# david-mathews-1994/deltarice

Measured on AMD Instinct MI355X. Metric: encode+decode GB/s (int16 in), higher is better.
Workload: dtype int16; 1 GPU; 1000000x7000 int16 Gaussian(sigma=10), m=8, 500 chunks of 2000x7000 per GPU, encode then decode, HBM resident; waveforms_per_gpu=1000000, wave_len=7000, rice_m=8, chunks_per_gpu=500, decode_impl=8

## Files before the change

deltarice_amd/_lib.py:

```python
from __future__ import annotations

import ctypes as C
import os

_HERE = os.path.dirname(os.path.abspath(__file__))
LIB_PATH = os.environ.get("DRX_LIB_PATH") or os.path.join(_HERE, "libdeltarice_hip.so")
PLUGIN_PATH = os.path.join(_HERE, "plugin", "libh5deltarice.so")

DRX_OK = 0
STATUS_NAMES = {0: "DRX_OK", 1: "DRX_ERR_ARG", 2: "DRX_ERR_DEVICE", 3: "DRX_ERR_CAPACITY",
                4: "DRX_ERR_CORRUPT", 5: "DRX_ERR_UNSUPPORTED", 6: "DRX_ERR_NOMEM"}
DRX_MAX_TAPS = 64

PATH_LANES_FUSED, PATH_LANES, PATH_BLOCKS, PATH_LONG, PATH_SIMPLE, PATH_IIR, PATH_IIR_FUSED = 1, 2, 4, 8, 16, 32, 64
PATH_SELECT = 128
PATH_GATHER = 256
PATH_STATS = 512
PATH_TRANSCODE = 1024
PATH_WINDOW = 2048
PATH_PULSES = 4096
PATH_WINDOWS = 8192
PATH_BINS = 16384
PATH_STACK = 32768
STACK_COUNT, STACK_SUM, STACK_SUMSQ = range(3)
STACK_COLS = 3
BIN_SUM, BIN_SUMSQ, BIN_MIN, BIN_MAX = range(4)
BIN_COLS = 4
STAT_MIN, STAT_ARGMIN, STAT_MAX, STAT_ARGMAX, STAT_SUM, STAT_SUMSQ, STAT_HEAD_SUM, STAT_HEAD_SUMSQ = range(8)
STAT_COLS = 8
PULSE_START, PULSE_WIDTH, PULSE_PEAK, PULSE_ARGPEAK, PULSE_SUM = range(5)
PULSE_COLS = 5
ENC_TWO_PASS, ENC_SEGMENTS, ENC_FUSED, ENC_PIECES, ENC_STREAM, ENC_STREAM_SEGS = 1, 2, 3, 4, 5, 6
DBG_BINS_LANES = 64
DBG_BINS_ALL_FALLBACK = 128
DBG_NO_LONG_PATHS = 256
DBG_LONG_NOT_BLOCKS = 512
DBG_TRANSCODE_LANES = 1024
DBG_NO_PARALLEL_WALKS = 2048
DBG_NO_PIECES = 4096
DBG_FORCE_SEGMENTS = 8192
DBG_TRANSCODE_ALL_FALLBACK = 16384
DBG_FORCE_PIECES = 32768
DBG_NO_WIDE_FUSED = 65536
DBG_RAGGED_ONE_LANES_LAUNCH = 131072
DBG_STREAM_THREE_WGS = 262144
DBG_FORCE_STREAM = 524288
DBG_REFILTER_SERIAL = 1048576
DBG_IIR_SEPARATE = 2097152
DBG_FORCE_STREAM_SEGS = 4194304
DBG_WALK_BY_SCAN = 8388608
DBG_WALK_BY_CHAINS = 16777216
DBG_GATHER_OTHER_COPY = 33554432
DBG_STATS_LANES = 67108864
DBG_STATS_ALL_FALLBACK = 134217728
DBG_PULSES_LANES = 268435456
DBG_PULSES_ALL_FALLBACK = 536870912
DBG_WINDOWS_LANES = 1073741824
DBG_WINDOWS_ALL_FALLBACK = 2147483648
STATS_FORM_LANES, STATS_FORM_BLOCKS, STATS_FORM_FALLBACK_ALL = 1, 2, 4
PULSES_FORM_LANES, PULSES_FORM_BLOCKS, PULSES_FORM_FALLBACK_ALL = 1, 2, 4
PULSES_STAGE_CAP = 8
WINDOWS_FORM_LANES, WINDOWS_FORM_BLOCKS, WINDOWS_FORM_FALLBACK_ALL = 1, 2, 4
BINS_FORM_LANES, BINS_FORM_BLOCKS, BINS_FORM_FALLBACK_ALL = 1, 2, 4
TRANSCODE_FORM_LANES, TRANSCODE_FORM_BLOCKS, TRANSCODE_FORM_FALLBACK_ALL = 1, 2, 4
TRANSCODE_FORM_REFILTER, TRANSCODE_FORM_REFILTER_SERIAL = 8, 16


class DrxOpts(C.Structure):
    _fields_ = [("rice_k", C.c_uint32), ("wave_len", C.c_int64), ("n_taps", C.c_uint32),
                ("taps", C.c_int32 * DRX_MAX_TAPS)]


class DeltaRiceError(RuntimeError):
    def __init__(self, status: int, msg: str = ""):
        self.status = status
        super().__init__(f"{STATUS_NAMES.get(status, status)}: {msg}")


_vp, _u64, _u32 = C.c_void_p, C.c_uint64, C.c_uint32
SIGNATURES = {
    "drx_version": (C.c_char_p, []),
    "drx_status_str": (C.c_char_p, [C.c_int]),
    "drx_device_count": (C.c_int, []),
    "drx_parse_cd_values": (C.c_int, [C.c_size_t, C.POINTER(C.c_uint), C.POINTER(DrxOpts)]),
    "drx_ctx_create": (C.c_int, [C.c_int, _vp, C.POINTER(_vp)]),
    "drx_ctx_destroy": (None, [_vp]),
    "drx_ctx_synchronize": (C.c_int, [_vp]),
    "drx_ctx_last_error": (C.c_char_p, [_vp]),
    "drx_ctx_stream": (_vp, [_vp]),
    "drx_ctx_device": (C.c_int, [_vp]),
    "drx_ctx_host_staging": (C.c_int, [_vp, C.c_size_t, C.POINTER(_vp)]),
    "drx_ctx_set_option": (C.c_int, [_vp, C.c_char_p, C.c_int64]),
    "drx_plan_create": (C.c_int, [_vp, _u64, C.POINTER(_u32), C.POINTER(_u32), _u32, C.POINTER(_vp)]),
    "drx_plan_create_uniform": (C.c_int, [_vp, _u64, _u32, _u32, _u32, C.POINTER(_vp)]),
    "drx_plan_set_filter": (C.c_int, [_vp, _u32, C.POINTER(C.c_int32)]),
    "drx_plan_destroy": (None, [_vp]),
    "drx_plan_n_chunks": (_u64, [_vp]),
    "drx_plan_total_samples": (_u64, [_vp]),
    "drx_plan_total_waves": (_u64, [_vp]),
    "drx_plan_max_encoded_words": (_u64, [_vp]),
    "drx_plan_wave_words": (_vp, [_vp]),
    "drx_plan_wave_word_off": (_vp, [_vp]),
    "drx_plan_last_decode_path": (C.c_uint32, [_vp]),
    "drx_plan_last_encode_path": (C.c_uint32, [_vp]),
    "drx_plan_last_stats_form": (C.c_uint32, [_vp]),
    "drx_plan_last_pulses_form": (C.c_uint32, [_vp]),
    "drx_plan_last_windows_form": (C.c_uint32, [_vp]),
    "drx_plan_last_windows_listed": (C.c_uint32, [_vp]),
    "drx_plan_last_bins_form": (C.c_uint32, [_vp]),
    "drx_plan_last_bins_listed": (C.c_uint32, [_vp]),
    "drx_plan_last_transcode_form": (C.c_uint32, [_vp]),
    "drx_plan_last_transcode_listed": (C.c_uint32, [_vp]),
    "drx_plan_last_pulses_listed": (C.c_uint32, [_vp]),
    "drx_plan_last_pulses_redone": (C.c_uint32, [_vp]),
    "drx_plan_read_wave_words": (C.c_int, [_vp, C.POINTER(_u32)]),
    "drx_encode": (C.c_int, [_vp, _vp, _vp, _u64, _vp]),
    "drx_decode": (C.c_int, [_vp, _vp, _u64, _vp, _vp]),
    "drx_decode_with_wave_words": (C.c_int, [_vp, _vp, _u64, _vp, _vp, _vp]),
    "drx_decode_select": (C.c_int, [_vp, _vp, _u64, _vp, C.POINTER(_u64), _u64, _vp, _u64]),
    "drx_decode_select_with_wave_words": (C.c_int, [_vp, _vp, _u64, _vp, _vp, C.POINTER(_u64), _u64, _vp, _u64]),
    "drx_gather_encoded": (C.c_int, [_vp, _vp, _u64, _vp, C.POINTER(_u64), _u64, _u64, _vp, _u64, _vp, _vp]),
    "drx_gather_encoded_with_wave_words": (C.c_int, [_vp, _vp, _u64, _vp, _vp, C.POINTER(_u64), _u64, _u64, _vp, _u64, _vp, _vp]),
    "drx_wave_stats": (C.c_int, [_vp, _vp, _u64, _vp, _u32, _vp]),
    "drx_wave_stats_with_wave_words": (C.c_int, [_vp, _vp, _u64, _vp, _vp, _u32, _vp]),
    "drx_wave_bins": (C.c_int, [_vp, _vp, _u64, _vp, _vp, _u64, C.c_int64, _u32, _u32, _vp, _u64]),
    "drx_wave_bins_with_wave_words": (C.c_int, [_vp, _vp, _u64, _vp, _vp, _vp, _u64, C.c_int64, _u32, _u32, _vp, _u64]),
    "drx_wave_stack": (C.c_int, [_vp, _vp, _u64, _vp, _vp, _u64, C.c_int64, _u32, _vp, _vp, _u64]),
    "drx_wave_stack_with_wave_words": (C.c_int, [_vp, _vp, _u64, _vp, _vp, _vp, _u64, C.c_int64, _u32, _vp, _vp, _u64]),
    "drx_decode_window": (C.c_int, [_vp, _vp, _u64, _vp, _vp, _u64, C.c_int64, _u32, C.c_int16, _vp, _u64]),
    "drx_decode_window_with_wave_words": (C.c_int, [_vp, _vp, _u64, _vp, _vp, _vp, _u64, C.c_int64, _u32, C.c_int16, _vp, _u64]),
    "drx_decode_windows": (C.c_int, [_vp, _vp, _u64, _vp, _vp, _u64, _u64, _vp, _u32, C.c_int64, _u32, C.c_int16, _vp, _u64, _u64]),
    "drx_decode_windows_with_wave_words": (C.c_int, [_vp, _vp, _u64, _vp, _vp, _vp, _u64, _u64, _vp, _u32, C.c_int64, _u32, C.c_int16, _vp, _u64,
                                                     _u64]),
    "drx_find_pulses": (C.c_int, [_vp, _vp, _u64, _vp, _vp, _u64, C.c_int64, C.c_int32, _u32, _u32, _vp, _vp]),
    "drx_find_pulses_with_wave_words": (C.c_int, [_vp, _vp, _u64, _vp, _vp, _vp, _u64, C.c_int64, C.c_int32, _u32, _u32, _vp, _vp]),
    "drx_transcode": (C.c_int, [_vp, _vp, _u64, _vp, _u32, _vp, _u64, _vp, _vp]),
    "drx_transcode_with_wave_words": (C.c_int, [_vp, _vp, _u64, _vp, _vp, _u32, _vp, _u64, _vp, _vp]),
    "drx_estimate_words_encoded": (C.c_int, [_vp, _vp, _u64, _vp, _vp, C.POINTER(_u64)]),
    "drx_transcode_filter": (C.c_int, [_vp, _vp, _u64, _vp, _u32, _u32, C.POINTER(C.c_int32), _vp, _u64, _vp, _vp]),
    "drx_transcode_filter_with_wave_words": (C.c_int, [_vp, _vp, _u64, _vp, _vp, _u32, _u32, C.POINTER(C.c_int32), _vp, _u64, _vp, _vp]),
    "drx_estimate_words_encoded_filter": (C.c_int, [_vp, _vp, _u64, _vp, _vp, _u32, C.POINTER(C.c_int32), C.POINTER(_u64)]),
    "drx_estimate_words": (C.c_int, [_vp, _vp, C.POINTER(_u64)]),
    "drx_plan_last_timings": (C.c_int, [_vp, C.POINTER(C.c_float)]),
    "drx_plan_finish": (C.c_int, [_vp, C.POINTER(_u64)]),
    "drx_filter_chunk_host": (C.c_int, [_vp, C.c_int, C.c_size_t, C.POINTER(C.c_uint), _vp, C.c_size_t,
                                        C.POINTER(_vp), C.POINTER(C.c_size_t)]),
}

_lib = None


def load() -> C.CDLL:
    global _lib
    if _lib is None:
        if not os.path.exists(LIB_PATH):
            raise ImportError(
                f"{LIB_PATH} is missing: build it with `make` (hipcc --offload-arch=gfx950). "
                "deltarice_amd has no CPU fallback.")
        lib = C.CDLL(LIB_PATH)
        for name, (res, args) in SIGNATURES.items():
            f = getattr(lib, name)
            f.restype = res
            f.argtypes = args
        _lib = lib
    return _lib
```

deltarice_amd/codec.py:

```python
from __future__ import annotations

import ctypes as C
import math
from dataclasses import dataclass
from typing import Optional, Sequence

import numpy as np
import torch

from . import _lib
from ._lib import DeltaRiceError, DrxOpts

H5FILTER = 32025


def _cd_values(opts: Sequence[int]):
    return (C.c_uint * max(len(opts), 1))(*[int(v) & 0xFFFFFFFF for v in opts])


def parse_opts(opts: Sequence[int] = ()) -> DrxOpts:
    lib = _lib.load()
    o = DrxOpts()
    st = lib.drx_parse_cd_values(len(opts), _cd_values(opts), C.byref(o))
    if st != _lib.DRX_OK:
# ... 605 lines not shown
        t = (1, -1) if taps is None else tuple(int(v) for v in taps)
        if not 1 <= len(t) <= _lib.DRX_MAX_TAPS:
            raise DeltaRiceError(1, f"taps: {len(t)} values (1 .. {_lib.DRX_MAX_TAPS})")
        if any(not -(1 << 31) <= v < 1 << 31 for v in t):
            raise DeltaRiceError(1, "taps: a value is not an int32")
        return (C.c_int32 * len(t))(*t), len(t), (None if t == (1, -1) else t)

    def estimate_words_refiltered(self, enc: EncodedBatch, taps: Optional[Sequence[int]],
                                  wave_words: Optional[torch.Tensor] = None) -> np.ndarray:
        self._open("estimate_words_refiltered")
        arr, n, _ = self._target_taps(taps)
        return self._estimate("drx_estimate_words_encoded_filter", enc, wave_words, n, arr)

    def refilter_async(self, words: torch.Tensor, chunk_word_off: torch.Tensor, taps: Optional[Sequence[int]], rice_m: int,
                       out_words: Optional[torch.Tensor] = None, in_words: Optional[int] = None,
                       wave_words: Optional[torch.Tensor] = None, out_chunk_word_off: Optional[torch.Tensor] = None,
                       out_wave_words: Optional[torch.Tensor] = None):
        self._open("refilter")
        k = parse_opts((int(rice_m),)).rice_k
        arr, n, _ = self._target_taps(taps)
        return self._batch_call("transcode_filter", words, chunk_word_off, wave_words, in_words, (k, n, arr), out_words,
                                out_chunk_word_off, self.n_chunks, out_wave_words, self.total_waves)

    def refilter(self, enc: EncodedBatch, taps: Optional[Sequence[int]], rice_m: Optional[int] = None,
                 wave_words: Optional[torch.Tensor] = None, out_words: Optional[torch.Tensor] = None) -> "Transcoded":
        self._open("refilter")
        _, _, carried = self._target_taps(taps)
        if rice_m is None:
            rice_m = 1 << int(np.argmin(self.estimate_words_refiltered(enc, taps, wave_words)))
        res, tab = self._sized(self.refilter_async, enc, (taps, rice_m), wave_words, out_words)
        return Transcoded(res, tab, int(rice_m), carried, self._chunk_samples.copy(), self._wave_lens.copy())

    def estimate_words(self, x: torch.Tensor) -> np.ndarray:
        self._dev_check(x, torch.int16, self.total_samples, "x")
        cur = torch.cuda.current_stream(self.ctx.device)
        self.ctx.stream.wait_stream(cur)
        out = (C.c_uint64 * 16)()
        self.ctx._check(self.ctx.lib.drx_estimate_words(self._h, x.data_ptr(), out))
        return np.array(list(out), dtype=np.uint64)

    def last_timings(self):
        ms = (C.c_float * 4)()
        self.ctx._check(self.ctx.lib.drx_plan_last_timings(self._h, ms))
        return tuple(float(v) for v in ms)

    def last_decode_path(self) -> int:
        return int(self.ctx.lib.drx_plan_last_decode_path(self._h))

    def last_stats_form(self) -> int:
        return int(self.ctx.lib.drx_plan_last_stats_form(self._h))

    def last_pulses_form(self) -> int:
        return int(self.ctx.lib.drx_plan_last_pulses_form(self._h))

    def last_windows_form(self) -> int:
        return int(self.ctx.lib.drx_plan_last_windows_form(self._h))

    def last_windows_listed(self) -> int:
        return int(self.ctx.lib.drx_plan_last_windows_listed(self._h))

    def last_bins_form(self) -> int:
        self._open("last_bins_form")
        return int(self.ctx.lib.drx_plan_last_bins_form(self._h))

    def last_bins_listed(self) -> int:
        self._open("last_bins_listed")
        return int(self.ctx.lib.drx_plan_last_bins_listed(self._h))

    def last_transcode_form(self) -> int:
        return int(self.ctx.lib.drx_plan_last_transcode_form(self._h))

    def last_transcode_listed(self) -> int:
        return int(self.ctx.lib.drx_plan_last_transcode_listed(self._h))

    def last_pulses_listed(self) -> int:
        return int(self.ctx.lib.drx_plan_last_pulses_listed(self._h))

    def last_pulses_redone(self) -> int:
        return int(self.ctx.lib.drx_plan_last_pulses_redone(self._h))

    def last_encode_path(self) -> int:
        return int(self.ctx.lib.drx_plan_last_encode_path(self._h))

    def wave_words(self) -> np.ndarray:
        buf = np.empty(self.total_waves, dtype=np.uint32)
        self.ctx._check(self.ctx.lib.drx_plan_read_wave_words(self._h, buf.ctypes.data_as(C.POINTER(C.c_uint32))))
        return buf
```

deltarice_amd/csrc/drx_api.h:

```cpp
#ifndef DRX_API_H
#define DRX_API_H
#include <hip/hip_runtime.h>

#include <cstring>
#include <mutex>
#include <string>
#include <vector>

#include "../../include/deltarice_hip.h"
#include "drx_internal.h"

struct Grown {
    void *ptr = nullptr;
    size_t cap = 0;
};

class Buffers {
    struct Buf { void *ptr; bool pinned; };
    std::vector<Buf> bufs_;
    static void free_buf(const Buf &b) {
        if (b.pinned) (void)hipHostFree(b.ptr);
        else (void)hipFree(b.ptr);
    }

// ... 21 lines not shown
    }
    template <typename T> hipError_t once(T **out, size_t bytes, bool pinned = false) {
        return *out ? hipSuccess : alloc(out, bytes, pinned);
    }

    enum Order { KeepOld, ReleaseFirst };
    static size_t size(size_t need, unsigned slack) { return slack ? need + need / slack + 4096 : need; }
    hipError_t reserve(Grown &b, size_t need, unsigned slack, bool pinned, Order order, hipStream_t wait) {
        if (b.cap >= need) return hipSuccess;
        void *fresh = nullptr;
        hipError_t e = order == KeepOld ? alloc(&fresh, size(need, slack), pinned) : hipSuccess;
        if (e == hipSuccess && b.ptr) e = hipStreamSynchronize(wait);
        if (e != hipSuccess) { release(fresh); return e; }
        release(b.ptr);
        b = Grown{};
        if (order == ReleaseFirst && (e = alloc(&fresh, size(need, slack), pinned)) != hipSuccess) return e;
        b = Grown{fresh, size(need, slack)};
        return hipSuccess;
    }
};

struct HostPlanKey {
    uint32_t samples = 0, wave_len = 0, k = 0, n_taps = 0;
    int32_t taps[DRX_MAX_TAPS] = {0};
    bool operator==(const HostPlanKey &o) const {
        return samples == o.samples && wave_len == o.wave_len && k == o.k && n_taps == o.n_taps && memcmp(taps, o.taps, sizeof taps) == 0;
    }
};

struct drx_ctx {
    int device = 0;
    hipStream_t stream = nullptr;
    bool own_stream = false;
    drx::SideStream side{nullptr, nullptr, nullptr};
    int decode_impl = 8;
    int encode_impl = 2;
    int bins_impl = 0;
    uint32_t stack_workgroups = 0;
    int profile = 0;
    uint32_t debug_flags = 0;
    std::string last_error;
    Buffers mem;
    struct HostPath {
        Grown d_raw, d_enc, h_pin;
        uint64_t *d_off = nullptr;
        drx_plan *plan = nullptr;
        HostPlanKey key;
    } host;
    Grown h_stage;
    std::mutex mu;
    std::mutex err_mu;
};

struct DeviceGuard {
    int prev = -1;
    hipError_t err;
    explicit DeviceGuard(int device) {
        if (hipGetDevice(&prev) != hipSuccess) prev = -1;
        err = (prev == device) ? hipSuccess : hipSetDevice(device);
        if (prev == device) prev = -1;
    }
    ~DeviceGuard() { if (prev >= 0) (void)hipSetDevice(prev); }
    DeviceGuard(const DeviceGuard &) = delete;
    DeviceGuard &operator=(const DeviceGuard &) = delete;
};
#define DRX_ON_DEVICE(ctx)                                                                         \
    DeviceGuard dev_guard_((ctx)->device);                                                         \
    if (dev_guard_.err != hipSuccess)                                                              \
        return drx::fail((ctx), DRX_ERR_DEVICE, "hipSetDevice(%d) failed: %s", (ctx)->device, hipGetErrorString(dev_guard_.err))

struct drx_plan {
    drx_ctx *ctx = nullptr;
    drx::Geom G{};
    Buffers mem;
    uint64_t max_words = 0;
    std::vector<drx::ChunkDesc> host_chunks;
    uint32_t *d_wave_words = nullptr;
    uint32_t *d_wave_rel = nullptr;
    uint64_t *d_wave_off = nullptr;
    uint64_t *d_chunk_words = nullptr;
    drx::DevStatus *d_status = nullptr;
    drx::DevStatus *h_status = nullptr;
    bool last_was_encode = false;
    struct Encoders {
        Grown scan;
        uint32_t *d_seg_bits = nullptr;
        uint64_t *d_seg_pos = nullptr;
        uint64_t *d_pc_scan = nullptr;
        uint64_t pc_wgs = 0;
        uint32_t last_path = 0;
        uint64_t words_per_wave = 0;
    } enc;
    struct Decoder {
        void *d_pw = nullptr;
        void *d_blk = nullptr;
        uint32_t last_path = 0;
    } dec;
    struct BlockForm {
        void *d = nullptr;
        uint32_t last_form = 0;
    };
    BlockForm stats;
    BlockForm windows;
    BlockForm bins;
    struct Pulses : BlockForm {
        Grown stage;
    } pulses;
    struct Transcode { void *d = nullptr; BlockForm blocks; } trc;
    void *stack_list = nullptr;
    struct Selection {
        Grown h, d;
        uint32_t *d_fail = nullptr;
        hipEvent_t copied = nullptr;
    } sel;
    struct Gather {
        Grown d;
        struct Key {
            bool valid = false;
            const uint32_t *d_in = nullptr, *d_sideband = nullptr;
            const uint64_t *d_off = nullptr;
            uint64_t in_words = 0, n_sel = 0, cw = 0;
        } last;
    } gat;
    struct Profiling {
        hipEvent_t ev[4] = {nullptr, nullptr, nullptr, nullptr};
        bool valid = false;
    } prof;
};

namespace drx {

drx_status fail(drx_ctx *ctx, drx_status st, const char *fmt, ...) __attribute__((format(printf, 3, 4)));

#define DRX_HIP(ctx, expr)                                                                           \
    do {                                                                                             \
        hipError_t e_ = (expr);                                                                      \
        if (e_ != hipSuccess)                                                                        \
            return drx::fail((ctx), DRX_ERR_DEVICE, "%s failed: %s", #expr, hipGetErrorString(e_)); \
    } while (0)

void plan_free(drx_plan *p);
hipError_t seg_scratch(drx_plan *p);

drx_status call_begin(drx_plan *p);
drx_status stream_call_begin(drx_plan *p, const uint32_t *d_in, uint64_t in_words, const uint64_t *d_chunk_word_off,
                             const uint32_t *d_sideband, bool tables_ready, StreamCall *c);
drx_status call_end(drx_plan *p, uint32_t path, bool encode = false);
drx_status stream_call_args(drx_plan *p, const char *who, bool have_pointers, const uint32_t *d_sideband, bool sideband);

drx_status decode_launch(drx_plan *p, const uint32_t *d_in, uint64_t in_words, const uint64_t *d_chunk_word_off, int16_t *d_out,
                         bool tables_ready, const uint32_t *d_sideband = nullptr);

}
#endif
```

deltarice_amd/csrc/drx_api_encode.hip:

```cpp
#include "drx_api.h"

using namespace drx;

static bool stream_encoder_suits(const drx_plan *p, int wide) {
    const Geom &G = p->G;
    if (wide != 0 || G.total_waves < kEsMinUnits) return false;
    const uint64_t L = G.uniform ? G.u_wave_len : G.max_wave_len64 / 64u;
    const uint64_t words = p->enc.words_per_wave ? p->enc.words_per_wave : (L * (2u * G.k + 7u)) / 64u;
    return words <= (uint64_t)kEsRingWords * 67u / 100u;
}

static uint32_t stream_segs_target(const drx_plan *p) {
    const Geom &G = p->G;
    const uint64_t L = G.u_wave_len;
    if (L < kEsSegsFromLen) return 0u;
    const uint64_t bps16 = p->enc.words_per_wave ? (p->enc.words_per_wave * 512u) / L : 16u * G.k + 56u;
    uint64_t t = ((uint64_t)kEsRingWords * 32u * 57u / 100u) * 16u / (bps16 ? bps16 : 1u);
    t = t > kEsSegMaxLen ? kEsSegMaxLen : (t < kEsSegMinLen ? kEsSegMinLen : t);
    const EsSegShape sh = es_seg_shape((uint32_t)L, (uint32_t)t);
    if (G.total_waves * sh.nseg < kEsMinUnits) return 0u;
    return (uint32_t)t;
}

struct EncodeRoute { uint32_t enc, seg_target; int wide; };

static EncodeRoute route_encode(const drx_plan *p, int impl, uint32_t dbg) {
    const Geom &G = p->G;
    const int wide = (dbg & DRX_DBG_NO_WIDE_FUSED) ? 0 : fused_wide(G);
    const bool fast = G.n_taps == 0 || G.enc_fast, single = impl >= 1;
    const bool segs_in = impl == 2 && stream_segs_admits(G), pieces_in = single && pieces_admits(G);
    const bool long_in = single && long_batch_admits(G), stream_in = impl == 2 && fast && G.total_waves < 0xffff0000ull;
    const bool fused_in = single && fast && G.total_waves <= kMaxWavefrontWaves;
    if ((dbg & DRX_DBG_FORCE_STREAM_SEGS) && segs_in) return {DRX_ENC_STREAM_SEGS, kEsSegMinLen, wide};
    if ((dbg & DRX_DBG_FORCE_SEGMENTS) && long_in) return {DRX_ENC_SEGMENTS, 0, wide};
    if ((dbg & DRX_DBG_FORCE_PIECES) && pieces_in) return {DRX_ENC_PIECES, 0, wide};
    if ((dbg & DRX_DBG_FORCE_STREAM) && stream_in) return {DRX_ENC_STREAM, 0, wide};
    if (segs_in && !(dbg & (DRX_DBG_NO_PIECES | DRX_DBG_NO_LONG_PATHS)))
        if (const uint32_t t = stream_segs_target(p)) return {DRX_ENC_STREAM_SEGS, t, wide};
    if (pieces_in && !(dbg & DRX_DBG_NO_PIECES) && pieces_batch(G, wide)) return {DRX_ENC_PIECES, 0, wide};
    if (long_in && !(dbg & DRX_DBG_NO_LONG_PATHS) && long_batch(G)) return {DRX_ENC_SEGMENTS, 0, wide};
    if (stream_in && stream_encoder_suits(p, wide)) return {DRX_ENC_STREAM, 0, wide};
    return {fused_in ? DRX_ENC_FUSED : DRX_ENC_TWO_PASS, 0, wide};
}

static drx_status route_scratch(drx_plan *p, const EncodeRoute &R) {
    drx_ctx *ctx = p->ctx;
    if (R.enc == DRX_ENC_STREAM_SEGS)
        DRX_HIP(ctx, p->mem.reserve(p->enc.scan, segs_scan_words(p->G, R.seg_target) * sizeof(uint64_t), 4, false, Buffers::KeepOld, ctx->stream));
    if (R.enc == DRX_ENC_SEGMENTS) DRX_HIP(ctx, seg_scratch(p));
    return DRX_OK;
}

extern "C" {

drx_status drx_encode(drx_plan *p, const int16_t *d_in, uint32_t *d_out, uint64_t out_cap_words,
                      uint64_t *d_chunk_word_off) {
    if (!p || !d_in || !d_out || !d_chunk_word_off) return DRX_ERR_ARG;
    drx_ctx *ctx = p->ctx;
    DRX_ON_DEVICE(ctx);
    if (const drx_status st = call_begin(p)) return st;
    if (const uint64_t w = *(volatile uint64_t *)p->G.host_words) p->enc.words_per_wave = p->G.total_waves ? w / p->G.total_waves : 0;
    const EncodeRoute R = route_encode(p, ctx->encode_impl, ctx->debug_flags);
    if (const drx_status st = route_scratch(p, R)) return st;
    const EncodeCall c{&p->G, d_in, EncOut{d_out, out_cap_words, d_chunk_word_off, p->d_wave_words}, p->d_status,
                       ctx->profile ? p->prof.ev : nullptr, ctx->stream};
    const drx_plan::Encoders &E = p->enc;
    uint64_t *d_scan = (uint64_t *)E.scan.ptr;
    switch (R.enc) {
    case DRX_ENC_STREAM_SEGS: DRX_HIP(ctx, launch_encode_stream_segs(c, R.seg_target, d_scan)); break;
    case DRX_ENC_PIECES: DRX_HIP(ctx, launch_encode_pieces(c, p->G.total_samples, E.d_pc_scan, E.pc_wgs)); break;
    case DRX_ENC_SEGMENTS: DRX_HIP(ctx, launch_encode_long(c, p->d_wave_rel, p->d_chunk_words, E.d_seg_bits, E.d_seg_pos)); break;
    case DRX_ENC_STREAM: DRX_HIP(ctx, launch_encode_stream(c, d_scan)); break;
    case DRX_ENC_FUSED: DRX_HIP(ctx, launch_encode_fused(c, R.wide, d_scan)); break;
    default: DRX_HIP(ctx, launch_encode(c, p->d_wave_rel, p->d_chunk_words));
    }
    return call_end(p, R.enc,  true);
}

drx_status drx_estimate_words(drx_plan *p, const int16_t *d_in, uint64_t words_out[16]) {
    if (!p || !d_in || !words_out) return DRX_ERR_ARG;
    drx_ctx *ctx = p->ctx;
    DRX_ON_DEVICE(ctx);
    DRX_HIP(ctx, hipStreamSynchronize(ctx->stream));
    DRX_HIP(ctx, launch_estimate_words(p->G, d_in, (unsigned long long *)p->enc.scan.ptr, ctx->stream));
    DRX_HIP(ctx, hipMemcpyAsync(words_out, p->enc.scan.ptr, 16 * sizeof(uint64_t), hipMemcpyDeviceToHost, ctx->stream));
    DRX_HIP(ctx, hipStreamSynchronize(ctx->stream));
    return DRX_OK;
}

}
```

deltarice_amd/csrc/drx_api_plan.hip:

```cpp
#include <cstdarg>
#include <cstdio>
#include <cstdlib>
#include <new>

#include "drx_api.h"

using namespace drx;

drx_status drx::fail(drx_ctx *ctx, drx_status st, const char *fmt, ...) {
    char buf[512];
    va_list ap;
    va_start(ap, fmt);
    vsnprintf(buf, sizeof buf, fmt, ap);
    va_end(ap);
    if (ctx) {
        std::lock_guard<std::mutex> lock(ctx->err_mu);
        ctx->last_error = buf;
    }
    return st;
}

drx_status drx::call_begin(drx_plan *p) {
    drx_ctx *ctx = p->ctx;
    p->gat.last.valid = false;
    DRX_HIP(ctx, hipMemsetAsync(p->d_status, 0, sizeof(DevStatus), ctx->stream));
    p->G.dbg = ctx->debug_flags;
    return DRX_OK;
}
drx_status drx::stream_call_begin(drx_plan *p, const uint32_t *d_in, uint64_t in_words, const uint64_t *d_chunk_word_off,
                                  const uint32_t *d_sideband, bool tables_ready, StreamCall *c) {
    drx_ctx *ctx = p->ctx;
    if (const drx_status st = call_begin(p)) return st;
    *c = StreamCall{&p->G, d_in, in_words, d_chunk_word_off, p->d_wave_off, p->d_wave_words, tables_ready || d_sideband, p->dec.d_pw,
                    p->d_status, ctx->profile ? p->prof.ev : nullptr, ctx->stream};
    if (d_sideband)
        DRX_HIP(ctx, launch_sideband_tables(*c, d_sideband));
    return DRX_OK;
}
drx_status drx::call_end(drx_plan *p, uint32_t path, bool encode) {
    (encode ? p->enc.last_path : p->dec.last_path) = path;
    p->prof.valid = p->ctx->profile != 0;
    p->last_was_encode = encode;
    return DRX_OK;
}
drx_status drx::stream_call_args(drx_plan *p, const char *who, bool have_pointers, const uint32_t *d_sideband, bool sideband) {
    if (!have_pointers || (sideband && !d_sideband)) return fail(p->ctx, DRX_ERR_ARG, "%s: null pointer", who);
    if (sideband && d_sideband == p->d_wave_words) return fail(p->ctx, DRX_ERR_ARG, "the side-band table must not be the plan's own (copy it first)");
    return DRX_OK;
}

template <typename T> static hipError_t upload(drx_plan *p, const T *host, size_t n, const T **view) {
    if (!n) return hipSuccess;
    T *d = const_cast<T *>(*view);
    const hipError_t e = p->mem.once(&d, n * sizeof(T));
    if (e != hipSuccess) return e;
    *view = d;
    return hipMemcpy(d, host, n * sizeof(T), hipMemcpyHostToDevice);
}
template <typename T> static hipError_t upload(drx_plan *p, const std::vector<T> &tab, const T **view) {
    return upload(p, tab.data(), tab.size(), view);
}

void drx::plan_free(drx_plan *p) {
    if (!p) return;
    DeviceGuard guard(p->ctx->device);
    for (hipEvent_t e : p->prof.ev) if (e) (void)hipEventDestroy(e);
    if (p->sel.copied) (void)hipEventDestroy(p->sel.copied);
    delete p;
}

hipError_t drx::seg_scratch(drx_plan *p) {
    drx_plan::Encoders &E = p->enc;
    if (E.d_seg_bits) return hipSuccess;
    const uint64_t units = long_batch_units(p->G);
    hipError_t e = p->mem.once(&E.d_seg_bits, units * sizeof(uint32_t));
    if (e == hipSuccess && (e = p->mem.once(&E.d_seg_pos, units * sizeof(uint64_t))) != hipSuccess) {
        p->mem.release(E.d_seg_bits);
        E.d_seg_bits = nullptr;
    }
    return e;
}

static drx_status plan_alloc(drx_plan *p) {
    drx_ctx *ctx = p->ctx;
    Geom &G = p->G;
    const uint64_t W = G.total_waves ? G.total_waves : 1;
    DRX_HIP(ctx, p->mem.alloc(&p->d_wave_words, W * sizeof(uint32_t)));
    DRX_HIP(ctx, p->mem.alloc(&p->d_wave_rel, W * sizeof(uint32_t)));
    DRX_HIP(ctx, p->mem.alloc(&p->d_wave_off, W * sizeof(uint64_t)));
    DRX_HIP(ctx, p->mem.alloc(&p->d_chunk_words, (G.n_chunks + 1) * sizeof(uint64_t)));
    uint64_t words = 2 * W + 192;
    if (stream_segs_admits(G) && G.u_wave_len >= kEsSegsFromLen) words = std::max(words, segs_scan_words(G, kEsSegMinLen));
    DRX_HIP(ctx, p->mem.reserve(p->enc.scan, words * sizeof(uint64_t), 0, false, Buffers::KeepOld, ctx->stream));
    DRX_HIP(ctx, p->mem.alloc(&p->d_status, sizeof(DevStatus)));
    DRX_HIP(ctx, hipMemset(p->d_status, 0, sizeof(DevStatus)));
    DRX_HIP(ctx, p->mem.alloc(&p->h_status, sizeof(DevStatus), true));
    memset(p->h_status, 0, sizeof(DevStatus));
    DRX_HIP(ctx, p->mem.alloc(&G.host_words, sizeof(uint64_t), true));
    *G.host_words = 0;
    for (hipEvent_t &e : p->prof.ev) DRX_HIP(ctx, hipEventCreate(&e));
    return DRX_OK;
}

static drx_status plan_ragged(drx_plan *p, const std::vector<ChunkDesc> &desc) {
    Geom &G = p->G;
    const ChunkDesc *d = desc.data();
    const std::vector<uint32_t> walk_lists = walk_plan_ragged(G, d);
    const std::vector<uint2> order = decode_plan_ragged(G, d);
    const std::vector<uint64_t> unit_base = segments_plan_ragged(G, d);
    const std::vector<uint32_t> wg_base = pieces_plan_ragged(G, d);
    p->enc.pc_wgs = wg_base.empty() ? 0 : wg_base.back();
    const std::vector<uint32_t> blk_list = blocks_plan_ragged(G, d);
    std::vector<uint64_t> tile_base;
    if (!blk_list.empty()) {
        tile_base.resize(G.n_chunks + 1);
        G.iir_n_tiles = iir_tiles(G, d, tile_base.data());
    }
    hipError_t e = upload(p, desc, &G.chunks);
    if (e == hipSuccess) e = upload(p, walk_lists, &G.walk_short);
    if (e == hipSuccess) e = upload(p, order, &G.rag_order);
    if (e == hipSuccess) e = upload(p, unit_base, &G.seg_unit_base);
    if (e == hipSuccess) e = upload(p, wg_base, &G.pc_wg_base);
    if (e == hipSuccess) e = upload(p, blk_list, &G.rag_blk_list);
    if (e == hipSuccess) e = upload(p, tile_base, &G.iir_chunk_tile_base);
    if (e != hipSuccess) return fail(p->ctx, DRX_ERR_DEVICE, "chunk table upload failed: %s", hipGetErrorString(e));
    G.walk_long = G.walk_short + G.n_short;
    return DRX_OK;
}

static drx_status plan_alloc_scratch(drx_plan *p) {
    drx_ctx *ctx = p->ctx;
    Geom &G = p->G;
    if (long_batch(G)) DRX_HIP(ctx, seg_scratch(p));
    if (const uint64_t nb = walk_scratch_bytes(G)) DRX_HIP(ctx, p->mem.alloc(&p->dec.d_pw, nb));
    if (const uint64_t nb = blocks_scratch_bytes(G)) {
        DRX_HIP(ctx, p->mem.alloc(&p->dec.d_blk, nb));
        if (G.uniform) G.iir_n_tiles = iir_tiles(G, nullptr, nullptr);
        DRX_HIP(ctx, p->mem.alloc(&G.iir_state, (G.iir_n_tiles + 1) * sizeof(uint64_t)));
    }
    if (G.uniform && pieces_admits(G)) p->enc.pc_wgs = pieces_workgroups(G);
    if (p->enc.pc_wgs) DRX_HIP(ctx, p->mem.alloc(&p->enc.d_pc_scan, pieces_scan_words(G, p->enc.pc_wgs) * sizeof(uint64_t)));
    return DRX_OK;
}

static drx_status chunk_desc(drx_ctx *ctx, uint64_t c, uint32_t N, uint32_t wave_len, ChunkDesc *out) {
    if (N == 0 || N > 0x7fffffffu) return fail(ctx, DRX_ERR_ARG, "chunk %llu: bad sample count %u", (unsigned long long)c, N);
    const uint32_t L = wave_len ? wave_len : N;
    if (L > 0x7fffffffu) return fail(ctx, DRX_ERR_ARG, "chunk %llu: bad waveform length", (unsigned long long)c);
    *out = ChunkDesc{0, 0, N, L, (uint32_t)(((uint64_t)N + L - 1) / L), 0};
    return DRX_OK;
}

static drx_status plan_create(drx_ctx *ctx, uint64_t n_chunks, const uint32_t *chunk_samples, const uint32_t *chunk_wave_len,
                              bool per_chunk, uint32_t rice_k, drx_plan **out) {
    if (!ctx || !out || !n_chunks || !chunk_samples || !chunk_wave_len) return DRX_ERR_ARG;
    *out = nullptr;
    if (rice_k > 15) return fail(ctx, DRX_ERR_ARG, "rice_k %u out of range 0..15", rice_k);
    if (n_chunks > 0xffffffffull) return fail(ctx, DRX_ERR_ARG, "too many chunks");
    ChunkDesc first;
    if (const drx_status st = chunk_desc(ctx, 0, chunk_samples[0], chunk_wave_len[0], &first)) return st;
    std::vector<ChunkDesc> desc;
    bool uniform = true;
    if (per_chunk) {
        desc.resize(n_chunks);
        uint64_t soff = 0, wbase = 0;
        for (uint64_t c = 0; c < n_chunks; ++c) {
            if (const drx_status st = chunk_desc(ctx, c, chunk_samples[c], chunk_wave_len[c], &desc[c])) return st;
            desc[c].sample_off = soff;
            desc[c].wave_base = wbase;
            uniform = uniform && desc[c].n_samples == first.n_samples && desc[c].wave_len == first.wave_len;
            soff += desc[c].n_samples;
            wbase += desc[c].n_waves;
        }
        if (uniform) desc.clear();
    }
    DRX_ON_DEVICE(ctx);
    drx_plan *p = new (std::nothrow) drx_plan;
    if (!p) return DRX_ERR_NOMEM;
// ... 154 lines not shown
    if (!strcmp(key, "debug_flags")) {
        c->debug_flags = (uint32_t)value;
        return DRX_OK;
    }
    if (!strcmp(key, "profile")) {
        c->profile = value != 0;
        return DRX_OK;
    }
    return DRX_ERR_ARG;
}

drx_status drx_plan_create(drx_ctx *ctx, uint64_t n_chunks, const uint32_t *chunk_samples,
                           const uint32_t *chunk_wave_len, uint32_t rice_k, drx_plan **out) {
    return plan_create(ctx, n_chunks, chunk_samples, chunk_wave_len, true, rice_k, out);
}

drx_status drx_plan_create_uniform(drx_ctx *ctx, uint64_t n_chunks, uint32_t chunk_samples,
                                   uint32_t wave_len, uint32_t rice_k, drx_plan **out) {
    return plan_create(ctx, n_chunks, &chunk_samples, &wave_len, false, rice_k, out);
}

drx_status drx_plan_set_filter(drx_plan *p, uint32_t n_taps, const int32_t *taps) {
    if (!p || !taps || n_taps == 0 || n_taps > DRX_MAX_TAPS) return DRX_ERR_ARG;
    drx_ctx *ctx = p->ctx;
    if (taps[0] == 0) return fail(ctx, DRX_ERR_ARG, "taps[0] must not be 0 (the inverse filter divides by it)");
    DRX_ON_DEVICE(ctx);
    DRX_HIP(ctx, hipStreamSynchronize(ctx->stream));
    Geom &G = p->G;
    p->enc.words_per_wave = 0;
    p->gat.last.valid = false;
    *G.host_words = 0;
    G.fast_taps = 0;
    G.enc_fast = 0;
    const bool delta = n_taps == 2 && taps[0] == 1 && taps[1] == -1;
    if (!delta && n_taps <= 4) {
        G.enc_fast = 1;
        for (uint32_t j = 0; j < 4; ++j) G.enc_t[j] = (j < n_taps) ? (uint32_t)taps[j] & 0xffffu : 0u;
    }
    if (!delta && n_taps <= 4 && (taps[0] == 1 || taps[0] == -1)) {
        G.fast_taps = 1;
        G.fast_t0neg = taps[0] == -1;
        for (uint32_t j = 1; j < 4; ++j) G.fast_nt[j - 1] = (j < n_taps) ? 0u - (uint32_t)taps[j] : 0u;
    }
    if (G.fast_taps && G.iir_state) {
        const uint32_t words = kIirTabWords + blocks_iir_tab_words();
        std::vector<uint32_t> tab(words);
        iir_tables(G.fast_nt, G.fast_t0neg, tab.data());
        blocks_iir_tables(G.fast_nt, G.fast_t0neg, tab.data() + kIirTabWords);
        DRX_HIP(ctx, upload(p, tab, &G.iir_tab));
        G.blk_iir_tab = G.iir_tab + kIirTabWords;
    } else {
        p->mem.release(G.iir_tab);
        G.iir_tab = G.blk_iir_tab = nullptr;
    }
    if (delta) {
        p->mem.release(G.taps);
        G.n_taps = 0;
        G.taps = nullptr;
        return DRX_OK;
    }
    int32_t t[DRX_MAX_TAPS] = {0};
    memcpy(t, taps, n_taps * sizeof(int32_t));
    DRX_HIP(ctx, upload(p, t, DRX_MAX_TAPS, &G.taps));
    G.n_taps = n_taps;
    return DRX_OK;
}

void drx_plan_destroy(drx_plan *p) { plan_free(p); }
uint64_t drx_plan_n_chunks(const drx_plan *p) { return p ? p->G.n_chunks : 0; }
uint64_t drx_plan_total_samples(const drx_plan *p) { return p ? p->G.total_samples : 0; }
uint64_t drx_plan_total_waves(const drx_plan *p) { return p ? p->G.total_waves : 0; }
uint64_t drx_plan_max_encoded_words(const drx_plan *p) { return p ? p->max_words : 0; }
const uint32_t *drx_plan_wave_words(const drx_plan *p) { return p ? p->d_wave_words : nullptr; }
const uint64_t *drx_plan_wave_word_off(const drx_plan *p) { return p ? p->d_wave_off : nullptr; }
uint32_t drx_plan_last_decode_path(const drx_plan *p) { return p ? p->dec.last_path : 0u; }
uint32_t drx_plan_last_encode_path(const drx_plan *p) { return p ? p->enc.last_path : 0u; }
uint32_t drx_plan_last_stats_form(const drx_plan *p) { return p ? p->stats.last_form : 0u; }
uint32_t drx_plan_last_pulses_form(const drx_plan *p) { return p ? p->pulses.last_form : 0u; }
uint32_t drx_plan_last_windows_form(const drx_plan *p) { return p ? p->windows.last_form : 0u; }
uint32_t drx_plan_last_transcode_form(const drx_plan *p) { return p ? p->trc.blocks.last_form : 0u; }
uint32_t drx_plan_last_transcode_listed(const drx_plan *p) { return (p && p->h_status && p->dec.last_path == DRX_PATH_TRANSCODE) ? p->h_status->listed : 0u; }
uint32_t drx_plan_last_pulses_redone(const drx_plan *p) { return (p && p->h_status && p->dec.last_path == DRX_PATH_PULSES) ? p->h_status->redone : 0u; }
uint32_t drx_plan_last_pulses_listed(const drx_plan *p) { return (p && p->h_status && p->dec.last_path == DRX_PATH_PULSES) ? p->h_status->listed : 0u; }
uint32_t drx_plan_last_bins_form(const drx_plan *p) { return p ? p->bins.last_form : 0u; }
uint32_t drx_plan_last_bins_listed(const drx_plan *p) { return (p && p->h_status && p->dec.last_path == DRX_PATH_BINS) ? p->h_status->listed : 0u; }
uint32_t drx_plan_last_windows_listed(const drx_plan *p) { return (p && p->h_status && p->dec.last_path == DRX_PATH_WINDOWS) ? p->h_status->listed : 0u; }

drx_status drx_plan_read_wave_words(drx_plan *p, uint32_t *host_out) {
    if (!p || !host_out) return DRX_ERR_ARG;
    drx_ctx *ctx = p->ctx;
    DRX_ON_DEVICE(ctx);
    DRX_HIP(ctx, hipMemcpyAsync(host_out, p->d_wave_words, p->G.total_waves * sizeof(uint32_t),
                                hipMemcpyDeviceToHost, ctx->stream));
    DRX_HIP(ctx, hipStreamSynchronize(ctx->stream));
    return DRX_OK;
}

drx_status drx_plan_last_timings(drx_plan *p, float ms[4]) {
    if (!p || !ms) return DRX_ERR_ARG;
    drx_ctx *ctx = p->ctx;
    if (!p->prof.valid) return fail(ctx, DRX_ERR_ARG, "set the context option \"profile\" before the call to be timed");
    DRX_ON_DEVICE(ctx);
    hipEvent_t *ev = p->prof.ev;
    DRX_HIP(ctx, hipEventSynchronize(ev[3]));
    for (int i = 0; i < 3; ++i) DRX_HIP(ctx, hipEventElapsedTime(&ms[i], ev[i], ev[i + 1]));
    DRX_HIP(ctx, hipEventElapsedTime(&ms[3], ev[0], ev[3]));
    return DRX_OK;
}

drx_status drx_plan_finish(drx_plan *p, uint64_t *total_words) {
    if (!p) return DRX_ERR_ARG;
    drx_ctx *ctx = p->ctx;
    DRX_ON_DEVICE(ctx);
    DRX_HIP(ctx, hipMemcpyAsync(p->h_status, p->d_status, sizeof(DevStatus), hipMemcpyDeviceToHost, ctx->stream));
    DRX_HIP(ctx, hipStreamSynchronize(ctx->stream));
    if (total_words) *total_words = p->h_status->total_words;
    if (p->last_was_encode && !p->h_status->err && p->G.total_waves) p->enc.words_per_wave = p->h_status->total_words / p->G.total_waves;
    if (p->h_status->err & kErrInternal) return fail(ctx, DRX_ERR_DEVICE, "encoder look-back timed out (internal error)");
    if (p->h_status->err & kErrCorrupt) return fail(ctx, DRX_ERR_CORRUPT, "encoded input failed header-chain validation");
    if (p->h_status->err & kErrCapacity)
        return fail(ctx, DRX_ERR_CAPACITY, "encoded batch needs %llu words", (unsigned long long)p->h_status->total_words);
    return DRX_OK;
}

}
```

deltarice_amd/csrc/drx_api_select.hip:

```cpp
#include <algorithm>
#include <new>

#include "drx_api.h"
#include "drx_sel_survey.h"

using namespace drx;

template <typename F>
static int plan_survey(drx_plan *p, const char *who, const uint64_t *wave_idx, uint64_t n_sel, bool sideband,
                       std::vector<uint32_t> &lists, uint32_t n_class[3], uint64_t *at, F &&per_entry) {
    const Geom &G = p->G;
    const SelGeom S{G.uniform != 0, G.n_chunks, G.total_waves, G.u_n_samples, G.u_wave_len, G.u_n_waves};
    const int r = sel_survey(S, p->host_chunks.data(), wave_idx, n_sel, sideband, select_walk_class, lists, n_class, at, per_entry);
    if (r == kSelBadIndex)
        (void)fail(p->ctx, DRX_ERR_ARG, "%s: entry %llu is waveform %llu of %llu", who, (unsigned long long)*at,
                   (unsigned long long)wave_idx[*at], (unsigned long long)G.total_waves);
    return r;
}

static drx_status sel_scratch(drx_plan *p, size_t bytes) {
    drx_ctx *ctx = p->ctx;
    drx_plan::Selection &S = p->sel;
    if (!S.copied) DRX_HIP(ctx, hipEventCreateWithFlags(&S.copied, hipEventDisableTiming));
    DRX_HIP(ctx, p->mem.once(&S.d_fail, p->G.n_chunks * sizeof(uint32_t)));
    DRX_HIP(ctx, p->mem.reserve(S.h, bytes, 4, true, Buffers::KeepOld, ctx->stream));
    const hipError_t e = p->mem.reserve(S.d, bytes, 4, false, Buffers::KeepOld, ctx->stream);
    if (e != hipSuccess) return fail(ctx, DRX_ERR_NOMEM, "selection scratch of %zu bytes: %s", Buffers::size(bytes, 4), hipGetErrorString(e));
    return DRX_OK;
}

static drx_status gather_scratch(drx_plan *p, size_t bytes) {
    const hipError_t e = p->mem.reserve(p->gat.d, bytes, 4, false, Buffers::KeepOld, p->ctx->stream);
    if (e != hipSuccess) return fail(p->ctx, DRX_ERR_NOMEM, "gather scratch of %zu bytes: %s", Buffers::size(bytes, 4), hipGetErrorString(e));
    return DRX_OK;
}

struct SelStaged {
    const uint64_t *d_sel;
    const uint32_t *d_chunk_n, *d_lists;
};
static SelStaged sel_staged(const drx_plan *p, uint64_t n_sel, uint64_t n_out) {
    const uint32_t *d_chunk_n = (const uint32_t *)((const char *)p->sel.d.ptr + n_sel * sizeof(uint64_t));
    return SelStaged{(const uint64_t *)p->sel.d.ptr, d_chunk_n, d_chunk_n + n_out};
}
static drx_status sel_stage(drx_plan *p, const uint64_t *wave_idx, uint64_t n_sel, const std::vector<uint32_t> &chunk_n,
                            const std::vector<uint32_t> &lists, size_t gather_bytes) {
    drx_ctx *ctx = p->ctx;
    const size_t sel_bytes = n_sel * sizeof(uint64_t), cn_bytes = chunk_n.size() * sizeof(uint32_t), ls_bytes = lists.size() * sizeof(uint32_t);
    if (const drx_status st = sel_scratch(p, sel_bytes + cn_bytes + ls_bytes)) return st;
    if (gather_bytes)
        if (const drx_status st = gather_scratch(p, gather_bytes)) return st;
    char *h_sel = (char *)p->sel.h.ptr;
    DRX_HIP(ctx, hipEventSynchronize(p->sel.copied));
    memcpy(h_sel, wave_idx, sel_bytes);
    if (cn_bytes) memcpy(h_sel + sel_bytes, chunk_n.data(), cn_bytes);
    memcpy(h_sel + sel_bytes + cn_bytes, lists.data(), ls_bytes);
    DRX_HIP(ctx, hipMemcpyAsync(p->sel.d.ptr, h_sel, sel_bytes + cn_bytes + ls_bytes, hipMemcpyHostToDevice, ctx->stream));
    DRX_HIP(ctx, hipEventRecord(p->sel.copied, ctx->stream));
    return DRX_OK;
}
static drx_status sel_walk(drx_plan *p, const StreamCall &c, const uint32_t *d_sideband, const uint32_t *d_lists, size_t n_lists,
                           const uint32_t n_class[3]) {
    drx_ctx *ctx = p->ctx;
    mark(c.ev, 0, c.s);
    if (d_sideband)
        DRX_HIP(ctx, launch_sideband_tables(c, d_sideband, d_lists, (uint32_t)n_lists));
    else
        DRX_HIP(ctx, launch_select_walk(c, d_lists, n_class[0], n_class[1], n_class[2], p->sel.d_fail));
    mark(c.ev, 1, c.s);
    return DRX_OK;
}

template <typename F> static drx_status list_call(drx_plan *p, const char *who, uint64_t n_sel, F &&f) {
    try {
        return f();
    } catch (const std::bad_alloc &) { return fail(p->ctx, DRX_ERR_NOMEM, "%s: host memory for a list of %llu entries", who, (unsigned long long)n_sel); }
}

static drx_status decode_select(drx_plan *p, const uint32_t *d_in, uint64_t in_words, const uint64_t *d_chunk_word_off,
                                const uint32_t *d_sideband, bool sideband, const uint64_t *wave_idx, uint64_t n_sel,
                                int16_t *d_out, uint64_t stride) {
    if (!p) return DRX_ERR_ARG;
    drx_ctx *ctx = p->ctx;
    if (n_sel == 0) return DRX_OK;
    if (!d_in || !d_chunk_word_off || !wave_idx || !d_out || (sideband && !d_sideband)) return fail(ctx, DRX_ERR_ARG, "decode_select: null pointer");
    if (sideband && d_sideband == p->d_wave_words) return fail(ctx, DRX_ERR_ARG, "the side-band table must not be the plan's own (copy it first)");
    if (n_sel >= (1ull << 32)) return fail(ctx, DRX_ERR_ARG, "decode_select: %llu entries (at most 2^32 - 1)", (unsigned long long)n_sel);
    uint32_t longest = 0;
    uint32_t n_class[3];
    uint64_t at;
    std::vector<uint32_t> lists;
    if (plan_survey(p, "decode_select", wave_idx, n_sel, sideband, lists, n_class, &at, [&](uint64_t, uint64_t, uint32_t len) {
            longest = std::max(longest, len);
            return 0;
        }))
        return DRX_ERR_ARG;
    p->gat.last.valid = false;
    if (stride < longest) return fail(ctx, DRX_ERR_ARG, "decode_select: row stride %llu below the longest selected waveform (%u)", (unsigned long long)stride, longest);
    DRX_ON_DEVICE(ctx);
    if (const drx_status st = sel_stage(p, wave_idx, n_sel, {}, lists, 0)) return st;
    const SelStaged S = sel_staged(p, n_sel, 0);
    StreamCall c;
    if (const drx_status st = stream_call_begin(p, d_in, in_words, d_chunk_word_off, nullptr, false, &c)) return st;
    if (const drx_status st = sel_walk(p, c, sideband ? d_sideband : nullptr, S.d_lists, lists.size(), n_class)) return st;
    DRX_HIP(ctx, launch_decode_select(c, S.d_sel, n_sel, d_out, stride));
    mark(c.ev, 2, c.s);
    mark(c.ev, 3, c.s);
    return call_end(p, DRX_PATH_SELECT);
}

constexpr uint64_t kGatherWavesFromWords = 192;

static drx_status gather_encoded(drx_plan *p, const uint32_t *d_in, uint64_t in_words, const uint64_t *d_chunk_word_off,
                                 const uint32_t *d_sideband, bool sideband, const uint64_t *wave_idx, uint64_t n_sel,
                                 uint64_t cw, uint32_t *d_out, uint64_t out_cap, uint64_t *d_out_off, uint32_t *d_out_wave_words) {
    if (!p) return DRX_ERR_ARG;
    drx_ctx *ctx = p->ctx;
    if (cw == 0) return fail(ctx, DRX_ERR_ARG, "gather_encoded: out_chunk_waves is 0");
    if (n_sel == 0) return DRX_OK;
    if (!d_in || !d_chunk_word_off || !wave_idx || !d_out_off || (sideband && !d_sideband)) return fail(ctx, DRX_ERR_ARG, "gather_encoded: null pointer");
    if (!d_out && out_cap) return fail(ctx, DRX_ERR_ARG, "gather_encoded: no output buffer but a capacity of %llu words", (unsigned long long)out_cap);
    if (sideband && (d_sideband == p->d_wave_words || d_out_wave_words == d_sideband))
        return fail(ctx, DRX_ERR_ARG, "the side-band table must be neither the plan's own nor the output's (copy it first)");
    if (n_sel >= (1ull << 32)) return fail(ctx, DRX_ERR_ARG, "gather_encoded: %llu entries (at most 2^32 - 1)", (unsigned long long)n_sel);
    const Geom &G = p->G;
    const uint64_t n_out = (n_sel + cw - 1) / cw;
    const EncOut out{d_out, out_cap, d_out_off, d_out_wave_words};
    const uint64_t mean_words = in_words / G.total_waves;
    const bool tiles = (mean_words < kGatherWavesFromWords) != ((ctx->debug_flags & DRX_DBG_GATHER_OTHER_COPY) != 0);
    const drx_plan::Gather::Key K = p->gat.last;
    p->gat.last.valid = false;
    if (K.valid && d_out && K.d_in == d_in && K.in_words == in_words && K.d_off == d_chunk_word_off && K.d_sideband == (sideband ? d_sideband : nullptr) &&
        K.n_sel == n_sel && K.cw == cw && memcmp(p->sel.h.ptr, wave_idx, n_sel * sizeof(uint64_t)) == 0) {
        DRX_ON_DEVICE(ctx);
        StreamCall c;
        if (const drx_status st = stream_call_begin(p, d_in, in_words, d_chunk_word_off, nullptr, true, &c)) return st;
        const SelStaged S = sel_staged(p, n_sel, n_out);
        mark(c.ev, 0, c.s);
        mark(c.ev, 1, c.s);
        DRX_HIP(ctx, launch_gather(c, S.d_sel, n_sel, cw, S.d_chunk_n, out, gather_scratch_view(p->gat.d.ptr, n_sel), tiles, mean_words,  true));
        mark(c.ev, 3, c.s);
        return call_end(p, DRX_PATH_GATHER);
    }
    std::vector<uint32_t> chunk_n(n_out);
    GatherChunks rule{cw, chunk_n.data()};
    uint32_t n_class[3], refused_len = 0;
    uint64_t at;
    std::vector<uint32_t> lists;
    const int refused = plan_survey(p, "gather_encoded", wave_idx, n_sel, sideband, lists, n_class, &at, [&](uint64_t i, uint64_t, uint32_t len) {
        refused_len = len;
        return (int)rule.add(i, len);
// ... 62 lines not shown
```

deltarice_amd/csrc/drx_api_stream.hip:

```cpp
#include "drx_api.h"

using namespace drx;

drx_status drx::decode_launch(drx_plan *p, const uint32_t *d_in, uint64_t in_words, const uint64_t *d_chunk_word_off, int16_t *d_out,
                              bool tables_ready, const uint32_t *d_sideband) {
    if (!p || !d_in || !d_chunk_word_off || !d_out) return DRX_ERR_ARG;
    drx_ctx *ctx = p->ctx;
    DRX_ON_DEVICE(ctx);
    StreamCall c;
    if (const drx_status st = stream_call_begin(p, d_in, in_words, d_chunk_word_off, d_sideband, tables_ready, &c)) return st;
    DRX_HIP(ctx, launch_decode(c, d_out, (uint64_t *)p->enc.scan.ptr, ctx->decode_impl, p->dec.d_blk, ctx->side.s ? &ctx->side : nullptr,
                               &p->dec.last_path));
    return call_end(p, p->dec.last_path);
}

static hipError_t form_scratch(drx_plan *p, const BlkFormRule &r, drx_plan::BlockForm &f, uint64_t (*bytes)(const Geom &)) {
    return blocks_form_batch(p->G, p->dec.d_blk, r) ? p->mem.once(&f.d, bytes(p->G)) : hipSuccess;
}

static drx_status wave_stats(drx_plan *p, const uint32_t *d_in, uint64_t in_words, const uint64_t *d_chunk_word_off,
                             const uint32_t *d_sideband, bool sideband, uint32_t head_len, int64_t *d_out) {
    if (!p) return DRX_ERR_ARG;
    drx_ctx *ctx = p->ctx;
    if (const drx_status st = stream_call_args(p, "wave_stats", d_in && d_chunk_word_off && d_out, d_sideband, sideband)) return st;
    DRX_ON_DEVICE(ctx);
    StreamCall c;
    if (const drx_status st = stream_call_begin(p, d_in, in_words, d_chunk_word_off, d_sideband, false, &c)) return st;
    DRX_HIP(ctx, form_scratch(p, kStatsForm, p->stats, stats_blocks_scratch_bytes));
    DRX_HIP(ctx, launch_wave_stats(c, p->dec.d_blk, p->stats.d, head_len, d_out, &p->stats.last_form));
    return call_end(p, DRX_PATH_STATS);
}

static drx_status wave_bins(drx_plan *p, const uint32_t *d_in, uint64_t in_words, const uint64_t *d_chunk_word_off,
                            const uint32_t *d_sideband, bool sideband, const int64_t *d_start, uint64_t start_stride, int64_t offset,
                            uint32_t bin, uint32_t n_bins, int64_t *d_out, uint64_t out_wave_stride) {
    if (!p) return DRX_ERR_ARG;
    drx_ctx *ctx = p->ctx;
    if (const drx_status st = stream_call_args(p, "wave_bins", d_in && d_chunk_word_off && d_out, d_sideband, sideband)) return st;
    if (bin == 0) return fail(ctx, DRX_ERR_ARG, "wave_bins: bin 0");
    if (d_start && start_stride == 0) return fail(ctx, DRX_ERR_ARG, "wave_bins: start_stride 0");
    if (out_wave_stride < (uint64_t)n_bins * DRX_BIN_COLS)
        return fail(ctx, DRX_ERR_ARG, "wave_bins: waveforms %llu int64 apart do not hold %u rows", (unsigned long long)out_wave_stride, n_bins);
    if (n_bins == 0) return DRX_OK;
    DRX_ON_DEVICE(ctx);
    StreamCall c;
    if (const drx_status st = stream_call_begin(p, d_in, in_words, d_chunk_word_off, d_sideband, false, &c)) return st;
    if (ctx->bins_impl == 1) DRX_HIP(ctx, form_scratch(p, kBinsForm, p->bins, bins_blocks_scratch_bytes));
    DRX_HIP(ctx, launch_wave_bins(c, p->dec.d_blk, p->bins.d, ctx->bins_impl, d_start, start_stride, offset, bin, n_bins, d_out, out_wave_stride,
                                  &p->bins.last_form));
    return call_end(p, DRX_PATH_BINS);
}

static drx_status decode_window(drx_plan *p, const uint32_t *d_in, uint64_t in_words, const uint64_t *d_chunk_word_off,
                                const uint32_t *d_sideband, bool sideband, const int64_t *d_start, uint64_t start_stride,
                                int64_t offset, uint32_t width, int16_t pad, int16_t *d_out, uint64_t out_stride) {
    if (!p) return DRX_ERR_ARG;
    drx_ctx *ctx = p->ctx;
    if (const drx_status st = stream_call_args(p, "decode_window", d_in && d_chunk_word_off && d_out, d_sideband, sideband)) return st;
    if (out_stride < width)
        return fail(ctx, DRX_ERR_ARG, "decode_window: rows %llu samples apart do not hold %u", (unsigned long long)out_stride, width);
    if (d_start && start_stride == 0) return fail(ctx, DRX_ERR_ARG, "decode_window: start_stride 0");
    if (width == 0) return DRX_OK;
    DRX_ON_DEVICE(ctx);
    StreamCall c;
    if (const drx_status st = stream_call_begin(p, d_in, in_words, d_chunk_word_off, d_sideband, false, &c)) return st;
    DRX_HIP(ctx, launch_decode_window(c, d_start, start_stride, offset, width, pad, d_out, out_stride));
    return call_end(p, DRX_PATH_WINDOW);
}

static drx_status wave_stack(drx_plan *p, const uint32_t *d_in, uint64_t in_words, const uint64_t *d_chunk_word_off,
                             const uint32_t *d_sideband, bool sideband, const int64_t *d_start, uint64_t start_stride, int64_t offset,
                             uint32_t width, const uint8_t *d_select, int64_t *d_out, uint64_t out_stride) {
    if (!p) return DRX_ERR_ARG;
    drx_ctx *ctx = p->ctx;
    if (const drx_status st = stream_call_args(p, "wave_stack", d_in && d_chunk_word_off && d_out, d_sideband, sideband)) return st;
    if (d_start && start_stride == 0) return fail(ctx, DRX_ERR_ARG, "wave_stack: start_stride 0");
    if (out_stride < (uint64_t)DRX_STACK_COLS)
        return fail(ctx, DRX_ERR_ARG, "wave_stack: rows %llu int64 apart do not hold %d", (unsigned long long)out_stride, DRX_STACK_COLS);
    if (width == 0) return DRX_OK;
    DRX_ON_DEVICE(ctx);
    StreamCall c;
    if (const drx_status st = stream_call_begin(p, d_in, in_words, d_chunk_word_off, d_sideband, false, &c)) return st;
    if (d_select) DRX_HIP(ctx, p->mem.once(&p->stack_list, stack_list_bytes(p->G)));
    DRX_HIP(ctx, launch_wave_stack(c, p->stack_list, ctx->stack_workgroups, d_start, start_stride, offset, width, d_select, d_out, out_stride));
    return call_end(p, DRX_PATH_STACK);
}

static drx_status decode_windows(drx_plan *p, const uint32_t *d_in, uint64_t in_words, const uint64_t *d_chunk_word_off,
                                 const uint32_t *d_sideband, bool sideband, const int64_t *d_start, uint64_t start_wave_stride,
                                 uint64_t start_win_stride, const uint32_t *d_count, uint32_t n_win, int64_t offset, uint32_t width,
                                 int16_t pad, int16_t *d_out, uint64_t out_wave_stride, uint64_t out_win_stride) {
    if (!p) return DRX_ERR_ARG;
    drx_ctx *ctx = p->ctx;
    if (const drx_status st = stream_call_args(p, "decode_windows", d_in && d_chunk_word_off && d_start && d_out, d_sideband, sideband)) return st;
    if (start_wave_stride == 0 || start_win_stride == 0) return fail(ctx, DRX_ERR_ARG, "decode_windows: a start stride of 0");
// ... 262 lines not shown
```

deltarice_amd/csrc/drx_decode_kernels.hip:

```cpp
#include <hip/hip_runtime.h>
#include <stdint.h>

#include <algorithm>
#include <type_traits>

#include "drx_internal.h"
#include "drx_device.h"
#include "drx_lane_stream.h"
#include "drx_walk.h"

namespace drx {

__global__ __launch_bounds__(64) void k_decode_simple(Geom G, const uint32_t *__restrict__ in,
                                                      const uint64_t *__restrict__ wave_off,
                                                      const uint32_t *__restrict__ wave_words, DevStatus *st,
                                                      int16_t *__restrict__ out, const uint32_t *__restrict__ only) {
    const uint64_t g = (uint64_t)blockIdx.x * 64u + threadIdx.x;
    if (g >= G.total_waves) return;
    if (only && !only[g]) return;
    const WaveRef r = locate(G, g);
    const uint32_t *s = in + wave_off[g] + 1;
    const uint32_t n = wave_words[g];
    int16_t *y = out + r.sample_off;
    int16_t hist[64];
// ... 547 lines not shown
            const int st = i * SPI + lane / PPS, p = lane % PPS;
            const uint4 v = orow16(st, p);
            store16(outg + wo_off[i] + t0, v);
        }
        wave_sync();
    }
    commit_if_fits();
    pneed = false;
    wave_sync();
    for (; t0 < steps; t0 += T) edge_round(t0);
    if (active && len && (((0u - Q_end) - 32u * s0 + 31u) >> 5) != n) atomicOr(&st->err, kErrCorrupt);
}

std::vector<uint2> decode_plan_ragged(Geom &G, const ChunkDesc *d) {
    const uint64_t n = G.n_chunks;
    uint32_t max_groups = 0, max_len = 0;
    for (uint64_t c = 0; c < n; ++c) {
        max_groups = std::max(max_groups, (d[c].n_waves + 63u) / 64u);
        max_len = std::max(max_len, d[c].wave_len);
    }
    G.max_groups = max_groups;
    G.max_wave_len64 = 64ull * max_len;
    std::vector<uint32_t> by_len(n);
    for (uint64_t c = 0; c < n; ++c) by_len[c] = (uint32_t)c;
    std::stable_sort(by_len.begin(), by_len.end(), [&](uint32_t a, uint32_t b) { return d[a].wave_len > d[b].wave_len; });
    std::vector<uint2> order;
    uint64_t n_long_groups = 0;
    for (uint32_t c : by_len)
        for (uint32_t j = 0; j < (d[c].n_waves + 63u) / 64u; ++j) {
            order.push_back(make_uint2(c, j));
            if (d[c].wave_len > kWalkShortLen) ++n_long_groups;
        }
    if (order.size() <= 0x7fffffffull) {
        G.rag_groups = (uint32_t)order.size();
        G.rag_groups_long = (uint32_t)n_long_groups;
    } else {
        order.clear();
    }
    return order;
}

enum class Dec { Simple, Blocks, Long, LanesFused, Lanes, LanesSplit };
enum class Walk { None, InLaunch, Parallel, Serial };
struct DecodeRoute {
    Dec dec;
    Walk walk;
    WalkRoute par;
    bool gen;
};

static DecodeRoute route_decode(const Geom &G, int impl, bool tables_ready, bool have_pw, bool have_blk, bool have_side) {
    DecodeRoute R{};
    R.gen = G.n_taps != 0;
    R.par = route_walk(G, tables_ready, have_pw);
    const bool simple = impl == 0 || (R.gen && !G.fast_taps);
    const bool want_fused = !tables_ready && impl == 8;
    const bool blocks = !simple && !(G.dbg & (DRX_DBG_NO_LONG_PATHS | DRX_DBG_LONG_NOT_BLOCKS)) && have_blk && blocks_batch(G) && (!R.gen || (G.iir_tab && G.iir_state));
    const bool longp = !simple && !blocks && !R.gen && !(G.dbg & DRX_DBG_NO_LONG_PATHS) && G.uniform && long_waveform_batch(G.total_waves, G.u_wave_len);
    const bool sparse = !G.uniform && (uint64_t)G.n_chunks * G.max_groups > 8ull * ((G.total_waves + 63u) / 64u) + 4096ull;
    R.dec = simple ? Dec::Simple : (blocks ? Dec::Blocks : (longp ? Dec::Long : Dec::Lanes));
    const bool parallel = R.par.chunk_wide || R.par.blocks;
    if (R.dec == Dec::Lanes && want_fused && !sparse && !parallel) R.dec = Dec::LanesFused;
    R.walk = tables_ready ? Walk::None : (R.dec == Dec::LanesFused ? Walk::InLaunch : (parallel ? Walk::Parallel : Walk::Serial));
    if (R.dec == Dec::Lanes && R.par.chunk_wide && R.par.blocks && have_side && G.rag_order && G.rag_groups_long &&
        G.rag_groups_long < G.rag_groups && !(G.dbg & DRX_DBG_RAGGED_ONE_LANES_LAUNCH)) R.dec = Dec::LanesSplit;
    return R;
}

hipError_t launch_decode(const StreamCall &c, int16_t *d_out, uint64_t *d_granules, int impl, void *d_blk, const SideStream *side,
                         uint32_t *path_out) {
    const Geom &G = *c.G;
    const hipStream_t s = c.s;
    uint32_t path_dummy = 0;
    uint32_t &path = path_out ? *path_out : path_dummy;
    path = 0;
    if (G.total_waves == 0) return hipSuccess;
    mark(c.ev, 0, s);
    const DecodeRoute R = route_decode(G, impl, c.tables_ready, c.d_pw != nullptr, d_blk != nullptr, side && side->s);
    const bool gen = R.gen;
    const unsigned nb_plain = blocks_for(G.total_waves, 64);

    auto launch_lanes = [&](const StreamCall &v, unsigned nb) {
        path |= DRX_PATH_LANES;
        if (gen)
            k_decode_lanes<false, true><<<nb, 64, 0, v.s>>>(*v.G, v.d_in, v.in_words, v.d_chunk_word_off, v.d_wave_off, v.d_wave_words, nullptr, nullptr, v.d_status, d_out);
        else
            k_decode_lanes<false><<<nb, 64, 0, v.s>>>(*v.G, v.d_in, v.in_words, v.d_chunk_word_off, v.d_wave_off, v.d_wave_words, nullptr, nullptr, v.d_status, d_out);
    };

    if (R.walk == Walk::InLaunch) {
        hipError_t e = hipMemsetAsync(d_granules, 0, (G.total_waves + 2) * sizeof(uint64_t), s);
        if (e != hipSuccess) return e;
    } else if (R.walk == Walk::Parallel) {
        const bool split = R.dec == Dec::LanesSplit;
        hipError_t e = walk_scratch_reset(G, c.d_pw, s);
        if (e != hipSuccess) return e;
        const bool forked = R.par.chunk_wide && R.par.blocks && side && side->s;
        hipStream_t spw = forked ? side->s : s;
        if (forked) {
            if ((e = hipEventRecord(side->fork, s)) != hipSuccess) return e;
            if ((e = hipStreamWaitEvent(side->s, side->fork, 0)) != hipSuccess) return e;
        }
        if (R.par.chunk_wide) launch_walk_chunk_wide(c.on(spw), R.par.by_chains);
        if (split) {
            Geom Gl = G;
            Gl.rag_groups = G.rag_groups_long;
            launch_lanes(c.view(Gl).on(spw), Gl.rag_groups);
        }
        if (forked && (e = hipEventRecord(side->join, side->s)) != hipSuccess) {
            (void)hipStreamSynchronize(side->s);
            return e;
        }
        if (R.par.blocks) launch_walk_blocks(c);
        if (split) {
            mark(c.ev, 1, s);
            Geom Gs = G;
            Gs.rag_order = G.rag_order + G.rag_groups_long;
            Gs.rag_groups = G.rag_groups - G.rag_groups_long;
            launch_lanes(c.view(Gs), Gs.rag_groups);
        }
        if (forked && (e = hipStreamWaitEvent(s, side->join, 0)) != hipSuccess) {
            (void)hipStreamSynchronize(side->s);
            return e;
        }
    } else if (R.walk == Walk::Serial) {
        launch_walk_serial(c);
    }
    if (R.dec != Dec::LanesSplit) mark(c.ev, 1, s);

    switch (R.dec) {
    case Dec::LanesFused: {
        uint32_t *ticket = reinterpret_cast<uint32_t *>(d_granules + G.total_waves);
        unsigned n_walk, groups;
        unsigned nb;
        if (G.uniform) {
            n_walk = (G.u_wave_len <= kWalkShortLen) ? (unsigned)G.n_chunks : blocks_for(G.n_chunks, kWalkChains);
            groups = (G.u_n_waves + 63u) / 64u;
            const uint32_t full = G.u_n_waves >> 6, rem = G.u_n_waves & 63u;
            nb = n_walk + (unsigned)(G.n_chunks * full) + (rem ? (unsigned)((G.n_chunks + 64u / rem - 1u) / (64u / rem)) : 0u);
        } else {
            n_walk = G.n_short + blocks_for(G.n_long, kWalkChains);
            groups = G.max_groups;
            nb = n_walk + (unsigned)(G.n_chunks * groups);
        }
        path |= DRX_PATH_LANES_FUSED;
        if (gen)
            k_decode_lanes<true, true><<<nb, 64, 0, s>>>(G, c.d_in, c.in_words, c.d_chunk_word_off, c.d_wave_off, c.d_wave_words, d_granules, ticket, c.d_status, d_out);
        else
            k_decode_lanes<true><<<nb, 64, 0, s>>>(G, c.d_in, c.in_words, c.d_chunk_word_off, c.d_wave_off, c.d_wave_words, d_granules, ticket, c.d_status, d_out);
        break;
    }
    case Dec::Blocks: {
        const uint32_t *fail = nullptr, *suspect = nullptr;
        bool fused = false;
        hipError_t e = launch_decode_blocks(c, d_blk, d_out, &fail, &suspect, gen, &fused);
        if (e != hipSuccess) return e;
        path |= DRX_PATH_BLOCKS | (gen ? (fused ? DRX_PATH_IIR_FUSED : DRX_PATH_IIR) : 0u);
        k_decode_long<<<(unsigned)G.total_waves, kLongThreads, 0, s>>>(G, c.d_in, c.d_wave_off, c.d_wave_words, c.d_status, d_out, fail, suspect, gen ? 1u : 0u);
        if (gen) {
            if (!fused && (e = launch_iir(G, G.iir_chunk_tile_base, G.iir_n_tiles, G.iir_tab, G.iir_state, fail, c.d_status, d_out, s)) != hipSuccess) return e;
            k_decode_simple<<<nb_plain, 64, 0, s>>>(G, c.d_in, c.d_wave_off, c.d_wave_words, c.d_status, d_out, fail);
        }
        break;
    }
    case Dec::Long:
        path |= DRX_PATH_LONG;
        k_decode_long<<<(unsigned)G.total_waves, kLongThreads, 0, s>>>(G, c.d_in, c.d_wave_off, c.d_wave_words, c.d_status, d_out, nullptr, nullptr, 0u);
        break;
    case Dec::Lanes:
        launch_lanes(c, (!G.uniform && G.rag_order) ? G.rag_groups : nb_plain);
        break;
    case Dec::LanesSplit:
        break;
    case Dec::Simple:
        path |= DRX_PATH_SIMPLE;
        k_decode_simple<<<nb_plain, 64, 0, s>>>(G, c.d_in, c.d_wave_off, c.d_wave_words, c.d_status, d_out, nullptr);
        break;
    }
    mark(c.ev, 2, s);
    mark(c.ev, 3, s);
    return hipGetLastError();
}

}
```

deltarice_amd/csrc/drx_encode_kernels.hip:

```cpp
#include <hip/hip_runtime.h>
#include <stdint.h>

#include <algorithm>
#include <type_traits>

#include "drx_internal.h"
#include "drx_device.h"
#include "drx_encode.h"
#include "drx_lookback.h"

namespace drx {

constexpr int kStageWords = 416;

__device__ __forceinline__ int load8(const int16_t *__restrict__ x, uint32_t len, uint32_t t0, int lane,
                                     bool vec_ok, int32_t v[8]) {
    const uint32_t i0 = t0 + 8u * (uint32_t)lane;
    const int nv = (i0 >= len) ? 0 : (int)((len - i0) < 8u ? (len - i0) : 8u);
    if (vec_ok && nv == 8) {
        const uint4 q = *reinterpret_cast<const uint4 *>(x + i0);
        v[0] = (int16_t)(q.x & 0xffffu); v[1] = (int16_t)(q.x >> 16);
        v[2] = (int16_t)(q.y & 0xffffu); v[3] = (int16_t)(q.y >> 16);
        v[4] = (int16_t)(q.z & 0xffffu); v[5] = (int16_t)(q.z >> 16);
        v[6] = (int16_t)(q.w & 0xffffu); v[7] = (int16_t)(q.w >> 16);
// ... 476 lines not shown
                                                  const uint64_t *__restrict__ chunk_word_off, uint32_t *__restrict__ out,
                                                  uint64_t out_cap, uint32_t upw) {
    __shared__ __attribute__((aligned(16))) uint32_t stage_all[4][4 + kStageWords + 12];
    const int lane = lane_id();
    const int wv = wave_id();
    uint32_t *row = stage_all[wv];
    uint32_t *stage = row + 4;
    const uint64_t u0 = ((uint64_t)blockIdx.x * 4u + (uint32_t)wv) * upw;
    for (uint32_t rep = 0; rep < upw; ++rep) {
        const uint64_t u = u0 + rep;
        if (u >= n_units) return;
        const SegRef q = locate_seg_uniform(G, u, segs_per_wave);
        if (q.count == 0) continue;
        for (int i = lane; i < 4 + (int)kStageWords + 12; i += 64) row[i] = 0;
        const uint64_t pos = chunk_word_off[q.r.chunk] + wave_rel[q.g];
        const uint32_t n = wave_words[q.g];
        if (pos + 1u + n > out_cap) continue;
        if (q.s == 0 && lane == 0) {
            out[pos] = n;
            if (q.r.idx == 0) out[pos - 1] = q.r.n_samples;
        }
        const uint64_t B = seg_pos[u];
        uint32_t *__restrict__ outp = out + pos + 1 + (B >> 5);
        const uint32_t stage_bits = lds_addr(stage) * 8u;
        uint32_t P = (uint32_t)(B & 31u);
        uint32_t wdone = 0;
        bool shared_first = (B & 31u) != 0;
        wave_sync();
        for_segment_tiles(in + q.r.sample_off, q, G.k, lane,
                          [&](const PackedCodes &c, uint32_t lane_bits, uint32_t incl, uint32_t tile_bits, bool full) {
            if (full && !__any(lane_bits > 128u)) {
                uint32_t cw[4];
                concat_codes(c, cw);
                place_words(cw, stage_bits + P + incl);
            } else {
                emit_tile<false>(c, stage_bits + P + incl - lane_bits);
            }
            P += tile_bits;
            wave_sync();
            const uint32_t nfull = P >> 5;
            for (uint32_t i = lane; i < nfull; i += 64) {
                const uint32_t v = stage[i];
                stage[i] = 0;
                if (i == 0 && shared_first) atomicOr(outp + wdone, v); else outp[wdone + i] = v;
            }
            wave_sync();
            if (nfull) {
                if (lane == 0) { const uint32_t cwd = stage[nfull]; stage[nfull] = 0; stage[0] = cwd; }
                shared_first = false;
                wdone += nfull;
                P &= 31u;
            }
            wave_sync();
        });
        if (P && lane == 0) {
            if (q.last && !shared_first) outp[wdone] = stage[0]; else atomicOr(outp + wdone, stage[0]);
        }

        wave_sync();
    }
}

constexpr uint64_t kWaveSliceBlocks = 1u << 22;
template <class F> static void for_wave_slices(uint64_t total_waves, F go) {
    const uint64_t blocks = (total_waves + 3u) / 4u;
    for (uint64_t b0 = 0; b0 < blocks; b0 += kWaveSliceBlocks) go(4u * b0, (unsigned)std::min(kWaveSliceBlocks, blocks - b0));
}

hipError_t launch_estimate_words(const Geom &G, const int16_t *d_in, unsigned long long *d_words16, hipStream_t s) {
    hipError_t e = hipMemsetAsync(d_words16, 0, 16 * sizeof(unsigned long long), s);
    if (e != hipSuccess || G.total_waves == 0) return e;
    const uint32_t per = (uint32_t)((G.total_waves + (1u << 18) - 1u) >> 18);
    k_estimate_words<<<blocks_for(G.total_waves, 4u * per), 256, 0, s>>>(G, per, d_in, d_words16);
    return hipGetLastError();
}

hipError_t launch_encode_fused(const EncodeCall &c, int wide, uint64_t *d_scan) {
    const Geom &G = *c.G;
    const hipStream_t s = c.s;
    if (G.total_waves == 0) return hipSuccess;
    mark(c.ev, 0, s);
    hipError_t e = hipMemsetAsync(d_scan, 0, (G.total_waves + 2) * sizeof(uint64_t), s);
    if (e != hipSuccess) return e;
    mark(c.ev, 1, s);
    mark(c.ev, 2, s);
    uint32_t *ticket = reinterpret_cast<uint32_t *>(d_scan + G.total_waves);
    auto go = [&](auto gen_tag, auto wv_tag, auto cap_tag) {
        constexpr bool GEN = decltype(gen_tag)::value;
        constexpr int WV = decltype(wv_tag)::value;
        constexpr uint32_t CAPW = decltype(cap_tag)::value;
        k_encode_fused<GEN, WV, CAPW><<<blocks_for(G.total_waves, WV), 64 * WV, 0, s>>>(G, c.d_in, c.out.d_out, c.out.out_cap, c.out.d_chunk_word_off,
                                                                                      c.out.d_wave_words, d_scan, ticket, c.d_status);
    };
    using std::integral_constant;
    const std::true_type T;
    const std::false_type F;
    auto pick = [&](auto wv_tag, auto cap_tag) { if (G.n_taps) go(T, wv_tag, cap_tag); else go(F, wv_tag, cap_tag); };
    switch (wide) {
        case 1: pick(integral_constant<int, 8>{}, integral_constant<uint32_t, kEncWide1Words>{}); break;
        case 2: pick(integral_constant<int, 4>{}, integral_constant<uint32_t, kEncWide2Words>{}); break;
        case 3: pick(integral_constant<int, 4>{}, integral_constant<uint32_t, kEncWide3Words>{}); break;
        default: pick(integral_constant<int, kEncWaves>{}, integral_constant<uint32_t, kEncCapWords>{}); break;
    }
    mark(c.ev, 3, s);
    return hipGetLastError();
}

hipError_t launch_chunk_offsets(const Geom &G, const uint32_t *d_wave_words, uint32_t *d_wave_rel, uint64_t *d_chunk_words,
                                uint64_t *d_chunk_word_off, uint64_t out_cap, DevStatus *d_status, hipStream_t s) {
    k_chunk_scan<<<(unsigned)G.n_chunks, 256, 0, s>>>(G, d_wave_words, d_wave_rel, d_chunk_words);
    k_chunk_offsets<<<1, 1024, 0, s>>>(G.n_chunks, d_chunk_words, d_chunk_word_off, out_cap, d_status, nullptr);
    return hipGetLastError();
}

hipError_t launch_encode(const EncodeCall &c, uint32_t *d_wave_rel, uint64_t *d_chunk_words) {
    const Geom &G = *c.G;
    const EncOut &o = c.out;
    const hipStream_t s = c.s;
    if (G.total_waves == 0) return hipSuccess;
    mark(c.ev, 0, s);
    for_wave_slices(G.total_waves, [&](uint64_t g0, unsigned nb) { k_encode_sizes<<<nb, 256, 0, s>>>(G, g0, c.d_in, o.d_wave_words); });
    mark(c.ev, 1, s);
    k_chunk_scan<<<(unsigned)G.n_chunks, 256, 0, s>>>(G, o.d_wave_words, d_wave_rel, d_chunk_words);
    k_chunk_offsets<<<1, 1024, 0, s>>>(G.n_chunks, d_chunk_words, o.d_chunk_word_off, o.out_cap, c.d_status, G.host_words);
    mark(c.ev, 2, s);
    for_wave_slices(G.total_waves, [&](uint64_t g0, unsigned nb) {
        k_encode_pack<<<nb, 256, 0, s>>>(G, g0, c.d_in, o.d_wave_words, d_wave_rel, o.d_chunk_word_off, o.d_out, o.out_cap);
    });
    mark(c.ev, 3, s);
    return hipGetLastError();
}

bool long_batch_admits(const Geom &G) {
    return !G.n_taps && (G.uniform || G.seg_unit_base != nullptr) && G.total_waves <= kMaxWavefrontWaves && long_batch_units(G) <= kMaxWavefrontWaves;
}
constexpr uint32_t kSegShortLen = 3072, kSegLongLen = 10240;
static bool seg_len_suits(uint32_t wave_len) { return wave_len <= kSegShortLen || wave_len >= kSegLongLen; }
bool long_batch(const Geom &G) {
    return long_batch_admits(G) && (!G.uniform || long_waveform_batch(G.total_waves, G.u_wave_len) || seg_len_suits(G.u_wave_len));
}
static uint32_t segments_of(uint32_t wave_len) { return (wave_len + kSegSamples - 1u) / kSegSamples; }
uint64_t long_batch_units(const Geom &G) { return G.uniform ? G.total_waves * segments_of(G.u_wave_len) : G.seg_units; }

std::vector<uint64_t> segments_plan_ragged(Geom &G, const ChunkDesc *d) {
    bool seg = false;
    std::vector<uint64_t> unit_base(G.n_chunks + 1, 0);
    for (uint64_t c = 0; c < G.n_chunks; ++c) {
        seg = seg || seg_len_suits(d[c].wave_len);
        unit_base[c + 1] = unit_base[c] + (uint64_t)d[c].n_waves * segments_of(d[c].wave_len);
    }
    if (!seg) return {};
    G.seg_units = unit_base[G.n_chunks];
    return unit_base;
}

hipError_t launch_encode_long(const EncodeCall &c, uint32_t *d_wave_rel, uint64_t *d_chunk_words, uint32_t *d_seg_bits,
                              uint64_t *d_seg_pos) {
    const Geom &G = *c.G;
    const EncOut &o = c.out;
    const hipStream_t s = c.s;
    if (G.total_waves == 0) return hipSuccess;
    const uint32_t S = G.uniform ? segments_of(G.u_wave_len) : 0u;
    const uint64_t units = long_batch_units(G);
    mark(c.ev, 0, s);
    const uint32_t upw = (G.uniform && S == 1u && G.u_wave_len <= 1024u) ? 8u : 1u;
    k_seg_sizes<<<blocks_for(units, 4 * upw), 256, 0, s>>>(G, c.d_in, S, units, upw, d_seg_bits);
// ... 14 lines not shown
```

deltarice_amd/csrc/drx_encode_stream.hip:

```cpp
#include <hip/hip_runtime.h>
#include <stdint.h>

#include <type_traits>

#include "drx_internal.h"
#include "drx_device.h"
#include "drx_encode.h"

namespace drx {

constexpr int kEsWaves = 4;
constexpr uint32_t kEsFront = kBufFront;
constexpr uint32_t kEsBack = 12;
constexpr uint64_t kEsFlag = 1ull << 63;
constexpr uint32_t kEsCtrlWords = 32;
constexpr uint32_t kEsRing = kEsRingWords;
constexpr int kEsPollSleep = 4;

__device__ __forceinline__ uint64_t es_load(const uint64_t *p) {
    return __hip_atomic_load(p, __ATOMIC_RELAXED, __HIP_MEMORY_SCOPE_AGENT);
}
__device__ __forceinline__ void es_store(uint64_t *p, uint64_t v) {
    __hip_atomic_store(p, v, __ATOMIC_RELAXED, __HIP_MEMORY_SCOPE_AGENT);
}

constexpr uint32_t kScPer = 8;

__device__ __forceinline__ void es_scanner(uint64_t total, const uint64_t *__restrict__ size, uint64_t *__restrict__ place,
                                           DevStatus *st) {
    const int lane = lane_id();
    if (threadIdx.x >= 64) return;
    __builtin_amdgcn_s_setprio(3);
    uint64_t pos = 0, base = 0;
    uint32_t idle = 0;
    auto sample = [&](uint64_t (&v)[kScPer], uint64_t at) {
#pragma unroll
        for (int j = 0; j < (int)kScPer; ++j) {
            const uint64_t e = at + 64u * j + (uint32_t)lane;
            v[j] = e < total ? es_load(size + e) : kEsFlag;
        }
    };
    while (pos < total) {
        uint64_t v[kScPer];
        const uint64_t bs = pos;
        sample(v, pos);
        uint64_t run = 0;
        bool open = true, big = false;
#pragma unroll
        for (int j = 0; j < (int)kScPer; ++j) {
            const uint64_t e = bs + 64u * j + (uint32_t)lane;
            const uint64_t m = __ballot(e < pos || (v[j] >> 63) != 0);
            const uint32_t l = (m == ~0ull) ? 64u : (uint32_t)__builtin_ctzll(~m);
            run += open ? l : 0u;
            open = open && l == 64u;
            big = big || __any((v[j] & ~kEsFlag) >= (1ull << 24));
        }
        uint64_t end = bs + run;
        end = end < total ? end : total;
        if (end <= pos) {
            if (++idle > (1u << 22)) {
                if (lane == 0) atomicOr(&st->err, kErrInternal);
                return;
            }
            __builtin_amdgcn_s_sleep(1);
            continue;
        }
        idle = 0;
        uint64_t running = 0;
#pragma unroll
        for (int j = 0; j < (int)kScPer; ++j) {
            if (bs + 64u * j < end) {
                const uint64_t e = bs + 64u * j + (uint32_t)lane;
                const bool in = e >= pos && e < end;
                const uint64_t val = in ? (v[j] & ~kEsFlag) : 0ull;
                uint64_t inc;
                if (!big) {
                    inc = wave_incl_scan_dpp((uint32_t)val);
                } else {
                    inc = val;
#pragma unroll
                    for (int d = 1; d < 64; d <<= 1) {
                        const uint64_t t = __shfl_up(inc, d);
                        if (lane >= d) inc += t;
                    }
                }
                if (in) es_store(place + e, kEsFlag | (base + running + inc - val));
                running += big ? __shfl(inc, 63) : (uint64_t)(uint32_t)__builtin_amdgcn_readlane((int)(uint32_t)inc, 63);
            }
        }
        base += running;
        pos = end;
    }
}

template <int WV>
struct EsShared {
    uint32_t role, arrive, ticket[4];
    uint64_t mine[2][WV];
    uint32_t place_t[2];
};

template <int WV>
__device__ __forceinline__ uint32_t es_rendezvous(EsShared<WV> &shm, uint32_t cyc, int lane, int wv, uint32_t *__restrict__ ctrl,
                                                  uint64_t *__restrict__ size, uint32_t Tprev, uint64_t &off) {
    typedef uint32_t __attribute__((address_space(3))) lds_u32;
    uint32_t arr = 0;
    if (lane == 0) arr = __hip_atomic_fetch_add((lds_u32 *)&shm.arrive, 1u, __ATOMIC_RELAXED, __HIP_MEMORY_SCOPE_WORKGROUP);
    arr = (uint32_t)__builtin_amdgcn_readfirstlane((int)arr);
    if (arr == (uint32_t)WV * cyc) {
        if (lane == 0) shm.ticket[cyc & 3u] = atomicAdd(ctrl + 32, 1u);
    }
    __syncthreads();
    const uint32_t T = rfl(shm.ticket[cyc & 3u]);
    if (cyc) {
        uint64_t sum = 0, before = 0;
#pragma unroll
        for (int i = 0; i < WV; ++i) {
            const uint64_t m = rfl64(shm.mine[(cyc - 1u) & 1u][i]);
            sum += m;
            before += i < wv ? m : 0ull;
        }
        off = before;
        if (wv == 0 && lane == 0) es_store(size + Tprev, kEsFlag | sum);
    }
    return T;
}

template <uint32_t RING>
__device__ __forceinline__ uint32_t es_gap(bool pend, uint32_t startA, uint32_t start, uint32_t behind) {
    if (!pend) return RING - 8u;
    const uint32_t d = startA >= start ? startA - start : startA + RING - start;
    return d > behind ? d - behind : 0u;
}

template <typename InLds, typename Wait, typename Copy>
__device__ __forceinline__ bool es_release(bool must, uint64_t P, InLds &&place_in_lds, Wait &&wait_place, Copy &&copy_out) {
    decltype(wait_place()) pl;
    const bool seen = place_in_lds(pl);
    if (!(seen || must)) return false;
    if (!seen) __builtin_amdgcn_s_setprio(0);
    else if (P < (uint64_t)(4u * kTile * 7u)) __builtin_amdgcn_s_setprio(2);
    else __builtin_amdgcn_s_setprio(1);
    copy_out(seen ? pl : wait_place());
    return true;
}

template <uint32_t RING, typename Put>
__device__ __forceinline__ void ring_put_with(const TileCodes &t, uint32_t *row, uint32_t s0, int lane, Put &&put) {
    constexpr uint32_t kRingBits = RING * 32u;
    uint32_t *ring = row + kEsFront;
    const uint32_t ring_bits0 = lds_addr(ring) * 8u;
    put([&](uint32_t bit) -> uint32_t {
        const uint32_t b = s0 + bit;
        return ring_bits0 + (b >= kRingBits ? b - kRingBits : b);
    });
    if (s0 < kRingBits && s0 + t.tile_bits >= kRingBits) {
        wave_sync();
        if (lane < (int)kEsFront) {
            const uint32_t v = row[lane];
            if (v) { ring[RING - kEsFront + lane] |= v; row[lane] = 0; }
        } else if (lane < (int)(kEsFront + kEsBack)) {
            const uint32_t i = (uint32_t)lane - kEsFront, v = ring[RING + i];
            if (v) { ring[i] |= v; ring[RING + i] = 0; }
        }
        wave_sync();
    }
}
template <bool FULLT, uint32_t RING>
__device__ __forceinline__ void ring_put(const TileCodes &t, uint32_t *row, uint32_t s0, int lane) {
    ring_put_with<RING>(t, row, s0, lane, [&](auto &&at) { put_tile<FULLT>(t, at); });
}

static unsigned es_grid(const Geom &G, uint64_t tickets) {
    const unsigned full = 256u * (16u / kEsWaves);
    return (G.dbg & DRX_DBG_STREAM_THREE_WGS) ? 3u : (unsigned)(tickets + 1 < full ? tickets + 1 : full);
}

template <bool GEN, int WV, uint32_t RING>
__global__ __launch_bounds__(64 * WV, 4) void k_encode_stream(Geom G, const int16_t *__restrict__ in, uint32_t *__restrict__ out,
                                                              uint64_t out_cap, uint64_t *__restrict__ chunk_word_off,
                                                              uint32_t *__restrict__ wave_words, uint64_t *__restrict__ size,
                                                              uint64_t *__restrict__ place, uint32_t *__restrict__ ctrl,
                                                              DevStatus *st) {
    __shared__ __attribute__((aligned(16))) uint32_t ring_all[WV][kEsFront + RING + kEsBack];
    __shared__ EsShared<WV> shm;
    __shared__ uint64_t s_place_v[2];
    typedef uint32_t __attribute__((address_space(3))) lds_u32;
    typedef uint64_t __attribute__((address_space(3))) lds_u64;
    static_assert((kEsFront + RING + kEsBack) % 4 == 0 && RING % 4 == 0, "16-byte LDS accesses");
    constexpr uint32_t kRowWords = kEsFront + RING + kEsBack;
    const int lane = lane_id(), wv = wave_id();
    uint32_t *row = ring_all[wv];
    uint32_t *ring = row + kEsFront;

    if (threadIdx.x == 0) {
        shm.role = atomicAdd(ctrl, 1u);
        shm.arrive = 0;
        shm.place_t[0] = shm.place_t[1] = 0;
    }
    zero_row(row, kRowWords, lane);
    __syncthreads();
    const uint64_t n_tickets = (G.total_waves + WV - 1) / WV;
    if (rfl(shm.role) == 0) {
        es_scanner(n_tickets, size, place, st);
        return;
    }

    const uint32_t k = G.k;
    const u16x2 tp[4] = {splat(GEN ? G.enc_t[0] : 1u), splat(GEN ? G.enc_t[1] : 0xffffu), splat(GEN ? G.enc_t[2] : 0u),
                         splat(GEN ? G.enc_t[3] : 0u)};

    bool pend = false, fitsA = true;
    uint64_t gA = 0, offA = 0;
    uint32_t TA = 0, startA = 0, nA = 0;
    WaveRef rA = {};

    auto place_header = [&](const WaveRef &r, uint64_t g, uint32_t n, uint64_t ex, uint64_t &pos) -> bool {
        const uint64_t mine = 1ull + n + (r.idx == 0 ? 1ull : 0ull);
        pos = ex + (r.idx == 0 ? 1ull : 0ull);
        if (lane == 0) {
            if (r.idx == 0) chunk_word_off[r.chunk] = ex;
            if (g + 1 == G.total_waves) {
                chunk_word_off[G.n_chunks] = ex + mine;
                st->total_words = ex + mine;
                if (G.host_words) *G.host_words = ex + mine;
                if (ex + mine > out_cap) atomicOr(&st->err, kErrCapacity);
            }
        }
        const bool room = pos + 1u + n <= out_cap;
        if (room && lane == 0) {
            out[pos] = n;
            if (r.idx == 0) out[pos - 1] = r.n_samples;
        }
        return room;
    };
    auto copy_out = [&](uint64_t ex) {
        uint64_t pos;
        const bool room = place_header(rA, gA, nA, ex + offA, pos);
        uint32_t *__restrict__ outp = out + pos + 1;
        typedef uint32_t u32x4s __attribute__((ext_vector_type(4)));
        typedef u32x4s __attribute__((address_space(1), aligned(4))) g_u32x4_a4;
        const uint32_t n4 = nA & ~3u;
        for (uint32_t i = 4u * (uint32_t)lane; i < n4; i += 256u) {
            uint32_t w = startA + i;
            w = w >= RING ? w - RING : w;
            const uint4 v = *reinterpret_cast<const uint4 *>(ring + w);
            if (room) *(g_u32x4_a4 *)(outp + i) = (u32x4s){v.x, v.y, v.z, v.w};
            *reinterpret_cast<uint4 *>(ring + w) = make_uint4(0, 0, 0, 0);
        }
        if ((uint32_t)lane < nA - n4) {
            uint32_t w = startA + n4 + (uint32_t)lane;
            w = w >= RING ? w - RING : w;
            if (room) outp[n4 + (uint32_t)lane] = ring[w];
            ring[w] = 0;
        }
        wave_sync();
        pend = false;
    };
    auto place_in_lds = [&](uint64_t &ex) -> bool {
        const uint32_t t = __hip_atomic_load((lds_u32 *)&shm.place_t[TA & 1u], __ATOMIC_RELAXED, __HIP_MEMORY_SCOPE_WORKGROUP);
        if (rfl(t) != TA + 1u) return false;
        ex = rfl64(__hip_atomic_load((lds_u64 *)&s_place_v[TA & 1u], __ATOMIC_RELAXED, __HIP_MEMORY_SCOPE_WORKGROUP));
        return true;
    };
    auto place_to_lds = [&](uint64_t ex) {
        if (lane == 0) {
            __hip_atomic_store((lds_u64 *)&s_place_v[TA & 1u], ex, __ATOMIC_RELAXED, __HIP_MEMORY_SCOPE_WORKGROUP);
            __hip_atomic_store((lds_u32 *)&shm.place_t[TA & 1u], TA + 1u, __ATOMIC_RELAXED, __HIP_MEMORY_SCOPE_WORKGROUP);
        }
    };
    auto wait_place = [&]() -> uint64_t {
        uint32_t spins = 0;
        for (;;) {
            uint64_t ex;
            bool have = place_in_lds(ex);
            if (!have) {
                uint64_t v = 0;
                if (lane == 0) v = es_load(place + TA);
                const uint32_t hi = (uint32_t)__builtin_amdgcn_readfirstlane((int)(uint32_t)(v >> 32));
                if (hi >> 31) {
                    ex = ((uint64_t)(hi & 0x7fffffffu) << 32) | (uint32_t)__builtin_amdgcn_readfirstlane((int)(uint32_t)v);
                    place_to_lds(ex);
                    have = true;
// ... 136 lines not shown
    __builtin_amdgcn_s_setprio(3);
    uint64_t pos = 0;
    uint64_t whdr = 1;
    uint64_t bits_in = 0;
    uint32_t idle = 0;
    const double rcp_tpw = 1.0 / (double)tpw;
    while (pos < total) {
        uint64_t v[kScPer];
        const uint64_t bs = pos;
#pragma unroll
        for (int j = 0; j < (int)kScPer; ++j) {
            const uint64_t e = bs + 64u * j + (uint32_t)lane;
            v[j] = e < total ? es_load(size + e) : 0ull;
        }
        uint64_t run = 0;
        bool open = true;
#pragma unroll
        for (int j = 0; j < (int)kScPer; ++j) {
            const uint64_t m = __ballot((v[j] >> 63) != 0);
            const uint32_t l = (m == ~0ull) ? 64u : (uint32_t)__builtin_ctzll(~m);
            run += open ? l : 0u;
            open = open && l == 64u;
        }
        const uint64_t end = bs + run;
        if (end <= pos) {
            if (++idle > (1u << 22)) {
                if (lane == 0) atomicOr(&st->err, kErrInternal);
                return;
            }
            __builtin_amdgcn_s_sleep(1);
            continue;
        }
        idle = 0;
#pragma unroll
        for (int j = 0; j < (int)kScPer; ++j) {
            if (bs + 64u * j < end) {
                const uint64_t e = bs + 64u * j + (uint32_t)lane;
                const bool in = e < end;
                const uint32_t val = in ? (uint32_t)(v[j] & 0xffffffffull) : 0u;
                const uint32_t e32 = (uint32_t)e;
                uint32_t g = (uint32_t)((double)e32 * rcp_tpw);
                uint32_t jj = e32 - g * tpw;
                if ((int32_t)jj < 0) { g -= 1u; jj += tpw; }
                if (jj >= tpw) { g += 1u; jj -= tpw; }
                const bool closing = in && jj + 1u == tpw;
                const uint32_t inc = wave_incl_scan_dpp(val), ex = inc - val;
                const int f = lane - (int)jj;
                const uint32_t exf = (uint32_t)__shfl((int)ex, f < 0 ? 0 : f);
                const uint64_t before = f < 0 ? bits_in + ex : (uint64_t)(ex - exf);
                const uint64_t nw = closing ? (before + val + 31ull) >> 5 : 0ull;
                const uint64_t contrib = closing ? 1ull + nw + (((g + 1u) % waves_per_chunk == 0u) ? 1ull : 0ull) : 0ull;
                uint64_t cinc;
                if (!__any(contrib >= (1ull << 24))) {
                    cinc = wave_incl_scan_dpp((uint32_t)contrib);
                } else {
                    cinc = contrib;
#pragma unroll
                    for (int d = 1; d < 64; d <<= 1) {
                        const uint64_t t = __shfl_up(cinc, d);
                        if (lane >= d) cinc += t;
                    }
                }
                const uint64_t my_whdr = whdr + cinc - contrib;
                if (in) {
                    es_store(place + 2u * e, kEsFlag | my_whdr);
                    es_store(place + 2u * e + 1u, kEsFlag | before);
                }
                const uint64_t left = end - (bs + 64u * j);
                const int li = __builtin_amdgcn_readfirstlane(left >= 64u ? 63 : (int)left - 1);
                const uint64_t wn = my_whdr + contrib, bn = closing ? 0ull : before + val;
                whdr = ((uint64_t)(uint32_t)__builtin_amdgcn_readlane((int)(uint32_t)(wn >> 32), li) << 32) | (uint32_t)__builtin_amdgcn_readlane((int)(uint32_t)wn, li);
                bits_in = ((uint64_t)(uint32_t)__builtin_amdgcn_readlane((int)(uint32_t)(bn >> 32), li) << 32) | (uint32_t)__builtin_amdgcn_readlane((int)(uint32_t)bn, li);
            }
        }
        pos = end;
    }
}

template <bool GEN, int WV, uint32_t RING>
__global__ __launch_bounds__(64 * WV, 4) void k_encode_stream_segs(Geom G, uint32_t seg_len, uint32_t tpw, const int16_t *__restrict__ in,
                                                                   uint32_t *__restrict__ out, uint64_t out_cap,
                                                                   uint64_t *__restrict__ chunk_word_off, uint32_t *__restrict__ wave_words,
                                                                   uint64_t *__restrict__ size, uint64_t *__restrict__ place,
                                                                   uint32_t *__restrict__ ctrl, DevStatus *st) {
    __shared__ __attribute__((aligned(16))) uint32_t ring_all[WV][kEsFront + RING + kEsBack];
    __shared__ EsShared<WV> shm;
    __shared__ uint64_t s_place_v[2][2];
    __shared__ uint32_t s_first[2][WV];
    typedef uint32_t __attribute__((address_space(3))) lds_u32;
    typedef uint64_t __attribute__((address_space(3))) lds_u64;
    static_assert((kEsFront + RING + kEsBack) % 4 == 0 && RING % 4 == 0, "16-byte LDS accesses");
    static_assert(WV == (int)kEsSegWaves, "es_seg_shape() counts tickets of kEsSegWaves segments");
    constexpr uint32_t kRowWords = kEsFront + RING + kEsBack;
    const int lane = lane_id(), wv = wave_id();
    uint32_t *row = ring_all[wv];
    uint32_t *ring = row + kEsFront;

    if (threadIdx.x == 0) {
        shm.role = atomicAdd(ctrl, 1u);
        shm.arrive = 0;
        shm.place_t[0] = shm.place_t[1] = 0;
    }
    zero_row(row, kRowWords, lane);
    __syncthreads();
    const uint64_t n_tickets = G.total_waves * tpw;
    if (rfl(shm.role) == 0) {
        es_scanner_segs(n_tickets, tpw, G.u_n_waves, size, place, st);
        return;
    }
    const uint32_t k = G.k;
    const u16x2 tp[4] = {splat(GEN ? G.enc_t[0] : 1u), splat(GEN ? G.enc_t[1] : 0xffffu), splat(GEN ? G.enc_t[2] : 0u),
                         splat(GEN ? G.enc_t[3] : 0u)};

    bool pend = false, fitsA = true, lastA = false, sibA = false;
    uint64_t gA = 0, offA = 0;
    uint32_t TA = 0, startA = 0, nA = 0, bitsA = 0, sbeginA = 0, sendA = 0, parA = 0;
    WaveRef rA = {};

    auto headers = [&](const WaveRef &r, const EsPlace2 &pl, uint64_t B) {
        if (lane != 0) return;
        if (sbeginA == 0u && r.idx == 0u) {
            chunk_word_off[r.chunk] = pl.whdr - 1u;
            if (pl.whdr - 1u < out_cap) out[pl.whdr - 1u] = r.n_samples;
        }
        if (lastA) {
            const uint64_t n = (B + bitsA + 31ull) >> 5;
            wave_words[gA] = (uint32_t)n;
            if (pl.whdr < out_cap) out[pl.whdr] = (uint32_t)n;
            if (gA + 1u == G.total_waves) {
                const uint64_t tot = pl.whdr + 1ull + n;
                chunk_word_off[G.n_chunks] = tot;
                st->total_words = tot;
                if (G.host_words) *G.host_words = tot;
                if (tot > out_cap) atomicOr(&st->err, kErrCapacity);
            }
        }
    };
    auto copy_out = [&](const EsPlace2 &pl) {
        const uint64_t B = pl.bits + offA;
        headers(rA, pl, B);
        const uint64_t w0 = pl.whdr + 1ull + (B >> 5);
        const uint32_t s = (uint32_t)B & 31u;
        const uint32_t i_lo = s ? 1u : 0u, i_hi = (s + bitsA + 31u) >> 5;
        const uint32_t nA4 = (nA + 3u) & ~3u, top = nA4 > i_hi ? nA4 : ((i_hi + 3u) & ~3u);
        if (sibA) {
            if (lane == 0) {
                const uint32_t F = s_first[parA][wv + 1], sh = bitsA & 31u;
                uint32_t wi = startA + (bitsA >> 5);
                wi = wi >= RING ? wi - RING : wi;
                ring[wi] |= F >> sh;
                if (sh) {
                    wi = wi + 1u >= RING ? wi + 1u - RING : wi + 1u;
                    ring[wi] |= F << (32u - sh);
                }
            }
            wave_sync();
        }
        uint32_t *__restrict__ outp = out + w0;
        const uint64_t room = out_cap > w0 ? out_cap - w0 : 0ull;
        typedef uint32_t u32x4s __attribute__((ext_vector_type(4)));
        typedef u32x4s __attribute__((address_space(1), aligned(4))) g_u32x4_a4;
        uint32_t carryw = 0;
        for (uint32_t i0 = 0; i0 < top; i0 += 256u) {
            const uint32_t i = i0 + 4u * (uint32_t)lane;
            uint4 v = make_uint4(0, 0, 0, 0);
            uint32_t w = startA + i;
            w = w >= RING ? w - RING : w;
            const bool inr = i < nA4;
            if (inr) v = *reinterpret_cast<const uint4 *>(ring + w);
            uint32_t pw = (uint32_t)__builtin_amdgcn_update_dpp(0, (int)v.w, 0x138, 0xf, 0xf, false);
            if (lane == 0) pw = carryw;
            carryw = (uint32_t)__builtin_amdgcn_readlane((int)v.w, 63);
            const uint32_t o0 = __builtin_amdgcn_alignbit(pw, v.x, s), o1 = __builtin_amdgcn_alignbit(v.x, v.y, s);
            const uint32_t o2 = __builtin_amdgcn_alignbit(v.y, v.z, s), o3 = __builtin_amdgcn_alignbit(v.z, v.w, s);
            if (i >= i_lo && i + 4u <= i_hi && (uint64_t)i + 4u <= room) {
                *(g_u32x4_a4 *)(outp + i) = (u32x4s){o0, o1, o2, o3};
            } else {
                if (i >= i_lo && i < i_hi && (uint64_t)i < room) outp[i] = o0;
                if (i + 1u >= i_lo && i + 1u < i_hi && (uint64_t)i + 1u < room) outp[i + 1u] = o1;
                if (i + 2u >= i_lo && i + 2u < i_hi && (uint64_t)i + 2u < room) outp[i + 2u] = o2;
                if (i + 3u >= i_lo && i + 3u < i_hi && (uint64_t)i + 3u < room) outp[i + 3u] = o3;
            }
            if (inr) *reinterpret_cast<uint4 *>(ring + w) = make_uint4(0, 0, 0, 0);
        }
        wave_sync();
        pend = false;
// ... 76 lines not shown
        const int16_t *x = in + r.sample_off + s_begin;

        auto gap = [&]() -> uint32_t { return es_gap<RING>(pend, startA, start, 12u); };
        if (pend && gap() < 512u) copy_out(wait_place());
        uint32_t limit = gap();

        uint64_t P = 0;
        uint32_t seg_bits = 0;
        bool first = true;
        bool fits = true;
        uint32_t carry = 0, carry2 = 0;
        if (s_begin) history_before<GEN>(x, carry, carry2);
        auto process_tile = [&](const uint32_t (&w)[4], int nv, int mark, auto full_tag) {
            constexpr bool FULLT = decltype(full_tag)::value;
            const TileCodes t = code_tile<GEN, FULLT>(w, nv, carry, carry2, tp, k);
            if (!FULLT && mark >= 0) seg_bits = (uint32_t)P + (mark ? (uint32_t)__builtin_amdgcn_readlane((int)t.incl, mark - 1) : 0u);
            const uint32_t need = ((uint32_t)P + t.tile_bits + 31u) >> 5;
            bool ok = fits && need < limit;
            if (pend && es_release(fits && !ok, P, place_in_lds, wait_place, copy_out)) {
                limit = gap();
                ok = fits && need < limit;
            }
            if (ok)
                ring_put<FULLT, RING>(t, row, start * 32u + (uint32_t)P, lane);
            else
                fits = false;
            P += t.tile_bits;
            if (first) {
                first = false;
                wave_sync();
                if (lane == 0) s_first[cyc & 1u][wv] = ring[start];
            }
        };
        const uint32_t n_fast = more ? slen / kTile : clen / kTile;
        uint64_t pollv = 0;
        bool polling = false;
        auto between = [&]() {
            if (!pend) return;
            if (polling) {
                polling = false;
                EsPlace2 pl;
                if (place_of(pollv, pl)) {
                    place_to_lds(pl);
                    return;
                }
            }
            pollv = 0;
            if (lane < 2) pollv = es_load(place + 2ull * TA + (uint32_t)lane);
            polling = true;
        };
        for_full_tiles(x, n_fast, lane, between, [&](const uint32_t (&w)[4]) { process_tile(w, 8, -1, std::true_type{}); });
        for (uint32_t t0 = n_fast * kTile; t0 < clen; t0 += kTile) {
            uint32_t w[4];
            const int nv = load8_dwords(x, clen, t0, lane, true, w);
            const int mark = (more && slen >= t0 && slen < t0 + (uint32_t)kTile) ? (int)((slen - t0) >> 3) : -1;
            process_tile(w, nv, mark, std::false_type{});
        }
        if (!more) seg_bits = (uint32_t)P;
        const uint32_t n = (uint32_t)((P + (sib ? 63u : 31u)) >> 5);
        wave_sync();
        if (lane == 0) shm.mine[cyc & 1u][wv] = seg_bits;
        if (pend) copy_out(wait_place());
        pend = true;
        fitsA = fits;
        gA = g;
        rA = r;
        TA = T;
        startA = start;
        nA = fits ? n : 0u;
        bitsA = seg_bits;
        sbeginA = s_begin;
        sendA = s_end;
        lastA = s_end == wlen;
        sibA = sib;
        parA = cyc & 1u;
        if (fits) {
            start += (n + 3u) & ~3u;
            start = start >= RING ? start - RING : start;
        }
    }
    if (pend) copy_out(wait_place());
}

hipError_t launch_encode_stream(const EncodeCall &c, uint64_t *d_scan) {
    const Geom &G = *c.G;
    const EncOut &o = c.out;
    const hipStream_t s = c.s;
    if (G.total_waves == 0) return hipSuccess;
    const uint64_t W = G.total_waves;
    const uint64_t tickets = (W + kEsWaves - 1) / kEsWaves;
    mark(c.ev, 0, s);
    hipError_t e = hipMemsetAsync(d_scan, 0, (2 * tickets + kEsCtrlWords) * sizeof(uint64_t), s);
    if (e != hipSuccess) return e;
    mark(c.ev, 1, s);
    mark(c.ev, 2, s);
    uint64_t *size = d_scan, *place = d_scan + tickets;
    uint32_t *ctrl = reinterpret_cast<uint32_t *>(d_scan + 2 * tickets);
    const unsigned grid = es_grid(G, tickets);
    if (G.n_taps)
        k_encode_stream<true, kEsWaves, kEsRing><<<grid, 64 * kEsWaves, 0, s>>>(G, c.d_in, o.d_out, o.out_cap, o.d_chunk_word_off, o.d_wave_words,
                                                                              size, place, ctrl, c.d_status);
    else
        k_encode_stream<false, kEsWaves, kEsRing><<<grid, 64 * kEsWaves, 0, s>>>(G, c.d_in, o.d_out, o.out_cap, o.d_chunk_word_off, o.d_wave_words,
                                                                               size, place, ctrl, c.d_status);
    mark(c.ev, 3, s);
    return hipGetLastError();
}

hipError_t launch_encode_stream_segs(const EncodeCall &c, uint32_t seg_target, uint64_t *d_scan) {
    const Geom &G = *c.G;
    const EncOut &o = c.out;
    const hipStream_t s = c.s;
    if (G.total_waves == 0) return hipSuccess;
    const EsSegShape sh = es_seg_shape(G.u_wave_len, seg_target);
    const uint64_t tickets = G.total_waves * sh.tpw;
    mark(c.ev, 0, s);
    hipError_t e = hipMemsetAsync(d_scan, 0, (3 * tickets + kEsCtrlWords) * sizeof(uint64_t), s);
    if (e != hipSuccess) return e;
    mark(c.ev, 1, s);
    mark(c.ev, 2, s);
    uint64_t *size = d_scan, *place = d_scan + tickets;
    uint32_t *ctrl = reinterpret_cast<uint32_t *>(d_scan + 3 * tickets);
    const unsigned grid = es_grid(G, tickets);
    if (G.n_taps)
        k_encode_stream_segs<true, kEsWaves, kEsRing><<<grid, 64 * kEsWaves, 0, s>>>(G, sh.seg_len, sh.tpw, c.d_in, o.d_out, o.out_cap, o.d_chunk_word_off,
                                                                                   o.d_wave_words, size, place, ctrl, c.d_status);
    else
        k_encode_stream_segs<false, kEsWaves, kEsRing><<<grid, 64 * kEsWaves, 0, s>>>(G, sh.seg_len, sh.tpw, c.d_in, o.d_out, o.out_cap, o.d_chunk_word_off,
                                                                                    o.d_wave_words, size, place, ctrl, c.d_status);
    mark(c.ev, 3, s);
    return hipGetLastError();
}

}
```

deltarice_amd/csrc/drx_internal.h:

```cpp
#ifndef DRX_INTERNAL_H
#define DRX_INTERNAL_H

#include <hip/hip_runtime.h>
#include <stdint.h>

#include <type_traits>
#include <vector>

#include "../../include/deltarice_hip.h"

namespace drx {

struct ChunkDesc {
    uint64_t sample_off;
    uint64_t wave_base;
    uint32_t n_samples;
    uint32_t wave_len;
    uint32_t n_waves;
    uint32_t pad_;
};

struct Geom {
    const ChunkDesc *chunks;
    uint64_t n_chunks;
    uint64_t total_waves;
    uint32_t uniform;
    uint32_t u_n_samples, u_wave_len, u_n_waves;
    uint32_t k;
    uint32_t n_taps;
    const int32_t *taps;
    uint32_t fast_taps, fast_t0neg;
    uint32_t fast_nt[3];
    uint32_t enc_fast;
    uint32_t enc_t[4];
    uint64_t total_samples;
    uint64_t *host_words;
    uint32_t dbg;
    const uint32_t *walk_short, *walk_long;
    uint32_t n_short, n_long, max_groups;
    uint64_t max_wave_len64;
    uint32_t rag_blocks, rag_blk_nt, rag_blk_slots;
    const uint32_t *rag_blk_list;
    uint32_t rag_blk_classes;
    uint32_t rag_blk_class_off[33], rag_blk_class_len[32];
    const uint32_t *iir_tab;
    const uint32_t *blk_iir_tab;
    const uint64_t *iir_chunk_tile_base;
    uint64_t iir_n_tiles;
    uint64_t *iir_state;
    const uint64_t *seg_unit_base;
    uint64_t seg_units;
    uint32_t rag_par, rag_bw_blocks_max;
    uint32_t rag_bw_min_len;
    uint32_t rag_pw_min_waves;
    const uint2 *rag_order;
    uint32_t rag_groups;
    uint32_t rag_groups_long;
    const uint32_t *pc_wg_base;
    uint32_t pc_super;
    uint32_t pc_packed;
};

struct DevStatus {
    uint32_t err;
    uint32_t listed;
    uint64_t total_words;
    uint32_t redone;
    uint32_t pad_;
};

constexpr uint32_t kErrCapacity = 1u;
constexpr uint32_t kErrCorrupt = 2u;
constexpr uint32_t kErrInternal = 4u;

struct StreamCall {
    const Geom *G;
    const uint32_t *d_in;
    uint64_t in_words;
    const uint64_t *d_chunk_word_off;
    uint64_t *d_wave_off;
    uint32_t *d_wave_words;
    bool tables_ready;
    void *d_pw;
    DevStatus *d_status;
    hipEvent_t *ev;
    hipStream_t s;
    StreamCall on(hipStream_t st) const { StreamCall c = *this; c.s = st; return c; }
    StreamCall view(const Geom &Gv) const { StreamCall c = *this; c.G = &Gv; return c; }
};
struct EncOut {
    uint32_t *d_out;
    uint64_t out_cap;
    uint64_t *d_chunk_word_off;
    uint32_t *d_wave_words;
};
struct EncodeCall {
    const Geom *G;
    const int16_t *d_in;
    EncOut out;
    DevStatus *d_status;
    hipEvent_t *ev;
    hipStream_t s;
};

hipError_t launch_encode(const EncodeCall &c, uint32_t *d_wave_rel, uint64_t *d_chunk_words);

__host__ __device__ inline bool long_waveform_batch(uint64_t total_waves, uint32_t wave_len) {
    return (wave_len >= 65536u && total_waves <= 16384u) || (wave_len >= 16384u && total_waves <= 4096u);
}
constexpr uint64_t kMaxWavefrontWaves = (1ull << 26) - 8u;
static inline unsigned blocks_for(uint64_t items, unsigned per_block) { return (unsigned)((items + per_block - 1) / per_block); }
static inline void mark(hipEvent_t *ev, int i, hipStream_t s) {
    if (ev) (void)hipEventRecord(ev[i], s);
}

inline uint64_t chunk_max_words(uint32_t n_samples, uint32_t n_waves) { return 1u + 2ull * n_waves + (((uint64_t)n_samples * 25u + 31u) >> 5); }

struct WalkRoute {
    bool chunk_wide, blocks;
    bool by_chains;
};
WalkRoute route_walk(const Geom &G, bool tables_ready, bool have_scratch);
std::vector<uint32_t> walk_plan_ragged(Geom &G, const ChunkDesc *host_chunks);
uint64_t walk_scratch_bytes(const Geom &G);
hipError_t walk_scratch_reset(const Geom &G, void *d_pw, hipStream_t s);
void launch_walk_chunk_wide(const StreamCall &c, bool by_chains);
void launch_walk_blocks(const StreamCall &c);
void launch_walk_serial(const StreamCall &c);
hipError_t launch_batch_walk(const StreamCall &c);
inline hipError_t batch_walk_prologue(const StreamCall &c) {
    mark(c.ev, 0, c.s);
    const hipError_t e = c.tables_ready ? hipSuccess : launch_batch_walk(c);
    if (e == hipSuccess) mark(c.ev, 1, c.s);
    return e;
}
template <class F> inline void for_wavefront_slices(const Geom &G, bool by_rag_order, F go) {
    constexpr uint64_t max_grid = 1ull << 25;
    const uint64_t n_wf = (by_rag_order && !G.uniform && G.rag_order) ? (uint64_t)G.rag_groups : (G.total_waves + 63u) / 64u;
    for (uint64_t base = 0; base < n_wf; base += max_grid) go(base, (unsigned)(n_wf - base < max_grid ? n_wf - base : max_grid));
}
hipError_t launch_sideband_tables(const StreamCall &c, const uint32_t *d_n, const uint32_t *d_list = nullptr,
                                  uint32_t n_list = 0);
int select_walk_class(uint32_t n_waves, uint32_t wave_len);
hipError_t launch_select_walk(const StreamCall &c, const uint32_t *d_lists, uint32_t n_sparse, uint32_t n_block, uint32_t n_chain,
                              uint32_t *d_fail);
hipError_t launch_decode_select(const StreamCall &c, const uint64_t *d_sel, uint64_t n_sel, int16_t *d_out, uint64_t stride);
uint64_t gather_scan_blocks(uint64_t n_sel);
struct GatherScratch {
    uint64_t *ent_pos, *block_sum;
    uint32_t *ent_words, *ctrl;
    uint64_t bytes;
};
inline GatherScratch gather_scratch_view(void *base, uint64_t n_sel) {
    GatherScratch t;
    t.ent_pos = (uint64_t *)base;
    t.block_sum = t.ent_pos + n_sel;
    t.ent_words = (uint32_t *)(t.block_sum + gather_scan_blocks(n_sel) + 2);
    t.ctrl = t.ent_words + n_sel;
    t.bytes = (n_sel + gather_scan_blocks(n_sel) + 2) * sizeof(uint64_t) + (n_sel + 1) * sizeof(uint32_t);
    return t;
}
hipError_t launch_gather(const StreamCall &c, const uint64_t *d_sel, uint64_t n_sel, uint64_t chunk_waves,
                         const uint32_t *d_chunk_samples, const EncOut &out, const GatherScratch &t, bool tiles, uint64_t mean_words,
                         bool resume);
struct BlkFormRule {
    double lane_us;
    uint32_t lanes_flag, all_fallback_flag;
    bool any_filter = false;
};
constexpr double kStatsLaneUs = 0.052;
constexpr BlkFormRule kStatsForm{kStatsLaneUs, DRX_DBG_STATS_LANES, DRX_DBG_STATS_ALL_FALLBACK};
constexpr double kPulsesLaneUs = 0.048;
constexpr BlkFormRule kPulsesForm{kPulsesLaneUs, DRX_DBG_PULSES_LANES, DRX_DBG_PULSES_ALL_FALLBACK};
constexpr double kWindowsLaneUs = 0.051;
constexpr BlkFormRule kWindowsForm{kWindowsLaneUs, DRX_DBG_WINDOWS_LANES, DRX_DBG_WINDOWS_ALL_FALLBACK};
constexpr double kTranscodeLaneUs = 0.2045;
constexpr double kTranscodeBlockFactor = 4.0;
constexpr BlkFormRule kTranscodeForm{kTranscodeLaneUs / kTranscodeBlockFactor, DRX_DBG_TRANSCODE_LANES, DRX_DBG_TRANSCODE_ALL_FALLBACK, true};
constexpr double kBinsLaneUs = 0.057;
constexpr double kBinsBlockFactor = 1.32;
constexpr BlkFormRule kBinsForm{kBinsLaneUs / kBinsBlockFactor, DRX_DBG_BINS_LANES, DRX_DBG_BINS_ALL_FALLBACK};
bool blocks_form_batch(const Geom &G, const void *d_blk, const BlkFormRule &r);
static_assert(DRX_STATS_FORM_LANES == DRX_PULSES_FORM_LANES && DRX_STATS_FORM_LANES == DRX_WINDOWS_FORM_LANES &&
                  DRX_STATS_FORM_BLOCKS == DRX_PULSES_FORM_BLOCKS && DRX_STATS_FORM_BLOCKS == DRX_WINDOWS_FORM_BLOCKS &&
                  DRX_STATS_FORM_FALLBACK_ALL == DRX_PULSES_FORM_FALLBACK_ALL && DRX_STATS_FORM_FALLBACK_ALL == DRX_WINDOWS_FORM_FALLBACK_ALL &&
                  DRX_STATS_FORM_LANES == DRX_TRANSCODE_FORM_LANES && DRX_STATS_FORM_BLOCKS == DRX_TRANSCODE_FORM_BLOCKS &&
                  DRX_STATS_FORM_FALLBACK_ALL == DRX_TRANSCODE_FORM_FALLBACK_ALL && DRX_STATS_FORM_LANES == DRX_BINS_FORM_LANES &&
                  DRX_STATS_FORM_BLOCKS == DRX_BINS_FORM_BLOCKS && DRX_STATS_FORM_FALLBACK_ALL == DRX_BINS_FORM_FALLBACK_ALL,
              "blocks_form_word() serves the five calls");
uint32_t blocks_form_word(const Geom &G, bool blocks, const BlkFormRule &r);
struct BlkFallbackList {
    uint32_t *n_listed, *listed;
    static constexpr uint64_t bytes(uint64_t W) { return 8u + 4u * W; }
    static BlkFallbackList at(void *base) { return {reinterpret_cast<uint32_t *>(base), reinterpret_cast<uint32_t *>(base) + 2}; }
};
hipError_t launch_wave_stats(const StreamCall &c, void *d_blk, void *d_sacc, uint32_t head_len, int64_t *d_out, uint32_t *form_out);
uint64_t stats_blocks_scratch_bytes(const Geom &G);
hipError_t launch_stats_blocks(const StreamCall &c, void *d_blk, void *d_sacc, uint32_t head_len, int64_t *d_out, BlkFallbackList *list_out);
hipError_t launch_wave_bins(const StreamCall &c, void *d_blk, void *d_list, int bins_impl, const int64_t *d_start, uint64_t start_stride,
                            int64_t offset, uint32_t bin, uint32_t n_bins, int64_t *d_out, uint64_t out_wave_stride, uint32_t *form_out);
uint64_t bins_blocks_scratch_bytes(const Geom &G);
hipError_t launch_bins_blocks(const StreamCall &c, void *d_blk, void *d_list, const int64_t *d_start, uint64_t start_stride, int64_t offset,
                              uint32_t bin, uint32_t n_bins, int64_t *d_out, uint64_t out_wave_stride);
hipError_t launch_decode_window(const StreamCall &c, const int64_t *d_start, uint64_t start_stride, int64_t offset, uint32_t width,
                                int16_t pad, int16_t *d_out, uint64_t out_stride);
inline uint64_t stack_list_bytes(const Geom &G) { return 8u * (G.total_waves + 1u); }
hipError_t launch_wave_stack(const StreamCall &c, void *d_list, uint32_t max_wgs, const int64_t *d_start, uint64_t start_stride, int64_t offset, uint32_t width,
                             const uint8_t *d_select, int64_t *d_out, uint64_t out_stride);
struct WinList;
hipError_t launch_decode_windows(const StreamCall &c, void *d_blk, void *d_wtab, const int64_t *d_start, uint64_t start_wave_stride,
                                 uint64_t start_win_stride, const uint32_t *d_count, uint32_t n_win, int64_t offset, uint32_t width,
                                 int16_t pad, int16_t *d_out, uint64_t out_wave_stride, uint64_t out_win_stride, uint32_t *form_out);
uint64_t windows_blocks_scratch_bytes(const Geom &G);
hipError_t launch_windows_blocks(const StreamCall &c, void *d_blk, void *d_wtab, const WinList &wl, BlkFallbackList *list_out);
hipError_t launch_find_pulses(const StreamCall &c, void *d_blk, void *d_ptab, void *d_pstage, const int64_t *d_thr, uint64_t thr_stride,
                              int64_t thr, bool neg, uint32_t min_width, uint32_t max_pulses, uint32_t *d_count, int64_t *d_out,
                              uint32_t *form_out);
uint64_t pulses_blocks_scratch_bytes(const Geom &G);
uint64_t pulses_blocks_staging_bytes(const Geom &G, uint32_t max_pulses);
hipError_t launch_pulses_blocks(const StreamCall &c, void *d_blk, void *d_ptab, void *d_pstage, const int64_t *d_thr, uint64_t thr_stride,
                                int64_t thr, bool neg, uint32_t min_width, uint32_t max_pulses, uint32_t *d_count, int64_t *d_out,
                                BlkFallbackList *list_out);
hipError_t launch_estimate_words(const Geom &G, const int16_t *d_in, unsigned long long *d_words16, hipStream_t s);
hipError_t launch_chunk_offsets(const Geom &G, const uint32_t *d_wave_words, uint32_t *d_wave_rel, uint64_t *d_chunk_words,
                                uint64_t *d_chunk_word_off, uint64_t out_cap, DevStatus *d_status, hipStream_t s);
struct TrcScratch {
    uint64_t *chunk_words;
    unsigned long long *est;
    uint32_t *words, *rel;
    uint64_t bytes;
};
inline TrcScratch trc_scratch_view(const Geom &G, void *base) {
    const uint64_t W = G.total_waves ? G.total_waves : 1, C = G.n_chunks + 1;
    TrcScratch t;
    t.chunk_words = (uint64_t *)base;
    t.est = (unsigned long long *)(t.chunk_words + C);
    t.words = (uint32_t *)(t.est + 16);
    t.rel = t.words + W;
    t.bytes = (C + 16) * sizeof(uint64_t) + 2 * W * sizeof(uint32_t);
    return t;
}
hipError_t launch_transcode(const StreamCall &c, uint32_t k2, const TrcScratch &t, const EncOut &out, void *d_blk, void *d_tb, uint32_t *form_out);
hipError_t launch_estimate_words_encoded(const StreamCall &c, unsigned long long *d_est, void *d_blk, void *d_tb, uint32_t *form_out);
uint64_t trc_blocks_scratch_bytes(const Geom &G);
hipError_t launch_trc_blocks_sizes(const StreamCall &c, void *d_blk, void *d_tb, uint32_t k2, const TrcScratch &t, uint32_t *d_out_wave_words,
                                   unsigned long long *d_est, BlkFallbackList *list_out);
hipError_t launch_trc_blocks_pack(const StreamCall &c, void *d_blk, void *d_tb, uint32_t k2, const TrcScratch &t, const EncOut &out);
struct RefilterTarget {
    uint32_t n_taps;
    const int32_t *taps;
};
hipError_t launch_refilter(const StreamCall &c, uint32_t k2, const RefilterTarget &T, const TrcScratch &t, const EncOut &out, uint32_t *form_out);
hipError_t launch_estimate_words_refiltered(const StreamCall &c, const RefilterTarget &T, unsigned long long *d_est, uint32_t *form_out);

hipError_t launch_encode_fused(const EncodeCall &c, int wide, uint64_t *d_scan);

constexpr uint32_t kEsRingWords = 2496;
constexpr uint64_t kEsMinUnits = 8192;
hipError_t launch_encode_stream(const EncodeCall &c, uint64_t *d_scan);

constexpr uint32_t kEsSegWaves = 4;
constexpr uint32_t kEsSegMinLen = 1024, kEsSegMaxLen = 7168;
struct EsSegShape { uint32_t seg_len, nseg, tpw; };
__host__ __device__ inline EsSegShape es_seg_shape(uint32_t L, uint32_t seg_target) {
    EsSegShape sh;
    uint32_t n = (L + seg_target - 1u) / seg_target;
    n = n ? n : 1u;
    const uint32_t dn = n / kEsSegWaves * kEsSegWaves, up = (n + kEsSegWaves - 1u) / kEsSegWaves * kEsSegWaves;
    n = up;
    if (dn && dn != up) {
        const uint64_t sd = (L + dn - 1u) / dn, su = (L + up - 1u) / up;
        const uint64_t pen_dn = sd > seg_target ? (sd - seg_target) * 55u : 0u, pen_up = su < seg_target ? (seg_target - su) * 40u : 0u;
        if (sd * 57u <= (uint64_t)seg_target * 67u && pen_dn < pen_up) n = dn;
    }
    sh.seg_len = (((L + n - 1u) / n) + 7u) & ~7u;
    sh.nseg = (L + sh.seg_len - 1u) / sh.seg_len;
    sh.tpw = (sh.nseg + kEsSegWaves - 1u) / kEsSegWaves;
    return sh;
}
inline bool stream_segs_admits(const Geom &G) { return G.uniform && (G.n_taps == 0 || G.enc_fast) && G.u_wave_len >= 64u &&
                                                       G.total_waves * es_seg_shape(G.u_wave_len, kEsSegMinLen).tpw < 0xffff0000ull; }
constexpr uint32_t kEsSegsFromLen = 20480;
inline uint64_t segs_scan_words(const Geom &G, uint32_t seg_target) { return 3 * G.total_waves * es_seg_shape(G.u_wave_len, seg_target).tpw + 192; }
hipError_t launch_encode_stream_segs(const EncodeCall &c, uint32_t seg_target, uint64_t *d_scan);

bool long_batch_admits(const Geom &G);
bool long_batch(const Geom &G);
uint64_t long_batch_units(const Geom &G);
std::vector<uint64_t> segments_plan_ragged(Geom &G, const ChunkDesc *host_chunks);
hipError_t launch_encode_long(const EncodeCall &c, uint32_t *d_wave_rel, uint64_t *d_chunk_words, uint32_t *d_seg_bits,
                              uint64_t *d_seg_pos);

struct SideStream {
    hipStream_t s;
    hipEvent_t fork, join;
};
hipError_t launch_decode(const StreamCall &c, int16_t *d_out, uint64_t *d_granules, int impl, void *d_blk, const SideStream *side,
                         uint32_t *path_out = nullptr);
bool blocks_batch(const Geom &G, double lane_us = 0.06, bool any_filter = false);
std::vector<uint32_t> blocks_plan_ragged(Geom &G, const ChunkDesc *host_chunks);
uint64_t blocks_scratch_bytes(const Geom &G);
uint64_t blocks_total_slots(const Geom &G);
hipError_t launch_decode_blocks(const StreamCall &c, void *d_blk, int16_t *d_out, const uint32_t **fail_out,
                                const uint32_t **suspect_out, bool resid, bool *fused_out);
constexpr uint32_t kBlkMaxClasses = 32;
struct BlkTables {
    uint32_t *fail, *suspect, *ends;
    uint64_t *state;
};
struct BlkClassLaunch {
    uint32_t *info;
    const uint32_t *list;
    uint32_t n_waves;
    int nt, sw;
    uint32_t spw, run_len;
    unsigned grid;
};
template <class F> inline void blk_dispatch(int nt, int sw, F f) {
    auto by_sw = [&](auto nt_tag) {
        switch (sw) {
            case 9: f(nt_tag, std::integral_constant<int, 9>{}); break;
            case 11: f(nt_tag, std::integral_constant<int, 11>{}); break;
            case 15: f(nt_tag, std::integral_constant<int, 15>{}); break;
            default: f(nt_tag, std::integral_constant<int, 19>{}); break;
        }
    };
    if (nt == 64) by_sw(std::integral_constant<int, 64>{});
    else if (nt == 128) by_sw(std::integral_constant<int, 128>{});
    else by_sw(std::integral_constant<int, 256>{});
}
hipError_t blocks_prepare(const Geom &G, uint64_t in_words, const uint32_t *d_wave_words, void *d_blk, hipStream_t s, BlkTables *T,
                          BlkClassLaunch *launches, uint32_t *n_launches);
uint32_t blocks_iir_tab_words();
void blocks_iir_tables(const uint32_t fast_nt[3], uint32_t t0neg, uint32_t *tab);
constexpr uint32_t kPcWaves = 8;
constexpr uint32_t kPcRunSamples = 7168;
constexpr uint32_t kPcMaxRun = 16;
constexpr uint32_t kPcSegSamples = 8192;
constexpr uint32_t kPcWholeLen = 10240;
constexpr uint32_t kPcMinLen = 64;
__host__ __device__ inline uint32_t pc_seg_samples(uint32_t k) {
    if (k <= 3u) return kPcSegSamples;
    const uint32_t s = (131072u / (2u * k + 9u)) & ~511u;
    return s < 512u ? 512u : s;
}
__host__ __device__ inline uint32_t pc_run_samples(uint32_t k) { return k <= 3u ? kPcRunSamples : pc_seg_samples(k) - 512u; }
__host__ __device__ inline uint32_t pc_whole_len(uint32_t k) { return k <= 3u ? kPcWholeLen : 65536u / (k + 4u); }
__host__ __device__ inline uint32_t pc_max_len(uint32_t k) { return pc_seg_samples(k) * kPcWaves; }
struct PieceShape {
    uint32_t run;
    uint32_t segs;
    uint32_t parts;
    uint32_t seg_len;
    uint32_t pieces;
    uint32_t wgs;
};
__host__ __device__ inline bool piece_packable(uint32_t L) { return L >= 8u && L < 512u && (L & 7u) == 0u; }
__host__ __device__ inline PieceShape piece_shape(uint32_t L, uint32_t W, uint32_t k, bool packed) {
    PieceShape s;
    s.parts = 1u;
    const uint32_t run_samples = pc_run_samples(k), seg_samples = pc_seg_samples(k), max_len = pc_max_len(k);
    if (packed) {
        const uint32_t bits = k <= 3u ? 9u : k + 6u;
        uint32_t by_samples = run_samples / L, by_words = 2000u / (1u + (bits * L + 31u) / 32u);
        by_samples = by_samples ? by_samples : 1u;
        by_words = by_words ? by_words : 1u;
        s.run = by_samples < by_words ? by_samples : by_words;
// ... 54 lines not shown
```

deltarice_amd/csrc/drx_walk.hip:

```cpp
#include <hip/hip_runtime.h>
#include <stdint.h>

#include <algorithm>
#include <type_traits>

#include "drx_internal.h"
#include "drx_device.h"
#include "drx_walk.h"

namespace drx {

__global__ __launch_bounds__(64) void k_walk_block(Geom G, const uint32_t *__restrict__ in, uint64_t in_words,
                                                   const uint64_t *__restrict__ chunk_word_off,
                                                   const uint32_t *__restrict__ chunk_list, uint32_t n_list,
                                                   uint64_t *__restrict__ wave_off, uint32_t *__restrict__ wave_words,
                                                   DevStatus *st) {
    __shared__ __attribute__((aligned(16))) uint32_t blk[kWalkBlockWords];
    __shared__ __attribute__((aligned(8))) uint2 hop[kWalkHopCap];
    if (blockIdx.x >= n_list) return;
    const uint64_t c = chunk_list ? chunk_list[blockIdx.x] : blockIdx.x;
    walk_chunk_block<kChasePad>(G, c, in, in_words, chunk_word_off, wave_off, wave_words, nullptr, st, blk, hop);
}

__global__ __launch_bounds__(64) void k_walk_block_only(Geom G, const uint32_t *__restrict__ in, uint64_t in_words,
// ... 151 lines not shown
    bool ok = chunk_extent_usable(begin, end, in_words, kParWalkMaxWords);
    if (ok && in[begin] != f.N) ok = false;
    if (!ok) { if (tid == 0) fail[c] = 1u; return; }
    const uint32_t len_w = (uint32_t)(end - begin);
    const uint32_t nc = cand_count[c];
    if (nc > kPwCap - 2u || nc < W) { if (tid == 0) fail[c] = 1u; return; }
    if (tid < 64u) {
        uint32_t run = 0;
        for (uint32_t s0 = 0; s0 < parts; s0 += 64u) {
            const uint32_t sl = s0 + tid;
            uint2 e = make_uint2(0u, 0u);
            if (sl < parts) e = cand[c * kPwStride + kPwCap + sl];
            const uint32_t incl = wave_running_prefix(e.y, run);
            if (sl < parts) { s_first[sl] = e.x; s_pre[sl + 1u] = incl; }
        }
        if (tid == 0) s_pre[0] = 0;
    }
    __syncthreads();
    if (s_pre[parts] != nc) { if (tid == 0) fail[c] = 1u; return; }
    uint32_t n_pad = 64u;
    while (n_pad < nc + 2u) n_pad <<= 1;
    for (uint32_t i = tid; i < n_pad; i += kPwThreads) {
        uint2 e = make_uint2(0xffffffffu, 0u);
        if (i < nc) {
            const uint32_t sl = slot_of(s_pre, parts, i);
            e = cand[c * kPwStride + s_first[sl] + (i - s_pre[sl])];
        }
        pos[i] = e.x;
        val[i] = e.y;
    }
    __syncthreads();
    const uint32_t END = nc, INV = nc + 1u;
    for (uint32_t i = tid; i < n_pad; i += kPwThreads) {
        uint32_t to = i;
        if (i < nc) {
            const uint64_t target = (uint64_t)pos[i] + val[i] + 1u;
            if (target == len_w) {
                to = END;
            } else if (target > len_w) {
                to = INV;
            } else {
                uint32_t lo = 0, hi = nc;
                while (lo < hi) { const uint32_t mid = (lo + hi) >> 1; if (pos[mid] < (uint32_t)target) lo = mid + 1u; else hi = mid; }
                to = (lo < nc && pos[lo] == (uint32_t)target) ? lo : INV;
            }
            if (pos[i] == 1u) s_start = i;
        }
        up[0][i] = (uint16_t)to;
    }
    __syncthreads();
    for (int k = 1; k < kPwLevels; ++k) {
        for (uint32_t i = tid; i < n_pad; i += kPwThreads) up[k][i] = up[k - 1][up[k - 1][i]];
        __syncthreads();
    }
    const uint32_t start = s_start;
    if (start == 0xffffffffu) { if (tid == 0) fail[c] = 1u; return; }
    bool bad = false;
    for (uint32_t w = tid; w < W; w += kPwThreads) {
        uint32_t node = start;
#pragma unroll
        for (int k = 0; k < kPwLevels; ++k)
            if ((w >> k) & 1u) node = up[k][node];
        if (node >= nc) { bad = true; continue; }
        const uint32_t n = val[node];
        if (!hb.ok(n, w + 1u == W)) { bad = true; continue; }
        if (w + 1u == W && up[0][node] != END) { bad = true; continue; }
        wave_off[f.base + w] = begin + pos[node];
        wave_words[f.base + w] = n;
    }
    if (bad) atomicOr(&s_bad, 1u);
    __syncthreads();
    if (tid == 0 && s_bad) fail[c] = 1u;
}

constexpr int kSwThreads = 1024;
constexpr uint32_t kSwSegs = 64;
constexpr uint32_t kSwCap = 192;
constexpr uint64_t kSwMaxChunks = 1u << 20;
constexpr uint32_t kSwMinWaves = 8, kSwMaxWaves = 8192;

__global__ __launch_bounds__(kSwThreads) void k_walk_sparse(Geom G, const uint32_t *__restrict__ in, uint64_t in_words,
                                                            const uint64_t *__restrict__ chunk_word_off,
                                                            uint64_t *__restrict__ wave_off, uint32_t *__restrict__ wave_words,
                                                            uint32_t *__restrict__ fail, const uint32_t *__restrict__ list) {
    __shared__ uint32_t s_a[kSwSegs + 1];
    __shared__ uint32_t s_cnt[kSwSegs], s_base[kSwSegs + 1];
    __shared__ uint32_t s_list[kSwSegs][kSwCap];
    __shared__ uint32_t s_bad;
    const uint32_t tid = threadIdx.x;
    const int lane = lane_id();
    const uint32_t wv = (uint32_t)wave_id();
    const uint64_t c = list ? (uint64_t)list[blockIdx.x] : blockIdx.x;
    const ChunkGeom f = chunk_geom(G, c);
    const uint32_t W = f.W;
    const uint64_t begin = chunk_word_off[c];
    const uint64_t end = chunk_word_off[c + 1];
    if (tid == 0) s_bad = 0;
    bool ok = chunk_extent_usable(begin, end, in_words, kParWalkMaxWords);
    if (ok && in[begin] != f.N) ok = false;
    if (!ok) { if (tid == 0) fail[c] = 1u; return; }
    const uint32_t len_w = (uint32_t)(end - begin);
    const HeaderBounds hb = header_bounds(f.L, f.N, W, G.k);
    const uint32_t min_full = hb.min_full, max_full = hb.max_full, min_last = hb.min_last, max_last = hb.max_last;
    const uint32_t lo_any = min_full < min_last ? min_full : min_last, hi_any = max_full > max_last ? max_full : max_last;
    uint32_t S = W / 8u;
    S = S > kSwSegs ? kSwSegs : (S < 1u ? 1u : S);
    if (len_w / W > 8192u) S = 1u;
    const uint32_t *cw = in + begin;
    if (tid == 0) { s_a[0] = 1u; s_a[S] = len_w; }
    __syncthreads();
    auto plausible = [&](uint32_t v, uint32_t i) { return v >= lo_any && v <= hi_any && (uint64_t)i + 1u + v <= len_w; };
    for (uint32_t sg = 1u + wv; sg < S; sg += blockDim.x >> 6) {
        uint32_t from = 1u + (uint32_t)(((uint64_t)(len_w - 1u) * sg) / S);
        const uint32_t stop = (uint64_t)from + 2u * (hi_any + 2u) < len_w ? from + 2u * (hi_any + 2u) : len_w;
        uint32_t found = len_w;
        for (uint32_t tries = 0; tries < 64u; ++tries) {
            constexpr uint32_t U = 8;
            found = len_w;
            for (uint32_t j0 = from; j0 < stop && found == len_w; j0 += 64u * U) {
                uint32_t v[U];
#pragma unroll
                for (uint32_t u = 0; u < U; ++u) {
                    const uint32_t i = j0 + 64u * u + (uint32_t)lane;
                    v[u] = i < len_w ? cw[i] : 0xffffffffu;
                }
#pragma unroll
                for (uint32_t u = 0; u < U; ++u) {
                    const uint64_t m = __ballot(plausible(v[u], j0 + 64u * u + (uint32_t)lane));
                    if (m && found == len_w) found = j0 + 64u * u + (uint32_t)__builtin_ctzll(m);
                }
            }
            if (found >= stop) {
                if (stop < len_w && lane == 0) atomicOr(&s_bad, 1u);
                found = len_w;
                break;
            }
            const uint32_t nxt = found + 1u + rfl(cw[found]);
            if (nxt == len_w || plausible(rfl(cw[nxt]), nxt)) break;
            from = found + 1u;
            found = len_w;
        }
        if (lane == 0) s_a[sg] = found;
    }
    __syncthreads();
    if (tid < S) {
        uint32_t pos = s_a[tid];
        const uint32_t target = s_a[tid + 1u];
        uint32_t cnt = 0;
        bool bad = false;
        while (pos < target) {
            const uint32_t n = cw[pos];
            if (n < lo_any || n > hi_any || cnt >= kSwCap) { bad = true; break; }
            s_list[tid][cnt] = pos;
            ++cnt;
            pos += n + 1u;
        }
        if (pos != target) bad = true;
        s_cnt[tid] = cnt;
        if (bad) atomicOr(&s_bad, 1u);
    }
    __syncthreads();
    if (tid < 64u) {
        const uint32_t cnt = tid < S ? s_cnt[tid] : 0u;
        const uint32_t incl = wave_incl_scan_dpp(cnt);
        s_base[tid] = incl - cnt;
        if (tid == 63u) s_base[64] = incl;
    }
    __syncthreads();
    if (s_bad || s_base[64] != W) { if (tid == 0) fail[c] = 1u; return; }
    bool bad = false;
    for (uint32_t sg = wv; sg < S; sg += blockDim.x >> 6) {
        const uint32_t cnt = rfl(s_cnt[sg]), b0 = rfl(s_base[sg]);
        for (uint32_t i = (uint32_t)lane; i < cnt; i += 64u) {
            const uint32_t at = s_list[sg][i];
            const uint32_t n = (i + 1u < cnt ? s_list[sg][i + 1u] : s_a[sg + 1u]) - at - 1u;
            const uint32_t w = b0 + i;
            if (!hb.ok(n, w + 1u == W)) bad = true;
            wave_off[f.base + w] = begin + at;
            wave_words[f.base + w] = n;
        }
    }
    if (bad) atomicOr(&s_bad, 1u);
    __syncthreads();
    if (tid == 0 && s_bad) fail[c] = 1u;
}

constexpr uint32_t kBwTries = 6;
constexpr uint32_t kBwCandCap = 512;
constexpr uint32_t kBwMaxList = 256;

struct BwBlock { uint32_t entry, count, exit, base; };

template <uint32_t B>
__device__ __forceinline__ void bw_block_prefix(const uint64_t *__restrict__ chunk_word_off, uint64_t in_words,
                                                const uint32_t *__restrict__ list, uint32_t n_list, uint32_t blocks_max,
                                                uint32_t *pre, int lane) {
    uint32_t run = 0;
    for (uint32_t s0 = 0; s0 < n_list; s0 += 64u) {
        const uint32_t sl = s0 + (uint32_t)lane;
        uint32_t nb = 0;
        if (sl < n_list) {
            const uint64_t c = list ? (uint64_t)list[sl] : sl;
            const uint64_t begin = chunk_word_off[c], end = chunk_word_off[c + 1];
            if (chunk_extent_usable(begin, end, in_words, kParWalkMaxWords)) nb = (uint32_t)((end - begin + B - 1u) / B);
            if (nb > blocks_max) nb = blocks_max;
        }
        const uint32_t incl = wave_running_prefix(nb, run);
        if (sl < n_list) pre[sl + 1u] = incl;
    }
    if (lane == 0) pre[0] = 0;
    wave_sync();
}

struct BwUnit {
    bool ok;
    uint64_t begin;
    ChunkGeom f;
    uint32_t b, b0, len_w, blk_len;
};
template <uint32_t B, class Body>
__device__ __forceinline__ void bw_stream_blocks(const Geom &G, const uint32_t *__restrict__ in, uint64_t in_words,
                                                 const uint64_t *__restrict__ chunk_word_off, const uint32_t *__restrict__ list,
                                                 uint32_t n_list, uint32_t blocks_max, const uint32_t *__restrict__ fail,
                                                 uint32_t *blk, uint32_t *pre, Body body) {
    constexpr int NV = B / 256;
    const int lane = lane_id();
    bw_block_prefix<B>(chunk_word_off, in_words, list, n_list, blocks_max, pre, lane);
    const uint32_t total = pre[n_list];
    uint32_t cached_slot = 0xffffffffu;
    BwUnit cached{};
    auto locate_unit = [&](uint32_t unit) __attribute__((always_inline)) {
        const uint32_t slot = slot_of(pre, n_list, unit);
        if (slot != cached_slot) {
            cached_slot = slot;
            const uint64_t cc = list ? (uint64_t)list[slot] : slot;
            cached.f = chunk_geom(G, cc);
            cached.begin = chunk_word_off[cc];
            cached.len_w = (uint32_t)(chunk_word_off[cc + 1] - cached.begin);
            cached.ok = !(fail && fail[cc]);
        }
        BwUnit u = cached;
        u.b = unit - pre[slot];
        u.b0 = u.b * B;
        if (u.b0 >= u.len_w) u.ok = false;
        u.blk_len = u.ok ? (u.len_w - u.b0 < B ? u.len_w - u.b0 : B) : 0u;
        return u;
    };
    const int64_t a_max = (int64_t)in_words - 4;
    auto fetch = [&](const BwUnit &u, uint4 (&v)[NV]) __attribute__((always_inline)) {
        const int64_t a0 = (int64_t)(u.begin + u.b0);
#pragma unroll
        for (int j = 0; j < NV; ++j) {
            const int64_t a = a0 + (int64_t)((uint32_t)(j * 64 + lane) * 4u);
            const int64_t ac = a > a_max ? (a_max < 0 ? 0 : a_max) : a;
            v[j] = *reinterpret_cast<const uint4 *>(in + ac);
        }
    };
    auto store = [&](const BwUnit &u, const uint4 (&v)[NV]) __attribute__((always_inline)) {
        const uint64_t a0 = u.begin + u.b0;
#pragma unroll
        for (int j = 0; j < NV; ++j) {
            const uint32_t i = (uint32_t)(j * 64 + lane) * 4u;
            uint4 w = v[j];
            if ((int64_t)(a0 + i) > a_max) {
                auto ld = [&](uint64_t q) { return q < in_words ? in[q] : 0xffffffffu; };
                w = make_uint4(ld(a0 + i), ld(a0 + i + 1u), ld(a0 + i + 2u), ld(a0 + i + 3u));
            }
// ... 286 lines not shown
}


static bool chunk_wide_walk_takes(uint32_t n_waves, uint32_t wave_len) {
    return wave_len > kWalkShortLen && n_waves >= kSwMinWaves && n_waves <= kSwMaxWaves;
}

int select_walk_class(uint32_t n_waves, uint32_t wave_len) {
    if (wave_len <= kWalkShortLen) return 1;
    return chunk_wide_walk_takes(n_waves, wave_len) ? 0 : 2;
}

static bool bw_walk_pays(uint64_t walked_chunks, uint32_t n_waves, uint32_t wave_len) {
    return walked_chunks <= n_waves / (wave_len <= kWalkShortLen ? 35u : 18u) && wave_len >= 16u;
}
constexpr uint64_t kBwMaxBlocks = 0xfffffu;
static uint64_t bw_chunk_blocks(uint32_t n_samples, uint32_t n_waves) {
    return (chunk_max_words(n_samples, n_waves) + kWalkBlockWords - 1u) / kWalkBlockWords;
}
static uint32_t bw_walk_blocks_max(const Geom &G) {
    if (!(G.uniform && bw_walk_pays(G.n_chunks, G.u_n_waves, G.u_wave_len) && G.n_chunks <= kPwMaxChunks && G.u_wave_len <= 5000u &&
          !chunk_wide_walk_takes(G.u_n_waves, G.u_wave_len))) return 0;
    const uint64_t nb = bw_chunk_blocks(G.u_n_samples, G.u_n_waves);
    return nb > kBwMaxBlocks ? 0u : (uint32_t)nb;
}

static uint32_t pw_parts(uint32_t n_chunks) { return n_chunks <= 4u ? 128u : (n_chunks <= 32u ? 32u : 16u); }

static uint32_t bw_hop_cap(uint32_t B, uint32_t min_len, uint32_t k) {
    const uint32_t mw = min_payload_words(min_len, k);
    if (mw < 32u || B > 4096u) return 0u;
    return B / (mw + 1u) + 2u;
}

struct ParWalks {
    bool pw, bw;
    const uint32_t *pw_list, *bw_list;
    uint32_t n_pw, n_bw;
    uint32_t bw_blocks_max;
    uint32_t bw_B, bw_waves_per_cu, bw_hop_cap;
    uint2 *cand;
    uint32_t *cnt, *pw_fail, *bw_fail;
    BwBlock *info;
    uint32_t *hops;
    uint64_t bytes;
};
static ParWalks par_walks(const Geom &G, void *base) {
    ParWalks P{};
    if (G.uniform) {
        P.bw_blocks_max = bw_walk_blocks_max(G);
        P.bw = P.bw_blocks_max != 0;
        P.pw = G.n_chunks <= kSwMaxChunks && chunk_wide_walk_takes(G.u_n_waves, G.u_wave_len);
        P.n_pw = P.n_bw = (uint32_t)G.n_chunks;
    } else if (G.rag_par) {
        P.pw = G.n_long != 0;
        P.bw = G.n_short != 0;
        P.pw_list = G.walk_long;
        P.bw_list = G.walk_short;
        P.n_pw = G.n_long;
        P.n_bw = G.n_short;
        P.bw_blocks_max = G.rag_bw_blocks_max;
    }
    if (!P.pw && !P.bw) return P;
    const uint32_t max_full = max_payload_words(G.uniform ? G.u_wave_len : kWalkShortLen);
    P.bw_B = max_full + 2u <= 1024u ? 1024u : (max_full + 2u <= 2048u ? 2048u : 4096u);
    P.bw_waves_per_cu = P.bw_B == 1024u ? 24u : (P.bw_B == 2048u ? 13u : 7u);
    P.bw_hop_cap = bw_hop_cap(P.bw_B, G.uniform ? G.u_wave_len : G.rag_bw_min_len, G.k);
    auto take = [&](uint64_t bytes) {
        char *p = base ? (char *)base + P.bytes : nullptr;
        P.bytes += bytes;
        return p;
    };
    const uint64_t n = G.n_chunks, bw_units = P.bw ? (uint64_t)P.n_bw * P.bw_blocks_max : 0;
    P.cand = (uint2 *)take(P.pw && n <= kPwMaxChunks ? n * kPwStride * sizeof(uint2) : 0);
    P.cnt = (uint32_t *)take(n * sizeof(uint32_t));
    P.pw_fail = (uint32_t *)take(n * sizeof(uint32_t));
    P.bw_fail = (uint32_t *)take((n + (n & 1u)) * sizeof(uint32_t));
    P.info = (BwBlock *)take(bw_units * (kWalkBlockWords / 1024u) * sizeof(BwBlock));
    P.hops = (uint32_t *)take(bw_units * (kWalkBlockWords / P.bw_B) * P.bw_hop_cap * sizeof(uint32_t));
    if (!P.bw_hop_cap) P.hops = nullptr;
    return P;
}
uint64_t walk_scratch_bytes(const Geom &G) { return par_walks(G, nullptr).bytes; }
hipError_t walk_scratch_reset(const Geom &G, void *d_pw, hipStream_t s) {
    return hipMemsetAsync(par_walks(G, d_pw).cnt, 0, 3u * G.n_chunks * sizeof(uint32_t), s);
}

std::vector<uint32_t> walk_plan_ragged(Geom &G, const ChunkDesc *d) {
    const uint64_t n = G.n_chunks;
    std::vector<uint32_t> lists;
    for (uint64_t c = 0; c < n; ++c) if (d[c].wave_len <= kWalkShortLen) lists.push_back((uint32_t)c);
    G.n_short = (uint32_t)lists.size();
    for (uint64_t c = 0; c < n; ++c) if (d[c].wave_len > kWalkShortLen) lists.push_back((uint32_t)c);
    G.n_long = (uint32_t)lists.size() - G.n_short;
    bool ok = G.n_long <= kPwMaxChunks && G.n_short <= kPwMaxChunks;
    uint64_t bmax = 0;
    uint32_t min_len = 0xffffffffu, min_long_waves = 0xffffffffu;
    for (uint64_t c = 0; c < n && ok; ++c) {
        if (d[c].wave_len > kWalkShortLen) {
            ok = d[c].n_waves <= kPwMaxWaves;
            min_long_waves = std::min(min_long_waves, d[c].n_waves);
        } else {
            ok = bw_walk_pays(G.n_short, d[c].n_waves, d[c].wave_len);
            bmax = std::max(bmax, bw_chunk_blocks(d[c].n_samples, d[c].n_waves));
            min_len = std::min(min_len, d[c].wave_len);
        }
    }
    G.rag_par = ok && bmax <= kBwMaxBlocks;
    G.rag_bw_blocks_max = (uint32_t)bmax;
    G.rag_bw_min_len = min_len;
    G.rag_pw_min_waves = min_long_waves;
    return lists;
}

WalkRoute route_walk(const Geom &G, bool tables_ready, bool have_scratch) {
    WalkRoute R{};
    if (tables_ready || !have_scratch || (G.dbg & DRX_DBG_NO_PARALLEL_WALKS)) return R;
    const ParWalks P = par_walks(G, nullptr);
    R.chunk_wide = P.pw;
    R.blocks = P.bw;
    const bool few_waves = G.uniform && (G.u_n_waves < 64u || G.u_n_waves > kPwMaxWaves);
    const bool chains_suit = (G.dbg & DRX_DBG_WALK_BY_CHAINS) || few_waves || ((G.uniform ? G.n_chunks : G.n_long) > 4u && (G.uniform || G.rag_pw_min_waves >= 64u));
    R.by_chains = (!(G.dbg & DRX_DBG_WALK_BY_SCAN) && chains_suit) || G.n_chunks > kPwMaxChunks || few_waves;
    return R;
}

hipError_t launch_sideband_tables(const StreamCall &c, const uint32_t *d_n, const uint32_t *d_list, uint32_t n_list) {
    const Geom &G = *c.G;
    if (G.total_waves == 0 || (d_list && !n_list)) return hipSuccess;
    k_sideband_tables<<<d_list ? n_list : (unsigned)G.n_chunks, 256, 0, c.s>>>(G, c.d_in, c.in_words, c.d_chunk_word_off, d_n, c.d_wave_off,
                                                                            c.d_wave_words, c.d_status, d_list);
    return hipGetLastError();
}

static void walk_chunk_wide(const StreamCall &c, const uint32_t *d_list, uint32_t n, unsigned chain_threads, uint2 *cand, uint32_t *cnt,
                            uint32_t *fail) {
    const Geom &G = *c.G;
    if (chain_threads) {
        k_walk_sparse<<<n, chain_threads, 0, c.s>>>(G, c.d_in, c.in_words, c.d_chunk_word_off, c.d_wave_off, c.d_wave_words, fail, d_list);
    } else {
        const uint32_t parts = pw_parts(n);
        k_pw_scan<<<(unsigned)(n * parts), 256, 0, c.s>>>(G, c.d_in, c.in_words, c.d_chunk_word_off, d_list, cand, cnt, parts);
        k_walk_parallel<<<n, kPwThreads, 0, c.s>>>(G, c.d_in, c.in_words, c.d_chunk_word_off, c.d_wave_off, c.d_wave_words, fail, d_list, cand, cnt, parts);
    }
    k_walk_scalar_only<<<blocks_for(G.n_chunks, kWalkChains), 64, 0, c.s>>>(G, c.d_in, c.in_words, c.d_chunk_word_off, c.d_wave_off,
                                                                            c.d_wave_words, c.d_status, fail);
}
void launch_walk_chunk_wide(const StreamCall &c, bool by_chains) {
    const Geom &G = *c.G;
    const ParWalks P = par_walks(G, c.d_pw);
    const unsigned chain_threads = (G.uniform && G.u_n_waves < 256u) ? 256u : (unsigned)kSwThreads;
    walk_chunk_wide(c, P.pw_list, P.n_pw, by_chains ? chain_threads : 0u, P.cand, P.cnt, P.pw_fail);
}

void launch_walk_blocks(const StreamCall &c) {
    const Geom &G = *c.G;
    const ParWalks P = par_walks(G, c.d_pw);
    const uint32_t *list = P.bw_list;
    const uint32_t n = P.n_bw;
    auto run_bw = [&](auto btag) {
        constexpr uint32_t B = decltype(btag)::value;
        const uint32_t bmax = P.bw_blocks_max * (kWalkBlockWords / B);
        const unsigned grid = 256u * P.bw_waves_per_cu;
        if (P.hops)
            k_bw_blocks<B, true><<<grid, 64, 0, c.s>>>(G, c.d_in, c.in_words, c.d_chunk_word_off, list, n, bmax, P.info, P.hops, P.bw_hop_cap);
        else
            k_bw_blocks<B, false><<<grid, 64, 0, c.s>>>(G, c.d_in, c.in_words, c.d_chunk_word_off, list, n, bmax, P.info, P.hops, P.bw_hop_cap);
        k_bw_scan<B><<<n, 64, 0, c.s>>>(G, c.d_in, c.in_words, c.d_chunk_word_off, list, n, bmax, P.info, P.bw_fail);
        if (P.hops)
            k_bw_emit<B><<<256u * 8u, 256, 0, c.s>>>(G, c.in_words, c.d_chunk_word_off, list, n, bmax, P.info, P.bw_fail, P.hops, P.bw_hop_cap, c.d_wave_off, c.d_wave_words, c.d_status);
        else
            k_bw_chase<B><<<grid, 64, 0, c.s>>>(G, c.d_in, c.in_words, c.d_chunk_word_off, list, n, bmax, P.info, P.bw_fail, c.d_wave_off, c.d_wave_words, c.d_status);
    };
    if (P.bw_B == 1024u) run_bw(std::integral_constant<uint32_t, 1024>{});
    else if (P.bw_B == 2048u) run_bw(std::integral_constant<uint32_t, 2048>{});
    else run_bw(std::integral_constant<uint32_t, 4096>{});
    k_walk_block_only<<<(unsigned)G.n_chunks, 64, 0, c.s>>>(G, c.d_in, c.in_words, c.d_chunk_word_off, c.d_wave_off, c.d_wave_words, c.d_status, P.bw_fail);
}

static void walk_serial(const StreamCall &c, const uint32_t *d_short, uint32_t n_short, const uint32_t *d_long, uint32_t n_long) {
    const Geom &G = *c.G;
    if (n_short)
        k_walk_block<<<n_short, 64, 0, c.s>>>(G, c.d_in, c.in_words, c.d_chunk_word_off, d_short, n_short, c.d_wave_off, c.d_wave_words, c.d_status);
    if (n_long && d_long)
        k_walk_list<<<blocks_for(n_long, 64), 64, 0, c.s>>>(G, c.d_in, c.in_words, c.d_chunk_word_off, d_long, n_long, c.d_wave_off, c.d_wave_words, c.d_status);
    else if (n_long)
        k_walk_scalar<<<blocks_for(G.n_chunks, kWalkChains), 64, 0, c.s>>>(G, c.d_in, c.in_words, c.d_chunk_word_off, c.d_wave_off, c.d_wave_words, c.d_status);
}
void launch_walk_serial(const StreamCall &c) {
    const Geom &G = *c.G;
    if (!G.uniform) return walk_serial(c, G.walk_short, G.n_short, G.walk_long, G.n_long);
    const uint32_t n = (uint32_t)G.n_chunks, n_short = G.u_wave_len <= kWalkShortLen ? n : 0u;
    walk_serial(c, nullptr, n_short, nullptr, n - n_short);
}

hipError_t launch_batch_walk(const StreamCall &c) {
    const WalkRoute R = route_walk(*c.G, false, c.d_pw != nullptr);
    if (R.chunk_wide || R.blocks) {
        const hipError_t e = walk_scratch_reset(*c.G, c.d_pw, c.s);
        if (e != hipSuccess) return e;
        if (R.chunk_wide) launch_walk_chunk_wide(c, R.by_chains);
        if (R.blocks) launch_walk_blocks(c);
    } else {
        launch_walk_serial(c);
    }
    return hipGetLastError();
}

hipError_t launch_select_walk(const StreamCall &c, const uint32_t *d_lists, uint32_t n_sparse, uint32_t n_block, uint32_t n_chain,
                              uint32_t *d_fail) {
    if (n_sparse) {
        const hipError_t e = hipMemsetAsync(d_fail, 0, c.G->n_chunks * sizeof(uint32_t), c.s);
        if (e != hipSuccess) return e;
        walk_chunk_wide(c, d_lists, n_sparse, kSwThreads, nullptr, nullptr, d_fail);
    }
    walk_serial(c, d_lists + n_sparse, n_block, d_lists + n_sparse + n_block, n_chain);
    return hipGetLastError();
}

}
```

include/deltarice_hip.h:

```cpp
#ifndef DELTARICE_HIP_H
#define DELTARICE_HIP_H

#include <stddef.h>
#include <stdint.h>

#ifdef __cplusplus
extern "C" {
#endif

#define DRX_FILTER_ID 32025
#define DRX_MAX_TAPS 64

typedef struct drx_ctx drx_ctx;
typedef struct drx_plan drx_plan;

typedef enum {
    DRX_OK = 0,
    DRX_ERR_ARG = 1,
    DRX_ERR_DEVICE = 2,
    DRX_ERR_CAPACITY = 3,
    DRX_ERR_CORRUPT = 4,
    DRX_ERR_UNSUPPORTED = 5,
    DRX_ERR_NOMEM = 6
} drx_status;
// ... 123 lines not shown
drx_status drx_decode_windows_with_wave_words(drx_plan *plan, const uint32_t *d_in, uint64_t in_words,
                                              const uint64_t *d_chunk_word_off, const uint32_t *d_wave_words, const int64_t *d_start,
                                              uint64_t start_wave_stride, uint64_t start_win_stride, const uint32_t *d_count,
                                              uint32_t n_win, int64_t offset, uint32_t width, int16_t pad, int16_t *d_out,
                                              uint64_t out_wave_stride, uint64_t out_win_stride);

#define DRX_PULSE_START 0
#define DRX_PULSE_WIDTH 1
#define DRX_PULSE_PEAK 2
#define DRX_PULSE_ARGPEAK 3
#define DRX_PULSE_SUM 4
#define DRX_PULSE_COLS 5
drx_status drx_find_pulses(drx_plan *plan, const uint32_t *d_in, uint64_t in_words, const uint64_t *d_chunk_word_off,
                           const int64_t *d_thr, uint64_t thr_stride, int64_t thr, int32_t polarity, uint32_t min_width,
                           uint32_t max_pulses, uint32_t *d_count, int64_t *d_out);
#define DRX_PULSES_FORM_LANES 1u
#define DRX_PULSES_FORM_BLOCKS 2u
#define DRX_PULSES_FORM_FALLBACK_ALL 4u
uint32_t drx_plan_last_pulses_form(const drx_plan *plan);
#define DRX_PULSES_STAGE_CAP 8u
uint32_t drx_plan_last_pulses_listed(const drx_plan *plan);
uint32_t drx_plan_last_pulses_redone(const drx_plan *plan);
drx_status drx_find_pulses_with_wave_words(drx_plan *plan, const uint32_t *d_in, uint64_t in_words,
                                           const uint64_t *d_chunk_word_off, const uint32_t *d_wave_words, const int64_t *d_thr,
                                           uint64_t thr_stride, int64_t thr, int32_t polarity, uint32_t min_width,
                                           uint32_t max_pulses, uint32_t *d_count, int64_t *d_out);

drx_status drx_transcode(drx_plan *plan, const uint32_t *d_in, uint64_t in_words, const uint64_t *d_chunk_word_off,
                         uint32_t new_rice_k, uint32_t *d_out, uint64_t out_cap_words, uint64_t *d_out_chunk_word_off,
                         uint32_t *d_out_wave_words);
drx_status drx_transcode_with_wave_words(drx_plan *plan, const uint32_t *d_in, uint64_t in_words, const uint64_t *d_chunk_word_off,
                                         const uint32_t *d_wave_words, uint32_t new_rice_k, uint32_t *d_out, uint64_t out_cap_words,
                                         uint64_t *d_out_chunk_word_off, uint32_t *d_out_wave_words);
drx_status drx_transcode_filter(drx_plan *plan, const uint32_t *d_in, uint64_t in_words, const uint64_t *d_chunk_word_off,
                                uint32_t new_rice_k, uint32_t new_n_taps, const int32_t *new_taps, uint32_t *d_out,
                                uint64_t out_cap_words, uint64_t *d_out_chunk_word_off, uint32_t *d_out_wave_words);
drx_status drx_transcode_filter_with_wave_words(drx_plan *plan, const uint32_t *d_in, uint64_t in_words,
                                                const uint64_t *d_chunk_word_off, const uint32_t *d_wave_words, uint32_t new_rice_k,
                                                uint32_t new_n_taps, const int32_t *new_taps, uint32_t *d_out, uint64_t out_cap_words,
                                                uint64_t *d_out_chunk_word_off, uint32_t *d_out_wave_words);
#define DRX_TRANSCODE_FORM_LANES 1u
#define DRX_TRANSCODE_FORM_BLOCKS 2u
#define DRX_TRANSCODE_FORM_FALLBACK_ALL 4u
#define DRX_TRANSCODE_FORM_REFILTER 8u
#define DRX_TRANSCODE_FORM_REFILTER_SERIAL 16u
uint32_t drx_plan_last_transcode_form(const drx_plan *plan);
uint32_t drx_plan_last_transcode_listed(const drx_plan *plan);
drx_status drx_estimate_words_encoded(drx_plan *plan, const uint32_t *d_in, uint64_t in_words, const uint64_t *d_chunk_word_off,
                                      const uint32_t *d_wave_words, uint64_t words_out[16]);
drx_status drx_estimate_words_encoded_filter(drx_plan *plan, const uint32_t *d_in, uint64_t in_words, const uint64_t *d_chunk_word_off,
                                             const uint32_t *d_wave_words, uint32_t new_n_taps, const int32_t *new_taps,
                                             uint64_t words_out[16]);

drx_status drx_estimate_words(drx_plan *plan, const int16_t *d_in, uint64_t words_out[16]);

drx_status drx_plan_finish(drx_plan *plan, uint64_t *total_words);

const uint32_t *drx_plan_wave_words(const drx_plan *plan);
const uint64_t *drx_plan_wave_word_off(const drx_plan *plan);
#define DRX_PATH_LANES_FUSED 1u
#define DRX_PATH_LANES 2u
#define DRX_PATH_BLOCKS 4u
#define DRX_PATH_LONG 8u
#define DRX_PATH_SIMPLE 16u
#define DRX_PATH_IIR 32u
#define DRX_PATH_IIR_FUSED 64u
#define DRX_PATH_SELECT 128u
#define DRX_PATH_GATHER 256u
#define DRX_PATH_STATS 512u
#define DRX_PATH_TRANSCODE 1024u
#define DRX_PATH_WINDOW 2048u
#define DRX_PATH_PULSES 4096u
#define DRX_PATH_WINDOWS 8192u
#define DRX_PATH_BINS 16384u
#define DRX_PATH_STACK 32768u
uint32_t drx_plan_last_decode_path(const drx_plan *plan);
#define DRX_ENC_TWO_PASS 1u
#define DRX_ENC_SEGMENTS 2u
#define DRX_ENC_FUSED 3u
#define DRX_ENC_PIECES 4u
#define DRX_ENC_STREAM 5u
#define DRX_ENC_STREAM_SEGS 6u
uint32_t drx_plan_last_encode_path(const drx_plan *plan);
drx_status drx_plan_read_wave_words(drx_plan *plan, uint32_t *host_out);

drx_status drx_filter_chunk_host(drx_ctx *ctx, int reverse, size_t cd_nelmts,
                                 const unsigned *cd_values, const void *in, size_t nbytes,
                                 void **out, size_t *out_bytes);

drx_status drx_plan_last_timings(drx_plan *plan, float ms[4]);

#define DRX_DBG_BINS_LANES 64u
#define DRX_DBG_BINS_ALL_FALLBACK 128u
#define DRX_DBG_NO_LONG_PATHS 256u
#define DRX_DBG_LONG_NOT_BLOCKS 512u
#define DRX_DBG_TRANSCODE_LANES 1024u
#define DRX_DBG_NO_PARALLEL_WALKS 2048u
#define DRX_DBG_NO_PIECES 4096u
#define DRX_DBG_FORCE_SEGMENTS 8192u
#define DRX_DBG_TRANSCODE_ALL_FALLBACK 16384u
#define DRX_DBG_FORCE_PIECES 32768u
#define DRX_DBG_NO_WIDE_FUSED 65536u
#define DRX_DBG_RAGGED_ONE_LANES_LAUNCH 131072u
#define DRX_DBG_STREAM_THREE_WGS 262144u
#define DRX_DBG_FORCE_STREAM 524288u
#define DRX_DBG_REFILTER_SERIAL 1048576u
#define DRX_DBG_IIR_SEPARATE 2097152u
#define DRX_DBG_FORCE_STREAM_SEGS 4194304u
#define DRX_DBG_WALK_BY_SCAN 8388608u
#define DRX_DBG_WALK_BY_CHAINS 16777216u
#define DRX_DBG_GATHER_OTHER_COPY 33554432u
#define DRX_DBG_STATS_LANES 67108864u
#define DRX_DBG_STATS_ALL_FALLBACK 134217728u
#define DRX_DBG_PULSES_LANES 268435456u
#define DRX_DBG_PULSES_ALL_FALLBACK 536870912u
#define DRX_DBG_WINDOWS_LANES 1073741824u
#define DRX_DBG_WINDOWS_ALL_FALLBACK 2147483648u
drx_status drx_ctx_set_option(drx_ctx *ctx, const char *key, int64_t value);

#ifdef __cplusplus
}
#endif
#endif
```

Baseline: 1560 GB/s.

## Hand off zeroed status and scan buffers between calls to skip memsets

```diff
diff --git a/deltarice_amd/_lib.py b/deltarice_amd/_lib.py
--- a/deltarice_amd/_lib.py
+++ b/deltarice_amd/_lib.py
@@ -103,6 +103,8 @@
     "drx_plan_wave_word_off": (_vp, [_vp]),
     "drx_plan_last_decode_path": (C.c_uint32, [_vp]),
     "drx_plan_last_encode_path": (C.c_uint32, [_vp]),
+    "drx_plan_last_launch_count": (C.c_uint32, [_vp]),
+    "drx_plan_last_serial_walks": (C.c_uint32, [_vp]),
     "drx_plan_last_stats_form": (C.c_uint32, [_vp]),
     "drx_plan_last_pulses_form": (C.c_uint32, [_vp]),
     "drx_plan_last_windows_form": (C.c_uint32, [_vp]),
diff --git a/deltarice_amd/codec.py b/deltarice_amd/codec.py
--- a/deltarice_amd/codec.py
+++ b/deltarice_amd/codec.py
@@ -711,6 +711,12 @@
     def last_encode_path(self) -> int:
         return int(self.ctx.lib.drx_plan_last_encode_path(self._h))
 
+    def last_launch_count(self) -> int:
+        return int(self.ctx.lib.drx_plan_last_launch_count(self._h))
+
+    def last_serial_walks(self) -> int:
+        return int(self.ctx.lib.drx_plan_last_serial_walks(self._h))
+
     def wave_words(self) -> np.ndarray:
         buf = np.empty(self.total_waves, dtype=np.uint32)
         self.ctx._check(self.ctx.lib.drx_plan_read_wave_words(self._h, buf.ctypes.data_as(C.POINTER(C.c_uint32))))
diff --git a/deltarice_amd/csrc/drx_api.h b/deltarice_amd/csrc/drx_api.h
--- a/deltarice_amd/csrc/drx_api.h
+++ b/deltarice_amd/csrc/drx_api.h
@@ -127,8 +127,20 @@
     drx::DevStatus *d_status = nullptr;
     drx::DevStatus *h_status = nullptr;
     bool last_was_encode = false;
+    struct Handover {
+        drx::DevStatus *status[2] = {nullptr, nullptr};
+        bool status_zero[2] = {false, false};
+        int status_cur = 0;
+        bool scan_zero[2] = {false, false};
+        uint64_t scan_zero_words[2] = {0, 0};
+        int scan_other = -1;
+        uint64_t scan_other_words = 0;
+        drx::CallTally tally;
+        uint32_t last_launches = 0;
+    } hand;
     struct Encoders {
         Grown scan;
+        Grown scan_alt;
         uint32_t *d_seg_bits = nullptr;
         uint64_t *d_seg_pos = nullptr;
         uint64_t *d_pc_scan = nullptr;
@@ -155,7 +167,6 @@
     void *stack_list = nullptr;
     struct Selection {
         Grown h, d;
-        uint32_t *d_fail = nullptr;
         hipEvent_t copied = nullptr;
     } sel;
     struct Gather {
diff --git a/deltarice_amd/csrc/drx_api_encode.hip b/deltarice_amd/csrc/drx_api_encode.hip
--- a/deltarice_amd/csrc/drx_api_encode.hip
+++ b/deltarice_amd/csrc/drx_api_encode.hip
@@ -45,9 +45,29 @@
 
 static drx_status route_scratch(drx_plan *p, const EncodeRoute &R) {
     drx_ctx *ctx = p->ctx;
-    if (R.enc == DRX_ENC_STREAM_SEGS)
+    if (R.enc == DRX_ENC_STREAM_SEGS) {
+        const void *had = p->enc.scan.ptr;
         DRX_HIP(ctx, p->mem.reserve(p->enc.scan, segs_scan_words(p->G, R.seg_target) * sizeof(uint64_t), 4, false, Buffers::KeepOld, ctx->stream));
+        if (p->enc.scan.ptr != had) p->hand.scan_zero[0] = false;
+    }
     if (R.enc == DRX_ENC_SEGMENTS) DRX_HIP(ctx, seg_scratch(p));
+    return DRX_OK;
+}
+
+static drx_status stream_scan(drx_plan *p, uint64_t words, EsScan *sc) {
+    drx_ctx *ctx = p->ctx;
+    drx_plan::Encoders &E = p->enc;
+    drx_plan::Handover &H = p->hand;
+    const void *had = E.scan_alt.ptr;
+    DRX_HIP(ctx, p->mem.reserve(E.scan_alt, E.scan.cap, 0, false, Buffers::KeepOld, ctx->stream));
+    if (E.scan_alt.ptr != had) H.scan_zero[1] = false;
+    auto zero = [&](int i) { return H.scan_zero[i] && H.scan_zero_words[i] >= words; };
+    const int use = zero(0) ? 0 : (zero(1) ? 1 : -1), cur = use < 0 ? 0 : use;
+    uint64_t *inst[2] = {(uint64_t *)E.scan.ptr, (uint64_t *)E.scan_alt.ptr};
+    *sc = EsScan{inst[cur], use >= 0, inst[cur ^ 1]};
+    H.scan_zero[0] = H.scan_zero[1] = false;
+    H.scan_other = cur ^ 1;
+    H.scan_other_words = words;
     return DRX_OK;
 }
 
@@ -63,17 +83,28 @@
     const EncodeRoute R = route_encode(p, ctx->encode_impl, ctx->debug_flags);
     if (const drx_status st = route_scratch(p, R)) return st;
     const EncodeCall c{&p->G, d_in, EncOut{d_out, out_cap_words, d_chunk_word_off, p->d_wave_words}, p->d_status,
-                       ctx->profile ? p->prof.ev : nullptr, ctx->stream};
+                       ctx->profile ? p->prof.ev : nullptr, ctx->stream, p->hand.status[p->hand.status_cur ^ 1], &p->hand.tally};
     const drx_plan::Encoders &E = p->enc;
     uint64_t *d_scan = (uint64_t *)E.scan.ptr;
+    EsScan sc{};
     switch (R.enc) {
-    case DRX_ENC_STREAM_SEGS: DRX_HIP(ctx, launch_encode_stream_segs(c, R.seg_target, d_scan)); break;
+    case DRX_ENC_STREAM_SEGS:
+        if (const drx_status st = stream_scan(p, stream_segs_scan_words(p->G, R.seg_target), &sc)) return st;
+        DRX_HIP(ctx, launch_encode_stream_segs(c, R.seg_target, sc));
+        break;
     case DRX_ENC_PIECES: DRX_HIP(ctx, launch_encode_pieces(c, p->G.total_samples, E.d_pc_scan, E.pc_wgs)); break;
     case DRX_ENC_SEGMENTS: DRX_HIP(ctx, launch_encode_long(c, p->d_wave_rel, p->d_chunk_words, E.d_seg_bits, E.d_seg_pos)); break;
-    case DRX_ENC_STREAM: DRX_HIP(ctx, launch_encode_stream(c, d_scan)); break;
-    case DRX_ENC_FUSED: DRX_HIP(ctx, launch_encode_fused(c, R.wide, d_scan)); break;
+    case DRX_ENC_STREAM:
+        if (const drx_status st = stream_scan(p, stream_scan_words(p->G), &sc)) return st;
+        DRX_HIP(ctx, launch_encode_stream(c, sc));
+        break;
+    case DRX_ENC_FUSED:
+        p->hand.scan_zero[0] = false;
+        DRX_HIP(ctx, launch_encode_fused(c, R.wide, d_scan));
+        break;
     default: DRX_HIP(ctx, launch_encode(c, p->d_wave_rel, p->d_chunk_words));
     }
+    if (R.enc != DRX_ENC_STREAM && R.enc != DRX_ENC_STREAM_SEGS && R.enc != DRX_ENC_FUSED) p->hand.tally.counted = false;
     return call_end(p, R.enc,  true);
 }
 
@@ -82,6 +113,7 @@
     drx_ctx *ctx = p->ctx;
     DRX_ON_DEVICE(ctx);
     DRX_HIP(ctx, hipStreamSynchronize(ctx->stream));
+    p->hand.scan_zero[0] = false;
     DRX_HIP(ctx, launch_estimate_words(p->G, d_in, (unsigned long long *)p->enc.scan.ptr, ctx->stream));
     DRX_HIP(ctx, hipMemcpyAsync(words_out, p->enc.scan.ptr, 16 * sizeof(uint64_t), hipMemcpyDeviceToHost, ctx->stream));
     DRX_HIP(ctx, hipStreamSynchronize(ctx->stream));
diff --git a/deltarice_amd/csrc/drx_api_plan.hip b/deltarice_amd/csrc/drx_api_plan.hip
--- a/deltarice_amd/csrc/drx_api_plan.hip
+++ b/deltarice_amd/csrc/drx_api_plan.hip
@@ -22,8 +22,19 @@
 
 drx_status drx::call_begin(drx_plan *p) {
     drx_ctx *ctx = p->ctx;
+    drx_plan::Handover &H = p->hand;
     p->gat.last.valid = false;
-    DRX_HIP(ctx, hipMemsetAsync(p->d_status, 0, sizeof(DevStatus), ctx->stream));
+    H.tally = CallTally{};
+    H.last_launches = 0;
+    H.scan_other = -1;
+    if (H.status_zero[H.status_cur ^ 1]) {
+        H.status_cur ^= 1;
+    } else {
+        DRX_HIP(ctx, hipMemsetAsync(H.status[H.status_cur], 0, sizeof(DevStatus), ctx->stream));
+        H.tally.add();
+    }
+    H.status_zero[0] = H.status_zero[1] = false;
+    p->d_status = H.status[H.status_cur];
     p->G.dbg = ctx->debug_flags;
     return DRX_OK;
 }
@@ -32,7 +43,7 @@
     drx_ctx *ctx = p->ctx;
     if (const drx_status st = call_begin(p)) return st;
     *c = StreamCall{&p->G, d_in, in_words, d_chunk_word_off, p->d_wave_off, p->d_wave_words, tables_ready || d_sideband, p->dec.d_pw,
-                    p->d_status, ctx->profile ? p->prof.ev : nullptr, ctx->stream};
+                    p->d_status, ctx->profile ? p->prof.ev : nullptr, ctx->stream, p->hand.status[p->hand.status_cur ^ 1], &p->hand.tally};
     if (d_sideband)
         DRX_HIP(ctx, launch_sideband_tables(*c, d_sideband));
     return DRX_OK;
@@ -41,6 +52,14 @@
     (encode ? p->enc.last_path : p->dec.last_path) = path;
     p->prof.valid = p->ctx->profile != 0;
     p->last_was_encode = encode;
+    drx_plan::Handover &H = p->hand;
+    H.status_zero[H.status_cur ^ 1] = H.tally.status_handed;
+    if (H.tally.scan_handed && H.scan_other >= 0) {
+        H.scan_zero[H.scan_other] = true;
+        H.scan_zero_words[H.scan_other] = H.scan_other_words;
+    }
+    const bool counts = encode || !(path & ~(uint32_t)(DRX_PATH_LANES_FUSED | DRX_PATH_LANES | DRX_PATH_LONG | DRX_PATH_SIMPLE));
+    H.last_launches = (counts && H.tally.counted) ? H.tally.launches : 0u;
     return DRX_OK;
 }
 drx_status drx::stream_call_args(drx_plan *p, const char *who, bool have_pointers, const uint32_t *d_sideband, bool sideband) {
@@ -92,8 +111,10 @@
     uint64_t words = 2 * W + 192;
     if (stream_segs_admits(G) && G.u_wave_len >= kEsSegsFromLen) words = std::max(words, segs_scan_words(G, kEsSegMinLen));
     DRX_HIP(ctx, p->mem.reserve(p->enc.scan, words * sizeof(uint64_t), 0, false, Buffers::KeepOld, ctx->stream));
-    DRX_HIP(ctx, p->mem.alloc(&p->d_status, sizeof(DevStatus)));
-    DRX_HIP(ctx, hipMemset(p->d_status, 0, sizeof(DevStatus)));
+    DRX_HIP(ctx, p->mem.alloc(&p->hand.status[0], 2 * sizeof(DevStatus)));
+    DRX_HIP(ctx, hipMemset(p->hand.status[0], 0, 2 * sizeof(DevStatus)));
+    p->hand.status[1] = p->hand.status[0] + 1;
+    p->d_status = p->hand.status[0];
     DRX_HIP(ctx, p->mem.alloc(&p->h_status, sizeof(DevStatus), true));
     memset(p->h_status, 0, sizeof(DevStatus));
     DRX_HIP(ctx, p->mem.alloc(&G.host_words, sizeof(uint64_t), true));
@@ -414,6 +435,8 @@
 uint32_t drx_plan_last_transcode_listed(const drx_plan *p) { return (p && p->h_status && p->dec.last_path == DRX_PATH_TRANSCODE) ? p->h_status->listed : 0u; }
 uint32_t drx_plan_last_pulses_redone(const drx_plan *p) { return (p && p->h_status && p->dec.last_path == DRX_PATH_PULSES) ? p->h_status->redone : 0u; }
 uint32_t drx_plan_last_pulses_listed(const drx_plan *p) { return (p && p->h_status && p->dec.last_path == DRX_PATH_PULSES) ? p->h_status->listed : 0u; }
+uint32_t drx_plan_last_launch_count(const drx_plan *p) { return p ? p->hand.last_launches : 0u; }
+uint32_t drx_plan_last_serial_walks(const drx_plan *p) { return (p && p->h_status) ? p->h_status->serial_walks : 0u; }
 uint32_t drx_plan_last_bins_form(const drx_plan *p) { return p ? p->bins.last_form : 0u; }
 uint32_t drx_plan_last_bins_listed(const drx_plan *p) { return (p && p->h_status && p->dec.last_path == DRX_PATH_BINS) ? p->h_status->listed : 0u; }
 uint32_t drx_plan_last_windows_listed(const drx_plan *p) { return (p && p->h_status && p->dec.last_path == DRX_PATH_WINDOWS) ? p->h_status->listed : 0u; }
diff --git a/deltarice_amd/csrc/drx_api_select.hip b/deltarice_amd/csrc/drx_api_select.hip
--- a/deltarice_amd/csrc/drx_api_select.hip
+++ b/deltarice_amd/csrc/drx_api_select.hip
@@ -22,7 +22,6 @@
     drx_ctx *ctx = p->ctx;
     drx_plan::Selection &S = p->sel;
     if (!S.copied) DRX_HIP(ctx, hipEventCreateWithFlags(&S.copied, hipEventDisableTiming));
-    DRX_HIP(ctx, p->mem.once(&S.d_fail, p->G.n_chunks * sizeof(uint32_t)));
     DRX_HIP(ctx, p->mem.reserve(S.h, bytes, 4, true, Buffers::KeepOld, ctx->stream));
     const hipError_t e = p->mem.reserve(S.d, bytes, 4, false, Buffers::KeepOld, ctx->stream);
     if (e != hipSuccess) return fail(ctx, DRX_ERR_NOMEM, "selection scratch of %zu bytes: %s", Buffers::size(bytes, 4), hipGetErrorString(e));
@@ -66,7 +65,7 @@
     if (d_sideband)
         DRX_HIP(ctx, launch_sideband_tables(c, d_sideband, d_lists, (uint32_t)n_lists));
     else
-        DRX_HIP(ctx, launch_select_walk(c, d_lists, n_class[0], n_class[1], n_class[2], p->sel.d_fail));
+        DRX_HIP(ctx, launch_select_walk(c, d_lists, n_class[0], n_class[1], n_class[2]));
     mark(c.ev, 1, c.s);
     return DRX_OK;
 }
diff --git a/deltarice_amd/csrc/drx_api_stream.hip b/deltarice_amd/csrc/drx_api_stream.hip
--- a/deltarice_amd/csrc/drx_api_stream.hip
+++ b/deltarice_amd/csrc/drx_api_stream.hip
@@ -9,8 +9,11 @@
     DRX_ON_DEVICE(ctx);
     StreamCall c;
     if (const drx_status st = stream_call_begin(p, d_in, in_words, d_chunk_word_off, d_sideband, tables_ready, &c)) return st;
+    const bool scan_was_zero = p->hand.scan_zero[0];
+    p->hand.scan_zero[0] = false;
     DRX_HIP(ctx, launch_decode(c, d_out, (uint64_t *)p->enc.scan.ptr, ctx->decode_impl, p->dec.d_blk, ctx->side.s ? &ctx->side : nullptr,
                                &p->dec.last_path));
+    if (!(p->dec.last_path & DRX_PATH_LANES_FUSED)) p->hand.scan_zero[0] = scan_was_zero;
     return call_end(p, p->dec.last_path);
 }
 
diff --git a/deltarice_amd/csrc/drx_decode_kernels.hip b/deltarice_amd/csrc/drx_decode_kernels.hip
--- a/deltarice_amd/csrc/drx_decode_kernels.hip
+++ b/deltarice_amd/csrc/drx_decode_kernels.hip
@@ -653,6 +653,7 @@
 
     auto launch_lanes = [&](const StreamCall &v, unsigned nb) {
         path |= DRX_PATH_LANES;
+        tally_add(c);
         if (gen)
             k_decode_lanes<false, true><<<nb, 64, 0, v.s>>>(*v.G, v.d_in, v.in_words, v.d_chunk_word_off, v.d_wave_off, v.d_wave_words, nullptr, nullptr, v.d_status, d_out);
         else
@@ -662,9 +663,10 @@
     if (R.walk == Walk::InLaunch) {
         hipError_t e = hipMemsetAsync(d_granules, 0, (G.total_waves + 2) * sizeof(uint64_t), s);
         if (e != hipSuccess) return e;
+        tally_add(c);
     } else if (R.walk == Walk::Parallel) {
         const bool split = R.dec == Dec::LanesSplit;
-        hipError_t e = walk_scratch_reset(G, c.d_pw, s);
+        hipError_t e = walk_scratch_reset(c, R.par);
         if (e != hipSuccess) return e;
         const bool forked = R.par.chunk_wide && R.par.blocks && side && side->s;
         hipStream_t spw = forked ? side->s : s;
@@ -715,6 +717,7 @@
             nb = n_walk + (unsigned)(G.n_chunks * groups);
         }
         path |= DRX_PATH_LANES_FUSED;
+        tally_add(c);
         if (gen)
             k_decode_lanes<true, true><<<nb, 64, 0, s>>>(G, c.d_in, c.in_words, c.d_chunk_word_off, c.d_wave_off, c.d_wave_words, d_granules, ticket, c.d_status, d_out);
         else
@@ -724,6 +727,7 @@
     case Dec::Blocks: {
         const uint32_t *fail = nullptr, *suspect = nullptr;
         bool fused = false;
+        tally_uncounted(c);
         hipError_t e = launch_decode_blocks(c, d_blk, d_out, &fail, &suspect, gen, &fused);
         if (e != hipSuccess) return e;
         path |= DRX_PATH_BLOCKS | (gen ? (fused ? DRX_PATH_IIR_FUSED : DRX_PATH_IIR) : 0u);
@@ -736,6 +740,7 @@
     }
     case Dec::Long:
         path |= DRX_PATH_LONG;
+        tally_add(c);
         k_decode_long<<<(unsigned)G.total_waves, kLongThreads, 0, s>>>(G, c.d_in, c.d_wave_off, c.d_wave_words, c.d_status, d_out, nullptr, nullptr, 0u);
         break;
     case Dec::Lanes:
@@ -745,6 +750,7 @@
         break;
     case Dec::Simple:
         path |= DRX_PATH_SIMPLE;
+        tally_add(c);
         k_decode_simple<<<nb_plain, 64, 0, s>>>(G, c.d_in, c.d_wave_off, c.d_wave_words, c.d_status, d_out, nullptr);
         break;
     }
diff --git a/deltarice_amd/csrc/drx_encode_kernels.hip b/deltarice_amd/csrc/drx_encode_kernels.hip
--- a/deltarice_amd/csrc/drx_encode_kernels.hip
+++ b/deltarice_amd/csrc/drx_encode_kernels.hip
@@ -582,6 +582,7 @@
     mark(c.ev, 0, s);
     hipError_t e = hipMemsetAsync(d_scan, 0, (G.total_waves + 2) * sizeof(uint64_t), s);
     if (e != hipSuccess) return e;
+    tally_add(c, 2);
     mark(c.ev, 1, s);
     mark(c.ev, 2, s);
     uint32_t *ticket = reinterpret_cast<uint32_t *>(d_scan + G.total_waves);
diff --git a/deltarice_amd/csrc/drx_encode_stream.hip b/deltarice_amd/csrc/drx_encode_stream.hip
--- a/deltarice_amd/csrc/drx_encode_stream.hip
+++ b/deltarice_amd/csrc/drx_encode_stream.hip
@@ -22,6 +22,14 @@
 }
 __device__ __forceinline__ void es_store(uint64_t *p, uint64_t v) {
     __hip_atomic_store(p, v, __ATOMIC_RELAXED, __HIP_MEMORY_SCOPE_AGENT);
+}
+
+__device__ __forceinline__ void es_zero_next(uint64_t *__restrict__ next, uint64_t words, DevStatus *next_st) {
+    if (next) {
+        const uint64_t stride = (uint64_t)gridDim.x * blockDim.x;
+        for (uint64_t i = (uint64_t)blockIdx.x * blockDim.x + threadIdx.x; i < words; i += stride) next[i] = 0;
+    }
+    if (next_st && blockIdx.x == 0 && threadIdx.x < sizeof(DevStatus) / sizeof(uint32_t)) reinterpret_cast<uint32_t *>(next_st)[threadIdx.x] = 0;
 }
 
 constexpr uint32_t kScPer = 8;
@@ -181,7 +189,8 @@
                                                               uint64_t out_cap, uint64_t *__restrict__ chunk_word_off,
                                                               uint32_t *__restrict__ wave_words, uint64_t *__restrict__ size,
                                                               uint64_t *__restrict__ place, uint32_t *__restrict__ ctrl,
-                                                              DevStatus *st) {
+                                                              DevStatus *st, uint64_t *__restrict__ next, uint64_t next_words,
+                                                              DevStatus *next_st) {
     __shared__ __attribute__((aligned(16))) uint32_t ring_all[WV][kEsFront + RING + kEsBack];
     __shared__ EsShared<WV> shm;
     __shared__ uint64_t s_place_v[2];
@@ -199,6 +208,7 @@
         shm.place_t[0] = shm.place_t[1] = 0;
     }
     zero_row(row, kRowWords, lane);
+    es_zero_next(next, next_words, next_st);
     __syncthreads();
     const uint64_t n_tickets = (G.total_waves + WV - 1) / WV;
     if (rfl(shm.role) == 0) {
@@ -501,7 +511,8 @@
                                                                    uint32_t *__restrict__ out, uint64_t out_cap,
                                                                    uint64_t *__restrict__ chunk_word_off, uint32_t *__restrict__ wave_words,
                                                                    uint64_t *__restrict__ size, uint64_t *__restrict__ place,
-                                                                   uint32_t *__restrict__ ctrl, DevStatus *st) {
+                                                                   uint32_t *__restrict__ ctrl, DevStatus *st, uint64_t *__restrict__ next,
+                                                                   uint64_t next_words, DevStatus *next_st) {
     __shared__ __attribute__((aligned(16))) uint32_t ring_all[WV][kEsFront + RING + kEsBack];
     __shared__ EsShared<WV> shm;
     __shared__ uint64_t s_place_v[2][2];
@@ -521,6 +532,7 @@
         shm.place_t[0] = shm.place_t[1] = 0;
     }
     zero_row(row, kRowWords, lane);
+    es_zero_next(next, next_words, next_st);
     __syncthreads();
     const uint64_t n_tickets = G.total_waves * tpw;
     if (rfl(shm.role) == 0) {
@@ -763,54 +775,68 @@
     if (pend) copy_out(wait_place());
 }
 
-hipError_t launch_encode_stream(const EncodeCall &c, uint64_t *d_scan) {
+uint64_t stream_scan_words(const Geom &G) { return 2 * ((G.total_waves + kEsWaves - 1) / kEsWaves) + kEsCtrlWords; }
+uint64_t stream_segs_scan_words(const Geom &G, uint32_t seg_target) { return 3 * G.total_waves * es_seg_shape(G.u_wave_len, seg_target).tpw + kEsCtrlWords; }
+
+static hipError_t es_prepare(const EncodeCall &c, const EsScan &sc, uint64_t words) {
+    mark(c.ev, 0, c.s);
+    if (!sc.zero) {
+        const hipError_t e = hipMemsetAsync(sc.cur, 0, words * sizeof(uint64_t), c.s);
+        if (e != hipSuccess) return e;
+        tally_add(c);
+    }
+    mark(c.ev, 1, c.s);
+    mark(c.ev, 2, c.s);
+    return hipSuccess;
+}
+static hipError_t es_launched(const EncodeCall &c, const EsScan &sc) {
+    tally_add(c);
+    if (c.tally) {
+        c.tally->status_handed = c.next_status != nullptr;
+        c.tally->scan_handed = sc.next != nullptr;
+    }
+    mark(c.ev, 3, c.s);
+    return hipGetLastError();
+}
+
+hipError_t launch_encode_stream(const EncodeCall &c, const EsScan &sc) {
     const Geom &G = *c.G;
     const EncOut &o = c.out;
     const hipStream_t s = c.s;
     if (G.total_waves == 0) return hipSuccess;
     const uint64_t W = G.total_waves;
-    const uint64_t tickets = (W + kEsWaves - 1) / kEsWaves;
-    mark(c.ev, 0, s);
-    hipError_t e = hipMemsetAsync(d_scan, 0, (2 * tickets + kEsCtrlWords) * sizeof(uint64_t), s);
-    if (e != hipSuccess) return e;
-    mark(c.ev, 1, s);
-    mark(c.ev, 2, s);
-    uint64_t *size = d_scan, *place = d_scan + tickets;
-    uint32_t *ctrl = reinterpret_cast<uint32_t *>(d_scan + 2 * tickets);
+    const uint64_t tickets = (W + kEsWaves - 1) / kEsWaves, words = stream_scan_words(G);
+    if (const hipError_t e = es_prepare(c, sc, words)) return e;
+    uint64_t *size = sc.cur, *place = sc.cur + tickets;
+    uint32_t *ctrl = reinterpret_cast<uint32_t *>(sc.cur + 2 * tickets);
     const unsigned grid = es_grid(G, tickets);
     if (G.n_taps)
         k_encode_stream<true, kEsWaves, kEsRing><<<grid, 64 * kEsWaves, 0, s>>>(G, c.d_in, o.d_out, o.out_cap, o.d_chunk_word_off, o.d_wave_words,
-                                                                              size, place, ctrl, c.d_status);
+                                                                              size, place, ctrl, c.d_status, sc.next, words, c.next_status);
     else
         k_encode_stream<false, kEsWaves, kEsRing><<<grid, 64 * kEsWaves, 0, s>>>(G, c.d_in, o.d_out, o.out_cap, o.d_chunk_word_off, o.d_wave_words,
-                                                                               size, place, ctrl, c.d_status);
-    mark(c.ev, 3, s);
-    return hipGetLastError();
-}
-
-hipError_t launch_encode_stream_segs(const EncodeCall &c, uint32_t seg_target, uint64_t *d_scan) {
+                                                                               size, place, ctrl, c.d_status, sc.next, words, c.next_status);
+    return es_launched(c, sc);
+}
+
+hipError_t launch_encode_stream_segs(const EncodeCall &c, uint32_t seg_target, const EsScan &sc) {
     const Geom &G = *c.G;
     const EncOut &o = c.out;
     const hipStream_t s = c.s;
     if (G.total_waves == 0) return hipSuccess;
     const EsSegShape sh = es_seg_shape(G.u_wave_len, seg_target);
-    const uint64_t tickets = G.total_waves * sh.tpw;
-    mark(c.ev, 0, s);
-    hipError_t e = hipMemsetAsync(d_scan, 0, (3 * tickets + kEsCtrlWords) * sizeof(uint64_t), s);
-    if (e != hipSuccess) return e;
-    mark(c.ev, 1, s);
-    mark(c.ev, 2, s);
-    uint64_t *size = d_scan, *place = d_scan + tickets;
-    uint32_t *ctrl = reinterpret_cast<uint32_t *>(d_scan + 3 * tickets);
+    const uint64_t tickets = G.total_waves * sh.tpw, words = stream_segs_scan_words(G, seg_target);
+    if (const hipError_t e = es_prepare(c, sc, words)) return e;
+    uint64_t *size = sc.cur, *place = sc.cur + tickets;
+    uint32_t *ctrl = reinterpret_cast<uint32_t *>(sc.cur + 3 * tickets);
     const unsigned grid = es_grid(G, tickets);
     if (G.n_taps)
         k_encode_stream_segs<true, kEsWaves, kEsRing><<<grid, 64 * kEsWaves, 0, s>>>(G, sh.seg_len, sh.tpw, c.d_in, o.d_out, o.out_cap, o.d_chunk_word_off,
-                                                                                   o.d_wave_words, size, place, ctrl, c.d_status);
+                                                                                   o.d_wave_words, size, place, ctrl, c.d_status, sc.next, words, c.next_status);
     else
         k_encode_stream_segs<false, kEsWaves, kEsRing><<<grid, 64 * kEsWaves, 0, s>>>(G, sh.seg_len, sh.tpw, c.d_in, o.d_out, o.out_cap, o.d_chunk_word_off,
-                                                                                    o.d_wave_words, size, place, ctrl, c.d_status);
-    mark(c.ev, 3, s);
-    return hipGetLastError();
-}
-
-}
+                                                                                    o.d_wave_words, size, place, ctrl, c.d_status, sc.next, words, c.next_status);
+    return es_launched(c, sc);
+}
+
+}
diff --git a/deltarice_amd/csrc/drx_internal.h b/deltarice_amd/csrc/drx_internal.h
--- a/deltarice_amd/csrc/drx_internal.h
+++ b/deltarice_amd/csrc/drx_internal.h
@@ -66,13 +66,20 @@
     uint32_t listed;
     uint64_t total_words;
     uint32_t redone;
-    uint32_t pad_;
+    uint32_t serial_walks;
 };
 
 constexpr uint32_t kErrCapacity = 1u;
 constexpr uint32_t kErrCorrupt = 2u;
 constexpr uint32_t kErrInternal = 4u;
 
+struct CallTally {
+    uint32_t launches = 0;
+    bool counted = true;
+    bool status_handed = false;
+    bool scan_handed = false;
+    void add(uint32_t n = 1) { launches += n; }
+};
 struct StreamCall {
     const Geom *G;
     const uint32_t *d_in;
@@ -85,6 +92,8 @@
     DevStatus *d_status;
     hipEvent_t *ev;
     hipStream_t s;
+    DevStatus *next_status = nullptr;
+    CallTally *tally = nullptr;
     StreamCall on(hipStream_t st) const { StreamCall c = *this; c.s = st; return c; }
     StreamCall view(const Geom &Gv) const { StreamCall c = *this; c.G = &Gv; return c; }
 };
@@ -101,7 +110,11 @@
     DevStatus *d_status;
     hipEvent_t *ev;
     hipStream_t s;
-};
+    DevStatus *next_status = nullptr;
+    CallTally *tally = nullptr;
+};
+template <class Call> inline void tally_add(const Call &c, uint32_t n = 1) { if (c.tally) c.tally->add(n); }
+template <class Call> inline void tally_uncounted(const Call &c) { if (c.tally) c.tally->counted = false; }
 
 hipError_t launch_encode(const EncodeCall &c, uint32_t *d_wave_rel, uint64_t *d_chunk_words);
 
@@ -123,11 +136,12 @@
 WalkRoute route_walk(const Geom &G, bool tables_ready, bool have_scratch);
 std::vector<uint32_t> walk_plan_ragged(Geom &G, const ChunkDesc *host_chunks);
 uint64_t walk_scratch_bytes(const Geom &G);
-hipError_t walk_scratch_reset(const Geom &G, void *d_pw, hipStream_t s);
+
 void launch_walk_chunk_wide(const StreamCall &c, bool by_chains);
 void launch_walk_blocks(const StreamCall &c);
 void launch_walk_serial(const StreamCall &c);
 hipError_t launch_batch_walk(const StreamCall &c);
+hipError_t walk_scratch_reset(const StreamCall &c, const WalkRoute &R);
 inline hipError_t batch_walk_prologue(const StreamCall &c) {
     mark(c.ev, 0, c.s);
     const hipError_t e = c.tables_ready ? hipSuccess : launch_batch_walk(c);
@@ -142,8 +156,7 @@
 hipError_t launch_sideband_tables(const StreamCall &c, const uint32_t *d_n, const uint32_t *d_list = nullptr,
                                   uint32_t n_list = 0);
 int select_walk_class(uint32_t n_waves, uint32_t wave_len);
-hipError_t launch_select_walk(const StreamCall &c, const uint32_t *d_lists, uint32_t n_sparse, uint32_t n_block, uint32_t n_chain,
-                              uint32_t *d_fail);
+hipError_t launch_select_walk(const StreamCall &c, const uint32_t *d_lists, uint32_t n_sparse, uint32_t n_block, uint32_t n_chain);
 hipError_t launch_decode_select(const StreamCall &c, const uint64_t *d_sel, uint64_t n_sel, int16_t *d_out, uint64_t stride);
 uint64_t gather_scan_blocks(uint64_t n_sel);
 struct GatherScratch {
@@ -257,7 +270,14 @@
 
 constexpr uint32_t kEsRingWords = 2496;
 constexpr uint64_t kEsMinUnits = 8192;
-hipError_t launch_encode_stream(const EncodeCall &c, uint64_t *d_scan);
+struct EsScan {
+    uint64_t *cur;
+    bool zero;
+    uint64_t *next;
+};
+uint64_t stream_scan_words(const Geom &G);
+uint64_t stream_segs_scan_words(const Geom &G, uint32_t seg_target);
+hipError_t launch_encode_stream(const EncodeCall &c, const EsScan &sc);
 
 constexpr uint32_t kEsSegWaves = 4;
 constexpr uint32_t kEsSegMinLen = 1024, kEsSegMaxLen = 7168;
@@ -282,7 +302,7 @@
                                                        G.total_waves * es_seg_shape(G.u_wave_len, kEsSegMinLen).tpw < 0xffff0000ull; }
 constexpr uint32_t kEsSegsFromLen = 20480;
 inline uint64_t segs_scan_words(const Geom &G, uint32_t seg_target) { return 3 * G.total_waves * es_seg_shape(G.u_wave_len, seg_target).tpw + 192; }
-hipError_t launch_encode_stream_segs(const EncodeCall &c, uint32_t seg_target, uint64_t *d_scan);
+hipError_t launch_encode_stream_segs(const EncodeCall &c, uint32_t seg_target, const EsScan &sc);
 
 bool long_batch_admits(const Geom &G);
 bool long_batch(const Geom &G);
diff --git a/deltarice_amd/csrc/drx_walk.hip b/deltarice_amd/csrc/drx_walk.hip
--- a/deltarice_amd/csrc/drx_walk.hip
+++ b/deltarice_amd/csrc/drx_walk.hip
@@ -257,7 +257,7 @@
 __global__ __launch_bounds__(kSwThreads) void k_walk_sparse(Geom G, const uint32_t *__restrict__ in, uint64_t in_words,
                                                             const uint64_t *__restrict__ chunk_word_off,
                                                             uint64_t *__restrict__ wave_off, uint32_t *__restrict__ wave_words,
-                                                            uint32_t *__restrict__ fail, const uint32_t *__restrict__ list) {
+                                                            DevStatus *st, DevStatus *next_st, const uint32_t *__restrict__ list) {
     __shared__ uint32_t s_a[kSwSegs + 1];
     __shared__ uint32_t s_cnt[kSwSegs], s_base[kSwSegs + 1];
     __shared__ uint32_t s_list[kSwSegs][kSwCap];
@@ -266,6 +266,8 @@
     const int lane = lane_id();
     const uint32_t wv = (uint32_t)wave_id();
     const uint64_t c = list ? (uint64_t)list[blockIdx.x] : blockIdx.x;
+    if (next_st && blockIdx.x == 0 && tid < sizeof(DevStatus) / sizeof(uint32_t)) reinterpret_cast<uint32_t *>(next_st)[tid] = 0;
+    auto by_chains = [&]() -> bool {
     const ChunkGeom f = chunk_geom(G, c);
     const uint32_t W = f.W;
     const uint64_t begin = chunk_word_off[c];
@@ -273,7 +275,7 @@
     if (tid == 0) s_bad = 0;
     bool ok = chunk_extent_usable(begin, end, in_words, kParWalkMaxWords);
     if (ok && in[begin] != f.N) ok = false;
-    if (!ok) { if (tid == 0) fail[c] = 1u; return; }
+    if (!ok) return true;
     const uint32_t len_w = (uint32_t)(end - begin);
     const HeaderBounds hb = header_bounds(f.L, f.N, W, G.k);
     const uint32_t min_full = hb.min_full, max_full = hb.max_full, min_last = hb.min_last, max_last = hb.max_last;
@@ -342,7 +344,7 @@
         if (tid == 63u) s_base[64] = incl;
     }
     __syncthreads();
-    if (s_bad || s_base[64] != W) { if (tid == 0) fail[c] = 1u; return; }
+    if (s_bad || s_base[64] != W) return true;
     bool bad = false;
     for (uint32_t sg = wv; sg < S; sg += blockDim.x >> 6) {
         const uint32_t cnt = rfl(s_cnt[sg]), b0 = rfl(s_base[sg]);
@@ -357,7 +359,14 @@
     }
     if (bad) atomicOr(&s_bad, 1u);
     __syncthreads();
-    if (tid == 0 && s_bad) fail[c] = 1u;
+    return s_bad != 0u;
+    };
+    if (!by_chains()) return;
+    __threadfence();
+    __syncthreads();
+    if (wv != 0u) return;
+    walk_chunks_scalar(G, c, nullptr, c + 1u, in, in_words, chunk_word_off, wave_off, wave_words, nullptr, st);
+    if (lane == 0) atomicAdd(&st->serial_walks, 1u);
 }
 
 constexpr uint32_t kBwTries = 6;
@@ -810,8 +819,10 @@
     return P;
 }
 uint64_t walk_scratch_bytes(const Geom &G) { return par_walks(G, nullptr).bytes; }
-hipError_t walk_scratch_reset(const Geom &G, void *d_pw, hipStream_t s) {
-    return hipMemsetAsync(par_walks(G, d_pw).cnt, 0, 3u * G.n_chunks * sizeof(uint32_t), s);
+hipError_t walk_scratch_reset(const StreamCall &c, const WalkRoute &R) {
+    if (!R.blocks && !(R.chunk_wide && !R.by_chains)) return hipSuccess;
+    tally_add(c);
+    return hipMemsetAsync(par_walks(*c.G, c.d_pw).cnt, 0, 3u * c.G->n_chunks * sizeof(uint32_t), c.s);
 }
 
 std::vector<uint32_t> walk_plan_ragged(Geom &G, const ChunkDesc *d) {
@@ -865,14 +876,18 @@
                             uint32_t *fail) {
     const Geom &G = *c.G;
     if (chain_threads) {
-        k_walk_sparse<<<n, chain_threads, 0, c.s>>>(G, c.d_in, c.in_words, c.d_chunk_word_off, c.d_wave_off, c.d_wave_words, fail, d_list);
-    } else {
-        const uint32_t parts = pw_parts(n);
-        k_pw_scan<<<(unsigned)(n * parts), 256, 0, c.s>>>(G, c.d_in, c.in_words, c.d_chunk_word_off, d_list, cand, cnt, parts);
-        k_walk_parallel<<<n, kPwThreads, 0, c.s>>>(G, c.d_in, c.in_words, c.d_chunk_word_off, c.d_wave_off, c.d_wave_words, fail, d_list, cand, cnt, parts);
-    }
+        k_walk_sparse<<<n, chain_threads, 0, c.s>>>(G, c.d_in, c.in_words, c.d_chunk_word_off, c.d_wave_off, c.d_wave_words, c.d_status,
+                                                    c.next_status, d_list);
+        tally_add(c);
+        if (c.tally) c.tally->status_handed = c.next_status != nullptr;
+        return;
+    }
+    const uint32_t parts = pw_parts(n);
+    k_pw_scan<<<(unsigned)(n * parts), 256, 0, c.s>>>(G, c.d_in, c.in_words, c.d_chunk_word_off, d_list, cand, cnt, parts);
+    k_walk_parallel<<<n, kPwThreads, 0, c.s>>>(G, c.d_in, c.in_words, c.d_chunk_word_off, c.d_wave_off, c.d_wave_words, fail, d_list, cand, cnt, parts);
     k_walk_scalar_only<<<blocks_for(G.n_chunks, kWalkChains), 64, 0, c.s>>>(G, c.d_in, c.in_words, c.d_chunk_word_off, c.d_wave_off,
                                                                             c.d_wave_words, c.d_status, fail);
+    tally_add(c, 3);
 }
 void launch_walk_chunk_wide(const StreamCall &c, bool by_chains) {
     const Geom &G = *c.G;
@@ -904,10 +919,12 @@
     else if (P.bw_B == 2048u) run_bw(std::integral_constant<uint32_t, 2048>{});
     else run_bw(std::integral_constant<uint32_t, 4096>{});
     k_walk_block_only<<<(unsigned)G.n_chunks, 64, 0, c.s>>>(G, c.d_in, c.in_words, c.d_chunk_word_off, c.d_wave_off, c.d_wave_words, c.d_status, P.bw_fail);
+    tally_add(c, 4);
 }
 
 static void walk_serial(const StreamCall &c, const uint32_t *d_short, uint32_t n_short, const uint32_t *d_long, uint32_t n_long) {
     const Geom &G = *c.G;
+    tally_add(c, (n_short ? 1u : 0u) + (n_long ? 1u : 0u));
     if (n_short)
         k_walk_block<<<n_short, 64, 0, c.s>>>(G, c.d_in, c.in_words, c.d_chunk_word_off, d_short, n_short, c.d_wave_off, c.d_wave_words, c.d_status);
     if (n_long && d_long)
@@ -925,7 +942,7 @@
 hipError_t launch_batch_walk(const StreamCall &c) {
     const WalkRoute R = route_walk(*c.G, false, c.d_pw != nullptr);
     if (R.chunk_wide || R.blocks) {
-        const hipError_t e = walk_scratch_reset(*c.G, c.d_pw, c.s);
+        const hipError_t e = walk_scratch_reset(c, R);
         if (e != hipSuccess) return e;
         if (R.chunk_wide) launch_walk_chunk_wide(c, R.by_chains);
         if (R.blocks) launch_walk_blocks(c);
@@ -935,13 +952,8 @@
     return hipGetLastError();
 }
 
-hipError_t launch_select_walk(const StreamCall &c, const uint32_t *d_lists, uint32_t n_sparse, uint32_t n_block, uint32_t n_chain,
-                              uint32_t *d_fail) {
-    if (n_sparse) {
-        const hipError_t e = hipMemsetAsync(d_fail, 0, c.G->n_chunks * sizeof(uint32_t), c.s);
-        if (e != hipSuccess) return e;
-        walk_chunk_wide(c, d_lists, n_sparse, kSwThreads, nullptr, nullptr, d_fail);
-    }
+hipError_t launch_select_walk(const StreamCall &c, const uint32_t *d_lists, uint32_t n_sparse, uint32_t n_block, uint32_t n_chain) {
+    if (n_sparse) walk_chunk_wide(c, d_lists, n_sparse, kSwThreads, nullptr, nullptr, nullptr);
     walk_serial(c, d_lists + n_sparse, n_block, d_lists + n_sparse + n_block, n_chain);
     return hipGetLastError();
 }
diff --git a/include/deltarice_hip.h b/include/deltarice_hip.h
--- a/include/deltarice_hip.h
+++ b/include/deltarice_hip.h
@@ -229,6 +229,8 @@
 #define DRX_ENC_STREAM 5u
 #define DRX_ENC_STREAM_SEGS 6u
 uint32_t drx_plan_last_encode_path(const drx_plan *plan);
+uint32_t drx_plan_last_launch_count(const drx_plan *plan);
+uint32_t drx_plan_last_serial_walks(const drx_plan *plan);
 drx_status drx_plan_read_wave_words(drx_plan *plan, uint32_t *host_out);
 
 drx_status drx_filter_chunk_host(drx_ctx *ctx, int reverse, size_t cd_nelmts,
```

Result: no change. 1555 GB/s (-0.3%).
